# patrickltobing/cyclevae-vc

Measured on AMD Instinct MI355X. Metric: mcep_frames_per_sec_hu1024_ld32_cyc2, higher is better.
Workload: dtype f32 (every matrix product on exact fp32 operands: each operand carried as three fp16 limbs x = l0 + l1/2^11 + l2/2^22, six v_mfma_f32_32x32x16_f16 per product, f32 accumulate; dropped terms < 2^-33 of a product; gates, carried state, projection and outputs f32)

## Files before the change

### cyclevae-vc_amd/_cabi.py

```python
import ctypes as C
import os

ABI_VERSION = 10
FLAG_PERSISTENT = 1
FLAG_PROFILE = 2
FLAG_GENERIC_STEP = 4
FLAG_STEP_TIMING = 8
FLAG_HOISTED_FRONTEND = 32
FLAG_SPLIT_F16 = 256
FLAG_EXACT3 = 512
STATUS_RANGE = 7
STATUS_RANGE_WORD = 3
CLAMP_LAPLACE = 1 << 30

_HERE = os.path.dirname(os.path.abspath(__file__))
DEFAULT_LIB = os.environ.get("CYCLEVAE_LIB") or os.path.join(_HERE, "libcyclevae_hip.so")

_fp = C.c_void_p


class NetDesc(C.Structure):
    _fields_ = [("in_dim", C.c_int32), ("out_dim", C.c_int32), ("hidden", C.c_int32), ("kernel_size", C.c_int32),
                ("layers", C.c_int32), ("has_scale_in", C.c_int32), ("has_scale_out", C.c_int32)]


WEIGHT_FIELDS = ("scale_in_w", "scale_in_b", "conv0_w", "conv0_b", "conv1_w", "conv1_b", "w_ih", "w_hh", "b_ih",
                 "b_hh", "out_w", "out_b", "scale_out_w", "scale_out_b", "conv2_w", "conv2_b")

STATE_KEYS = {"scale_in_w": "scale_in.weight", "scale_in_b": "scale_in.bias", "conv0_w": "conv.conv.0.weight",
              "conv0_b": "conv.conv.0.bias", "conv1_w": "conv.conv.1.weight", "conv1_b": "conv.conv.1.bias",
              "conv2_w": "conv.conv.2.weight", "conv2_b": "conv.conv.2.bias",
              "w_ih": "gru.weight_ih_l0", "w_hh": "gru.weight_hh_l0", "b_ih": "gru.bias_ih_l0",
              "b_hh": "gru.bias_hh_l0", "out_w": "out_1.weight", "out_b": "out_1.bias",
              "scale_out_w": "scale_out.weight", "scale_out_b": "scale_out.bias"}


class NetWeights(C.Structure):
    _fields_ = [(f, _fp) for f in WEIGHT_FIELDS]


GRAD_FIELDS = ("conv0_w", "conv0_b", "conv1_w", "conv1_b", "w_ih", "w_hh", "b_ih", "b_hh", "out_w", "out_b")


class GruLayer(C.Structure):
    _fields_ = [(f, _fp) for f in ("w_ih", "w_hh", "b_ih", "b_hh")]


def upper_layer_keys(n_layers):
    return [tuple("gru.%s_l%d" % (k, l) for k in ("weight_ih", "weight_hh", "bias_ih", "bias_hh")) for l in range(1, n_layers)]


DEEP_PER_STEP, DEEP_GENERIC, DEEP_RESIDENT = 0, 1, 2
EVAL_PER_STEP, EVAL_GENERIC, EVAL_V2, EVAL_V4, EVAL_V5, EVAL_V6, EVAL_LL, EVAL_V6H = range(8)
MAX_LAYERS = 8


class NetGrads(C.Structure):
    _fields_ = [(f, _fp) for f in GRAD_FIELDS]


class Seg(C.Structure):
    _fields_ = [("ptr", _fp), ("width", C.c_int32), ("row_stride", C.c_int32)]


class PassInput(C.Structure):
    _fields_ = [("seg0", Seg), ("seg1", Seg), ("lat", _fp), ("lat_dim", C.c_int32), ("eps", _fp),
                ("seed", C.c_uint64), ("draw_id", C.c_uint64), ("frames", C.c_int32), ("n_draws", C.c_int32),
                ("ctx_before", C.c_int32), ("ctx_after", C.c_int32), ("draw_frame0", C.c_int64), ("eps_draw_stride", C.c_int64)]


class DtwProblem(C.Structure):
    _fields_ = [("org", _fp), ("trg", _fp), ("ld_org", C.c_int64), ("ld_trg", C.c_int64), ("T1", C.c_int32), ("T2", C.c_int32),
                ("D", C.c_int32), ("mcd", C.c_int32), ("aligned", _fp), ("twf", _fp), ("frames", _fp), ("mean_out", _fp)]


STAT_GV, STAT_MCD_SPC, STAT_MCD_L1, STAT_KL, STAT_GATHER64, STAT_LATDIST = range(6)
STAT_MEANSTD64, STAT_MCD64 = 6, 7


class StatJob(C.Structure):
    _fields_ = [("kind", C.c_int32), ("rows", C.c_int32), ("c0", C.c_int32), ("c1", C.c_int32), ("src_rows", C.c_int32),
                ("pad_", C.c_int32), ("a", _fp), ("b", _fp), ("lda", C.c_int64), ("ldb", C.c_int64), ("idx", _fp), ("dst", _fp),
                ("out_off", C.c_int64)]


class LatMeanJob(C.Structure):
    _fields_ = [("lat", _fp), ("eps", _fp), ("draw_id", C.c_uint64), ("frames", C.c_int32), ("pad_", C.c_int32), ("out", _fp)]


class Mc2eJob(C.Structure):
    _fields_ = [("mc", _fp), ("is_f64", C.c_int32), ("T", C.c_int32), ("D", C.c_int32), ("pad_", C.c_int32), ("ld", C.c_int64), ("e_out", _fp)]


# ... 46 lines not shown

                def fn(*args, _raw=raw, _ctx=ctx):
                    return _raw(_ctx, *args)
            self._cache[name] = fn
        return fn


NO_CONTEXT = ("cvae_last_error_string", "cvae_abi_version", "cvae_ctx_create", "cvae_ctx_destroy")
_CDLLS = {}


class CvaeLib(object):

    def __init__(self, path=None, _cdll=None):
        path = path or DEFAULT_LIB
        if not os.path.exists(path):
            raise CvaeError("HIP library %s not found: build it with `python __graft_entry__.py` (hipcc "
                            "--offload-arch=gfx950); there is no CPU fallback" % path)
        self.path = path
        if _cdll is None:
            _cdll = _CDLLS.get(path)
        if _cdll is None:
            _cdll = _CDLLS[path] = self._declare(C.CDLL(path), path)
        self.cdll = _cdll
        self.ctx = C.c_void_p(_cdll.cvae_ctx_create())
        if not self.ctx.value:
            raise CvaeError("cvae_ctx_create failed: %s" % _cdll.cvae_last_error_string().decode())
        self.lib = _Bound(_cdll, self.ctx)

    def new_context(self):
        return CvaeLib(self.path, _cdll=self.cdll)

    def close(self):
        if getattr(self, "ctx", None) is not None and self.ctx.value:
            self.cdll.cvae_ctx_destroy(self.ctx)
            self.ctx = C.c_void_p(None)

    @staticmethod
    def _declare(L, path):
        L.cvae_last_error_string.restype = C.c_char_p
        L.cvae_abi_version.restype = C.c_int
        for fn in ("cvae_net_prepared_bytes", "cvae_net_prepare_scratch_bytes"):
            getattr(L, fn).restype = C.c_size_t
            getattr(L, fn).argtypes = [C.POINTER(NetDesc)]
        L.cvae_net_prepare.restype = C.c_int
        L.cvae_net_prepare.argtypes = [C.POINTER(NetDesc), C.POINTER(NetWeights), _fp, C.c_size_t, _fp, C.c_size_t, _fp]
        L.cvae_net_prepared_in_range.restype = C.c_int
        L.cvae_net_prepared_in_range.argtypes = [C.POINTER(NetDesc), C.c_int, _fp, _fp]
        L.cvae_pass_workspace_bytes.restype = C.c_size_t
        L.cvae_pass_workspace_bytes.argtypes = [C.POINTER(NetDesc), C.c_int, C.c_int]
        L.cvae_gru_rnn_forward.restype = C.c_int
        L.cvae_gru_rnn_forward.argtypes = [C.POINTER(NetDesc), _fp, C.POINTER(PassInput), _fp, _fp, C.c_int, C.c_int,
                                           C.c_int, _fp, _fp, _fp, _fp, C.c_size_t, C.c_int, _fp]
        L.cvae_gru_rnn_forward_stacked.restype = C.c_int
        L.cvae_gru_rnn_forward_stacked.argtypes = [C.POINTER(NetDesc), _fp, C.c_int, C.POINTER(PassInput), C.POINTER(C.c_void_p),
                                                   C.c_int, C.c_int, C.c_int, C.POINTER(C.c_void_p), _fp, C.c_size_t, C.c_int, _fp]
        L.cvae_gru_rnn_forward_stacked_carry.restype = C.c_int
        L.cvae_gru_rnn_forward_stacked_carry.argtypes = [C.POINTER(NetDesc), _fp, C.c_int, C.POINTER(PassInput), C.POINTER(C.c_void_p),
                                                         C.POINTER(C.c_void_p), C.c_int, C.c_int, C.c_int, C.POINTER(C.c_void_p),
                                                         C.POINTER(C.c_void_p), _fp, C.c_size_t, C.c_int, _fp]
        for fn in ("cvae_net_prepared_bytes_deep", "cvae_net_prepare_scratch_bytes_deep"):
            getattr(L, fn).restype = C.c_size_t
            getattr(L, fn).argtypes = [C.POINTER(NetDesc), C.c_int]
        L.cvae_net_prepare_deep.restype = C.c_int
        L.cvae_net_prepare_deep.argtypes = [C.POINTER(NetDesc), C.c_int, C.POINTER(NetWeights), C.POINTER(GruLayer), _fp, C.c_size_t, _fp,
                                            C.c_size_t, _fp]
        L.cvae_pass_workspace_bytes_deep.restype = C.c_size_t
        L.cvae_pass_workspace_bytes_deep.argtypes = [C.POINTER(NetDesc), C.c_int, C.c_int, C.c_int]
        L.cvae_plan_pass.restype = C.c_int
        L.cvae_plan_pass.argtypes = [C.POINTER(NetDesc), C.c_int, C.c_int, C.c_int]
        L.cvae_plan_pass_deep.restype = C.c_int
        L.cvae_plan_pass_deep.argtypes = [C.POINTER(NetDesc), C.c_int, C.c_int, C.c_int, C.c_int]
        L.cvae_gru_rnn_forward_deep.restype = C.c_int
        L.cvae_gru_rnn_forward_deep.argtypes = [C.POINTER(NetDesc), C.c_int, _fp, C.POINTER(PassInput), _fp, _fp, C.c_int, C.c_int,
                                                C.c_int, _fp, _fp, _fp, _fp, C.c_size_t, C.c_int, _fp]
        L.cvae_sample.restype = C.c_int
        L.cvae_sample.argtypes = [_fp, C.c_int, C.c_int, _fp, C.c_uint64, C.c_uint64, _fp, _fp, _fp]
        L.cvae_sample_laplace.restype = C.c_int
        L.cvae_sample_laplace.argtypes = [_fp, C.c_int, C.c_int, _fp, C.c_uint64, C.c_uint64, _fp, _fp, _fp]
        L.cvae_sample_laplace_backward.restype = C.c_int
        L.cvae_sample_laplace_backward.argtypes = [_fp, _fp, _fp, C.c_int, C.c_int, _fp, _fp]
        L.cvae_cycle_workspace_bytes.restype = C.c_size_t
        L.cvae_cycle_workspace_bytes.argtypes = [C.POINTER(NetDesc), C.POINTER(NetDesc), C.c_int, C.c_int, C.c_int]
        L.cvae_cycle_forward.restype = C.c_int
        L.cvae_cycle_forward.argtypes = [C.POINTER(NetDesc), _fp, C.POINTER(NetDesc), _fp, _fp, _fp, C.c_int, _fp, _fp,
                                         C.c_int, _fp, _fp, C.c_int, C.c_int, C.c_int, C.c_int, _fp, C.c_uint64,
                                         _fp, _fp, _fp, _fp, _fp, _fp, C.c_size_t, C.c_int, _fp]
        L.cvae_cycle_forward_carry.restype = C.c_int
        L.cvae_cycle_forward_carry.argtypes = L.cvae_cycle_forward.argtypes + [C.POINTER(CycleState), C.POINTER(CycleState)]
        L.cvae_workspace_status.restype = C.c_int
        L.cvae_workspace_status.argtypes = [_fp, C.POINTER(C.c_int32 * 4), _fp]
        L.cvae_train_image_bytes.restype = C.c_size_t
        L.cvae_train_image_bytes.argtypes = [C.POINTER(NetDesc)]
        L.cvae_net_prepare_train.restype = C.c_int
        L.cvae_net_prepare_train.argtypes = [C.POINTER(NetDesc), C.POINTER(NetWeights), _fp, C.c_size_t, C.c_float, _fp]
        L.cvae_net_prepare_train_v.restype = C.c_int
        L.cvae_net_prepare_train_v.argtypes = [C.POINTER(NetDesc), C.POINTER(NetWeights), _fp, C.c_size_t, C.c_float, C.c_int, _fp]
        L.cvae_train_variants_needed.restype = C.c_int
        L.cvae_train_variants_needed.argtypes = [C.POINTER(NetDesc), C.c_int, C.c_int]
        for fn in ("cvae_train_tape_bytes", "cvae_train_scratch_bytes"):
            getattr(L, fn).restype = C.c_size_t
            getattr(L, fn).argtypes = [C.POINTER(NetDesc), C.c_int, C.c_int]
        L.cvae_gru_rnn_forward_train.restype = C.c_int
        L.cvae_gru_rnn_forward_train.argtypes = [C.POINTER(NetDesc), _fp, _fp, _fp, _fp, C.c_int, C.c_int, C.c_int, _fp, _fp,
                                                 C.c_uint64, C.c_float, _fp, _fp, _fp, _fp, C.c_size_t, _fp, C.c_size_t, _fp]
        L.cvae_gru_rnn_backward.restype = C.c_int
        L.cvae_gru_rnn_backward.argtypes = [C.POINTER(NetDesc), _fp, _fp, C.c_int, C.c_int, C.c_int, _fp, _fp, C.c_size_t, _fp,
                                            C.POINTER(NetGrads), C.c_int, _fp]
        L.cvae_train_debug_counters.restype = C.c_int
        L.cvae_train_debug_counters.argtypes = [C.POINTER(NetDesc), C.c_int, C.c_int, _fp, C.POINTER(C.c_longlong * 8), _fp]
        L.cvae_adam_step.restype = C.c_int
        L.cvae_adam_step.argtypes = [_fp, _fp, _fp, _fp, C.c_size_t, C.c_float, C.c_float, C.c_float, C.c_float, C.c_int, _fp, _fp]
        L.cvae_adam_step_counted.restype = C.c_int
        L.cvae_adam_step_counted.argtypes = [_fp, _fp, _fp, _fp, C.c_size_t, C.c_float, C.c_float, C.c_float, C.c_float, _fp, _fp, _fp]
        L.cvae_sample_cat.restype = C.c_int
        L.cvae_sample_cat.argtypes = [_fp, _fp, _fp, _fp, _fp, C.c_uint64, C.c_uint64, C.c_uint64, C.c_int, C.c_int, C.c_int, C.c_int,
                                      C.c_int, _fp, _fp, _fp]
        L.cvae_sample_cat_backward.restype = C.c_int
        L.cvae_sample_cat_backward.argtypes = [_fp, _fp, _fp, C.c_int, C.c_int, C.c_int, C.c_int, C.c_int, _fp, _fp]
        L.cvae_stage4_loss.restype = C.c_int
        L.cvae_stage4_loss.argtypes = [_fp, _fp, _fp, _fp, _fp, C.c_int, C.c_int, _fp, _fp, C.c_float, C.c_int, C.c_int, C.c_int, C.c_int,
                                       _fp, _fp, _fp, _fp, _fp, _fp, C.c_int, _fp]
        L.cvae_mcd_l1.restype = C.c_int
        L.cvae_mcd_l1.argtypes = [_fp, C.c_long, _fp, C.c_long, C.c_int, C.c_int, _fp, _fp, _fp]
        L.cvae_mcd_l1_backward.restype = C.c_int
        L.cvae_mcd_l1_backward.argtypes = [_fp, C.c_long, _fp, C.c_long, C.c_int, C.c_int, _fp, _fp, _fp, _fp, _fp]
        L.cvae_kl_gauss.restype = C.c_int
        L.cvae_kl_gauss.argtypes = [_fp, C.c_long, C.c_int, C.c_int, _fp, _fp]
        L.cvae_kl_gauss_backward.restype = C.c_int
        L.cvae_kl_gauss_backward.argtypes = [_fp, C.c_long, C.c_int, C.c_int, _fp, _fp, _fp]
        L.cvae_gv_postfilter.restype = C.c_int
        L.cvae_gv_postfilter.argtypes = [_fp, C.c_int, C.c_int, _fp, _fp, _fp, _fp, _fp, _fp, _fp]
        L.cvae_mc2e.restype = C.c_int
        L.cvae_mc2e.argtypes = [_fp, C.c_int, C.c_long, C.c_int, C.c_int, C.c_double, C.c_int, _fp, _fp]
        L.cvae_mcd_aligned.restype = C.c_int
        L.cvae_mcd_aligned.argtypes = [_fp, C.c_long, _fp, C.c_long, C.c_int, C.c_int, C.c_int, C.c_int, _fp, _fp, _fp]
        L.cvae_dtw_work_bytes.restype = C.c_size_t
        L.cvae_dtw_work_bytes.argtypes = [C.c_int, C.c_int]
        L.cvae_dtw_org_to_trg.restype = C.c_int
        L.cvae_dtw_org_to_trg.argtypes = [_fp, _fp, C.c_int, C.c_int, C.c_int, C.c_int, _fp, _fp, _fp, _fp, _fp, C.c_size_t, _fp]
        L.cvae_dtw_batch_work_bytes.restype = C.c_size_t
        L.cvae_dtw_batch_work_bytes.argtypes = [C.c_int, C.c_int, C.c_int]
        L.cvae_dtw_batch.restype = C.c_int
        L.cvae_dtw_batch.argtypes = [C.POINTER(DtwProblem), C.c_int, _fp, C.c_size_t, _fp]
        L.cvae_eval_stats.restype = C.c_int
        L.cvae_eval_stats.argtypes = [_fp, C.c_int, _fp, _fp]
        L.cvae_latent_mean.restype = C.c_int
        L.cvae_latent_mean.argtypes = [C.POINTER(LatMeanJob), C.c_int, C.c_int, C.c_int, C.c_uint64, _fp]
        L.cvae_mc2e_batch_work_bytes.restype = C.c_size_t
        L.cvae_mc2e_batch_work_bytes.argtypes = [C.c_int, C.c_int, C.c_int]
        L.cvae_mc2e_batch.restype = C.c_int
        L.cvae_mc2e_batch.argtypes = [C.POINTER(Mc2eJob), C.c_int, C.c_double, C.c_int, _fp, C.c_size_t, _fp]
        L.cvae_decode_jobs.restype = C.c_int
        L.cvae_decode_jobs.argtypes = [C.POINTER(DecodeJob), C.c_int, _fp, C.c_size_t, _fp]
        L.cvae_step_timing.restype = C.c_int
        L.cvae_step_timing.argtypes = [C.POINTER(NetDesc), C.c_int, C.c_int, _fp, C.POINTER(C.c_double * 8), _fp]
        L.cvae_profile_collect.restype = C.c_int
        L.cvae_profile_collect.argtypes = [C.POINTER(C.c_double), C.POINTER(C.c_int)]
        L.cvae_profile_collect_launches.restype = C.c_int
        L.cvae_profile_collect_launches.argtypes = [C.POINTER(C.c_double), C.POINTER(C.c_int), C.POINTER(C.c_int), C.c_int]
        L.cvae_train_profile_collect.restype = C.c_int
        L.cvae_train_profile_collect.argtypes = [C.POINTER(C.c_double * 4), C.POINTER(C.c_int * 4), C.POINTER(C.c_double * 4)]
        L.cvae_set_status_sink.restype = C.c_int
        L.cvae_set_status_sink.argtypes = [_fp]
        L.cvae_status_latch.restype = C.c_int
        L.cvae_status_latch.argtypes = [_fp, _fp]
# ... 78 lines not shown
        n = len(pins)
        arr = (PassInput * n)(*pins)
        ys = (C.c_void_p * n)(*y_ins)
        outs = (C.c_void_p * n)(*trj_outs)
        self._check(self.lib.cvae_gru_rnn_forward_stacked(C.byref(d), prepared, n, arr, ys, B, T, clamp_lat_dim, outs, ws,
                                                          ws_bytes, flags, stream or None), "cvae_gru_rnn_forward_stacked")

    def gru_rnn_forward_stacked_carry(self, d, prepared, pins, y_ins, h_ins, B, T, clamp_lat_dim, trj_outs, h_lasts, ws, ws_bytes,
                                      flags=0, stream=0):
        n = len(pins)
        arr = (PassInput * n)(*pins)
        ys = (C.c_void_p * n)(*[y or None for y in y_ins])
        hi = (C.c_void_p * n)(*[h or None for h in h_ins])
        outs = (C.c_void_p * n)(*trj_outs)
        hl = (C.c_void_p * n)(*[h or None for h in h_lasts])
        self._check(self.lib.cvae_gru_rnn_forward_stacked_carry(C.byref(d), prepared, n, arr, ys, hi, B, T, clamp_lat_dim, outs, hl,
                                                                ws, ws_bytes, flags, stream or None),
                    "cvae_gru_rnn_forward_stacked_carry")

    def gru_rnn_forward(self, d, prepared, pin, y_in, h_in, B, T, clamp_lat_dim, trj_out, y_last, h_last, ws, ws_bytes,
                        flags=0, stream=0):
        self._check(self.lib.cvae_gru_rnn_forward(C.byref(d), prepared, C.byref(pin), y_in, h_in or None, B, T,
                                                  clamp_lat_dim, trj_out, y_last or None, h_last or None, ws, ws_bytes,
                                                  flags, stream or None), "cvae_gru_rnn_forward")

    def prepared_bytes_deep(self, d, n_layers):
        n = self.lib.cvae_net_prepared_bytes_deep(C.byref(d), n_layers)
        if n == 0:
            raise CvaeError("bad net descriptor / n_layers: %s" % self.lib.cvae_last_error_string().decode())
        return n

    def prepare_scratch_bytes_deep(self, d, n_layers):
        return self.lib.cvae_net_prepare_scratch_bytes_deep(C.byref(d), n_layers)

    def net_prepare_deep(self, d, n_layers, weight_ptrs, upper_ptrs, prepared, prepared_bytes, scratch, scratch_bytes, stream=0):
        if len(upper_ptrs) != n_layers - 1:
            raise CvaeError("net_prepare_deep: %d upper layers given, n_layers=%d" % (len(upper_ptrs), n_layers))
        w = NetWeights(**{f: weight_ptrs.get(f) or None for f in WEIGHT_FIELDS})
        up = (GruLayer * max(1, n_layers - 1))(*[GruLayer(*u) for u in upper_ptrs])
        self._check(self.lib.cvae_net_prepare_deep(C.byref(d), n_layers, C.byref(w), up, prepared, prepared_bytes, scratch,
                                                   scratch_bytes, stream or None), "cvae_net_prepare_deep")

    def pass_workspace_bytes_deep(self, d, n_layers, B, T):
        n = self.lib.cvae_pass_workspace_bytes_deep(C.byref(d), n_layers, B, T)
        if n == 0:
            raise CvaeError("cvae_pass_workspace_bytes_deep: bad arguments (n_layers=%d, B=%d, T=%d)" % (n_layers, B, T))
        return n

    def plan_pass(self, d, rows, T, flags=0):
        rc = self.lib.cvae_plan_pass(C.byref(d), rows, T, flags)
        if rc < 0:
            self._check(rc, "cvae_plan_pass")
        return rc

    def plan_pass_deep(self, d, n_layers, B, T, flags=0):
        rc = self.lib.cvae_plan_pass_deep(C.byref(d), n_layers, B, T, flags)
        if rc < 0:
            self._check(rc, "cvae_plan_pass_deep")
        return rc

    def gru_rnn_forward_deep(self, d, n_layers, prepared, pin, y_in, h_in, B, T, clamp_lat_dim, trj_out, y_last, h_last, ws, ws_bytes,
                             flags=0, stream=0):
        self._check(self.lib.cvae_gru_rnn_forward_deep(C.byref(d), n_layers, prepared, C.byref(pin), y_in, h_in or None, B, T,
                                                       clamp_lat_dim, trj_out, y_last or None, h_last or None, ws, ws_bytes, flags,
                                                       stream or None), "cvae_gru_rnn_forward_deep")

    def sample(self, lat, rows, lat_dim, eps, seed, draw_id, z, eps_out=None, stream=0):
        self._check(self.lib.cvae_sample(lat, rows, lat_dim, eps or None, seed, draw_id, z, eps_out or None,
                                         stream or None), "cvae_sample")

    def sample_laplace(self, lat, rows, lat_dim, eps, seed, draw_id, z, eps_out=None, stream=0):
        self._check(self.lib.cvae_sample_laplace(lat, rows, lat_dim, eps or None, seed, draw_id, z, eps_out or None, stream or None),
                    "cvae_sample_laplace")

    def sample_laplace_backward(self, dz, lat, z, rows, lat_dim, dlat, stream=0):
        self._check(self.lib.cvae_sample_laplace_backward(dz, lat, z, rows, lat_dim, dlat, stream or None), "cvae_sample_laplace_backward")

    def cycle_workspace_bytes(self, de, dd, B, T, n_cyc):
        n = self.lib.cvae_cycle_workspace_bytes(C.byref(de), C.byref(dd), B, T, n_cyc)
        if n == 0:
            raise CvaeError("cvae_cycle_workspace_bytes: bad arguments")
        return n

    def cycle_forward(self, de, enc_prep, dd, dec_prep, x, cvx, stdim, code_src, code_trg, ncode, y_in_enc, y_in_dec,
                      B, T, n_cyc, lat_dim, eps, seed, out_lat, out_rec, out_cv, out_latcv, out_reccyc, ws, ws_bytes,
                      flags=0, stream=0):
        self._check(self.lib.cvae_cycle_forward(C.byref(de), enc_prep, C.byref(dd), dec_prep, x, cvx, stdim, code_src,
                                                code_trg, ncode, y_in_enc, y_in_dec, B, T, n_cyc, lat_dim, eps or None,
                                                seed, out_lat or None, out_rec or None, out_cv or None,
                                                out_latcv or None, out_reccyc or None, ws, ws_bytes, flags,
                                                stream or None), "cvae_cycle_forward")

    def cycle_forward_carry(self, de, enc_prep, dd, dec_prep, x, cvx, stdim, code_src, code_trg, ncode, y_in_enc, y_in_dec,
                            B, T, n_cyc, lat_dim, eps, seed, out_lat, out_rec, out_cv, out_latcv, out_reccyc, ws, ws_bytes,
                            flags=0, stream=0, state_in=None, state_out=None):
        si = CycleState(*state_in) if state_in else None
        so = CycleState(*state_out) if state_out else None
        self._check(self.lib.cvae_cycle_forward_carry(C.byref(de), enc_prep, C.byref(dd), dec_prep, x, cvx, stdim, code_src,
                                                      code_trg, ncode, y_in_enc, y_in_dec, B, T, n_cyc, lat_dim, eps or None,
                                                      seed, out_lat or None, out_rec or None, out_cv or None,
                                                      out_latcv or None, out_reccyc or None, ws, ws_bytes, flags,
                                                      stream or None, C.byref(si) if si else None, C.byref(so) if so else None),
                    "cvae_cycle_forward_carry")

    def train_image_bytes(self, d):
        return self.lib.cvae_train_image_bytes(C.byref(d))

    def net_prepare_train(self, d, weight_ptrs, image, image_bytes, stream=0, gru_drop_p=0.0, variants=7):
        w = NetWeights(**{f: weight_ptrs.get(f) or None for f in WEIGHT_FIELDS})
        self._check(self.lib.cvae_net_prepare_train_v(C.byref(d), C.byref(w), image, image_bytes, gru_drop_p, int(variants),
                                                      stream or None), "cvae_net_prepare_train_v")

    def train_variants_needed(self, d, B, T):
        return self.lib.cvae_train_variants_needed(C.byref(d), B, T)

    def train_tape_bytes(self, d, B, T):
        return self.lib.cvae_train_tape_bytes(C.byref(d), B, T)

    def train_scratch_bytes(self, d, B, T):
        return self.lib.cvae_train_scratch_bytes(C.byref(d), B, T)

    def forward_train(self, d, image, x, y_in, h_in, B, T, clamp_lat_dim, cmask, gmask, seed, p_drop, trj_out, y_last, h_last,
                      tape, tape_bytes, scratch, scratch_bytes, stream=0):
        self._check(self.lib.cvae_gru_rnn_forward_train(C.byref(d), image, x, y_in, h_in or None, B, T, clamp_lat_dim,
                                                        cmask or None, gmask or None, seed, p_drop, trj_out, y_last or None,
                                                        h_last or None, tape, tape_bytes, scratch, scratch_bytes,
                                                        stream or None), "cvae_gru_rnn_forward_train")

    def backward(self, d, image, dout, B, T, clamp_lat_dim, tape, scratch, scratch_bytes, dx, grad_ptrs, accumulate=False,
                 stream=0):
        g = NetGrads(**{f: grad_ptrs[f] for f in GRAD_FIELDS})
        self._check(self.lib.cvae_gru_rnn_backward(C.byref(d), image, dout, B, T, clamp_lat_dim, tape, scratch, scratch_bytes,
                                                   dx or None, C.byref(g), int(bool(accumulate)), stream or None),
                    "cvae_gru_rnn_backward")

    def train_debug_counters(self, d, B, T, scratch, stream=0):
        out = (C.c_longlong * 8)()
        self._check(self.lib.cvae_train_debug_counters(C.byref(d), B, T, scratch, C.byref(out), stream or None),
                    "cvae_train_debug_counters")
        return list(out)

    def adam_step(self, p, g, m, v, n, lr, b1, b2, eps, step, stream=0, gate=None):
        self._check(self.lib.cvae_adam_step(p, g, m, v, n, lr, b1, b2, eps, step, gate or None, stream or None), "cvae_adam_step")

    def adam_step_counted(self, p, g, m, v, n, lr, b1, b2, eps, state, stream=0, gate=None):
        self._check(self.lib.cvae_adam_step_counted(p, g, m, v, n, lr, b1, b2, eps, state, gate or None, stream or None),
                    "cvae_adam_step_counted")

    def sample_cat(self, lat, codes, eps, seed, draws, B, T, lat_dim, ncode, out, eps_out, stream=0):
        parts = len(codes)
        c = list(codes) + [None] * (2 - parts)
        e = list(eps) + [None] * (2 - parts)
        d = list(draws) + [0] * (2 - parts)
        self._check(self.lib.cvae_sample_cat(lat, c[0], c[1] or None, e[0] or None, e[1] or None, seed, d[0], d[1], B, T, lat_dim, ncode,
                                             parts, out, eps_out, stream or None), "cvae_sample_cat")

    def sample_cat_backward(self, dout, lat, eps, B, T, lat_dim, ncode, parts, dlat, stream=0):
        self._check(self.lib.cvae_sample_cat_backward(dout, lat, eps, B, T, lat_dim, ncode, parts, dlat, stream or None),
                    "cvae_sample_cat_backward")

    def stage4_loss(self, rec, reccyc, lat, latcv, x, x_stride, stdim, w, latcv_w, kl_scale, B, T, D, lat_dim, d_rec, d_reccyc, d_lat,
                    d_latcv, frame_loss, loss, accumulate, stream=0):
        self._check(self.lib.cvae_stage4_loss(rec, reccyc or None, lat, latcv or None, x, x_stride, stdim, w, latcv_w or None, kl_scale,
                                              B, T, D, lat_dim, d_rec, d_reccyc or None, d_lat, d_latcv or None, frame_loss, loss,
                                              int(bool(accumulate)), stream or None), "cvae_stage4_loss")

# ... 48 lines not shown
        arr = (Mc2eJob * max(1, len(jobs)))(*jobs)
        self._check(self.lib.cvae_mc2e_batch(arr, len(jobs), alpha, irlen, work, work_bytes, stream or None), "cvae_mc2e_batch")

    def decode_jobs(self, jobs, work, work_bytes, stream=0):
        arr = (DecodeJob * max(1, len(jobs)))(*jobs)
        self._check(self.lib.cvae_decode_jobs(arr, len(jobs), work, work_bytes, stream or None), "cvae_decode_jobs")

    def step_timing(self, d, B, T, ws, stream=0):
        out = (C.c_double * 8)()
        self._check(self.lib.cvae_step_timing(C.byref(d), B, T, ws, C.byref(out), stream or None), "cvae_step_timing")
        return list(out)

    def set_status_sink(self, ptr):
        self._check(self.lib.cvae_set_status_sink(ptr or None), "cvae_set_status_sink")

    def status_latch(self, latch, stream=0):
        self._check(self.lib.cvae_status_latch(latch, stream or None), "cvae_status_latch")

    def set_draw_origin(self, row0, global_rows, frames_per_row=0):
        self._check(self.lib.cvae_set_draw_origin(row0, global_rows, frames_per_row), "cvae_set_draw_origin")

    def selftest_limbs(self, x_ptr, y_ptr, n, stream=None):
        self._check(self.lib.cvae_selftest_limbs(x_ptr, y_ptr, n, stream), "cvae_selftest_limbs")

    def selftest_occupy(self, blocks, lds_bytes, cycles, stream=None):
        self._check(self.lib.cvae_selftest_occupy(blocks, lds_bytes, cycles, stream), "cvae_selftest_occupy")

    def selftest_gemm_work_bytes(self):
        return self.lib.cvae_selftest_gemm_work_bytes()

    def selftest_gemm(self, case, work, work_bytes, stream=None):
        ran = (C.c_int32 * 4)()
        self._check(self.lib.cvae_selftest_gemm(C.byref(case), work or None, work_bytes, C.byref(ran), stream or None), "cvae_selftest_gemm")
        return list(ran)

    def set_side_stream(self, stream):
        self._check(self.lib.cvae_set_side_stream(stream), "cvae_set_side_stream")

    def join_side_stream(self, stream):
        self._check(self.lib.cvae_join_side_stream(stream), "cvae_join_side_stream")

    def set_draw_parts(self, parts):
        self._check(self.lib.cvae_set_draw_parts(parts), "cvae_set_draw_parts")

    def set_option(self, name, value):
        self._check(self.lib.cvae_set_option(name.encode(), int(value)), "cvae_set_option")

    def get_option(self, name):
        v = C.c_int64(0)
        self._check(self.lib.cvae_get_option(name.encode(), C.byref(v)), "cvae_get_option")
        return v.value

    def reset_options(self):
        self._check(self.lib.cvae_reset_options(), "cvae_reset_options")

    def profile_collect(self):
        ms, n = C.c_double(0.0), C.c_int(0)
        self._check(self.lib.cvae_profile_collect(C.byref(ms), C.byref(n)), "cvae_profile_collect")
        return ms.value, n.value

    def profile_collect_launches(self, cap=4096):
        ms, rows, cin = (C.c_double * cap)(), (C.c_int * cap)(), (C.c_int * cap)()
        n = self.lib.cvae_profile_collect_launches(ms, rows, cin, cap)
        if n < 0:
            raise CvaeError("cvae_profile_collect_launches failed (%d): %s" % (n, self.lib.cvae_last_error_string().decode()))
        return [(ms[i], rows[i], cin[i]) for i in range(n)]

    TRAIN_PROFILE_CLASSES = ("fwd_recurrence", "bwd_recurrence", "forward_and_dgrad_gemms", "wgrad_gemms")

    def train_profile_collect(self):
        ms, n, fl = (C.c_double * 4)(), (C.c_int * 4)(), (C.c_double * 4)()
        self._check(self.lib.cvae_train_profile_collect(C.byref(ms), C.byref(n), C.byref(fl)), "cvae_train_profile_collect")
        return {name: (ms[i], n[i], fl[i]) for i, name in enumerate(self.TRAIN_PROFILE_CLASSES)}

    def workspace_status(self, ws, stream=0):
        st = (C.c_int32 * 4)()
        self._check(self.lib.cvae_workspace_status(ws, C.byref(st), stream or None), "cvae_workspace_status")
        return list(st)


EXPORTS = ("cvae_last_error_string", "cvae_abi_version", "cvae_ctx_create", "cvae_ctx_destroy", "cvae_set_status_sink", "cvae_status_latch", "cvae_set_draw_origin", "cvae_set_draw_parts",
           "cvae_set_option", "cvae_get_option", "cvae_reset_options", "cvae_selftest_limbs", "cvae_selftest_occupy", "cvae_selftest_gemm_work_bytes", "cvae_selftest_gemm", "cvae_set_side_stream", "cvae_join_side_stream", "cvae_net_prepared_bytes", "cvae_net_prepare_scratch_bytes",
           "cvae_net_prepare", "cvae_pass_workspace_bytes", "cvae_gru_rnn_forward", "cvae_gru_rnn_forward_stacked", "cvae_gru_rnn_forward_stacked_carry", "cvae_sample", "cvae_sample_laplace", "cvae_sample_laplace_backward",
           "cvae_cycle_workspace_bytes", "cvae_cycle_forward", "cvae_cycle_forward_carry", "cvae_profile_collect", "cvae_profile_collect_launches", "cvae_train_profile_collect", "cvae_step_timing", "cvae_workspace_status",
           "cvae_train_image_bytes", "cvae_net_prepare_train", "cvae_net_prepare_train_v", "cvae_train_variants_needed", "cvae_train_tape_bytes", "cvae_train_scratch_bytes",
           "cvae_gru_rnn_forward_train", "cvae_gru_rnn_backward", "cvae_adam_step", "cvae_adam_step_counted", "cvae_train_debug_counters",
           "cvae_sample_cat", "cvae_sample_cat_backward", "cvae_stage4_loss", "cvae_mcd_l1", "cvae_mcd_l1_backward", "cvae_kl_gauss",
           "cvae_kl_gauss_backward",
           "cvae_gv_postfilter", "cvae_mcd_aligned", "cvae_mc2e", "cvae_dtw_work_bytes", "cvae_dtw_org_to_trg",
           "cvae_dtw_batch_work_bytes", "cvae_dtw_batch", "cvae_eval_stats", "cvae_latent_mean",
           "cvae_mc2e_batch_work_bytes", "cvae_mc2e_batch", "cvae_decode_jobs",
           "cvae_net_prepared_bytes_deep", "cvae_net_prepare_scratch_bytes_deep", "cvae_net_prepare_deep", "cvae_pass_workspace_bytes_deep",
           "cvae_plan_pass", "cvae_plan_pass_deep", "cvae_gru_rnn_forward_deep", "cvae_net_prepared_in_range")
```

### cyclevae-vc_amd/csrc/cvae_exact3.h

```cpp
#pragma once
#include <cvae_intrin.h>

#if defined(__HIP_DEVICE_COMPILE__)
#define CVAE_V6_IN_AGPR(x) asm volatile("" : "+a"(x))
#else
#define CVAE_V6_IN_AGPR(x) ((void)0)
#endif

struct Step6Params {
    const float* gx0;
    const float* w2s;
    float* hbuf;
    long mtot;
    float* hx;
    const float* wrec3;
    const float* afold3;
    const float* cfold;
    const float* bhn;
    const float* xt;
    int Tp, Cp;
    int B, Bp, H, T;
    unsigned* flags;
    int* status;
    long long* prof;
// ... 319 lines not shown
            if (live) {
                float sg[4];
#pragma unroll
                for (int g = 0; g < 4; ++g)
                    sg[g] = red[(0 * 32 + row) * RS + g * 8 + u] + red[(1 * 32 + row) * RS + g * 8 + u] +
                            red[(2 * 32 + row) * RS + g * 8 + u] + red[(3 * 32 + row) * RS + g * 8 + u];
                const float rg = cvae_sigmoid_fast(gxr + sg[0]);
                const float zg = cvae_sigmoid_fast(gxz + sg[1]);
                const float ng = cvae_tanh_fast(gxn + sg[2] + rg * (sg[3] + bhn));
                hn_ = ng + zg * (hold - ng);
            }
            if (keep1) hkeep1 = hn_; else hkeep0 = hn_;
            hsh[row * 8 + u] = hn_;
            unsigned short l0, l1;
            unsigned char l2;
            cvae_split3_f16b8(hn_, l0, l1, l2);
            hl[row * 8 + u] = l0;
            hl[256 + row * 8 + u] = l1;
            ((unsigned char*)(hl + 512))[row * 8 + u] = l2;
        }
        __syncthreads();
        if (tid < 64) {
            const unsigned so = ((unsigned)(c >> 1) * tstride + tile0 + (unsigned)(p.Bp >> 5)) * 2560u;
            cvae_buf_store_f4_sc1(xb_, (unsigned)(c & 1) * 512u + (unsigned)(tid & 31) * 16u, so + (unsigned)(tid >> 5) * 1024u,
                                  *(const f32x4*)(hl + tid * 8));
            if (LIMBS == 3 && tid < 32)
                cvae_buf_store_f2_sc1(xb_, 2048u + (unsigned)(c & 1) * 256u + (unsigned)tid * 8u, so, *(const f32x2*)(hl + 512 + tid * 4));
            cvae_drain_vmem();
            cvae_wave_barrier();
            if (tid == 0) cvae_atomic_store_agent(p.flags + (long)i * NB + c, (unsigned)(t + 1));
        } else if (tid < 128 && p.want_f32) {
            const int l = tid - 64, r = l >> 1, half = l & 1;
            *(f32x4*)(p.hbuf + (((long)(c >> 1) * p.mtot + row0 + p.Bp + r) * 16 + (c & 1) * 8 + half * 4)) =
                *(const f32x4*)(hsh + r * 8 + half * 4);
        }
        if constexpr (!HOIST) {
            if (k + 1 < ntask && (xmode == 1 || (xmode == 2 && wave == 0))) {
#pragma unroll
                for (int s = 0; s < RF; ++s) load_x(s);
            }
        }
        if (ntile > 1 && k + 1 < ntask) {
            const int kn = k + 1, tn = kn / ntile, in_ = ti + (kn % ntile) * rts;
            fpre = (unsigned)tn;
            if (tn > 0 && lane < 2 * KPW && 2 * s_lo + lane < NB)
                fpre = cvae_atomic_load_agent(p.flags + (long)in_ * NB + 2 * s_lo + lane);
        }
        if constexpr (FPRE && FW0_EARLY) { if (k + 1 < ntask) load_fw(0); }
        if constexpr (PROF) { const long long c1 = cvae_clock(); pc[3] += c1 - c0; c0 = c1; }
    }
    if constexpr (PROF) {
        if (p.prof && tid == 64 * ((p.exp >> 2) & 3))
            for (int q = 0; q < 4; ++q) p.prof[(long)blockIdx.x * 4 + q] = pc[q];
    }
}

struct Out6Params {
    const float* hx;
    long mtot;
    const float* wo3;
    const float* bo2;
    int H, Bp, T, B, ncell, Co, clamp_from;
    float clamp_min;
    float* out[CVAE_MAX_CELLS];
};

__global__ void k_prep_wo3(const float* wo2, float* wo3, int H, int Cop, int NT, int* unfit) {
    const int nk = H >> 4;
    const long idx = (long)blockIdx.x * blockDim.x + threadIdx.x;
    if (idx < (long)NT * nk * 512) {
        const int e = (int)(idx & 7), lane = (int)((idx >> 3) & 63), s = (int)((idx >> 9) % nk), n = (int)((idx >> 9) / nk);
        const int col = 32 * n + (lane & 31), k = 16 * s + 8 * (lane >> 5) + e;
        const float w = col < Cop ? wo2[(long)col * H + k] : 0.0f;
        unsigned short l0, l1, l2;
        cvae_split3_f16(w, l0, l1, l2);
        cvae_flag_unfit(unfit, w);
        unsigned short* dst = (unsigned short*)wo3 + (((long)n * nk + s) * 3) * 512 + lane * 8 + e;
        dst[0] = l0;
        dst[512] = l1;
        dst[1024] = l2;
    }
}

template <int KPW>
__global__ __launch_bounds__(256) void k_outproj_v6(Out6Params p) {
    constexpr float S1 = 1.0f / 2048.0f;
    constexpr int RS = 36;
    const int tid = threadIdx.x, wave = cvae_uniform(tid >> 6), lane = tid & 63, lc = lane & 31, kh = lane >> 5;
    const int nk = p.H >> 4, nt32 = p.Bp >> 5;
    const int n = blockIdx.y;
    const long tile = (long)nt32 + blockIdx.x;
    float* red = (float*)CVAE_SMEM;
    const long tstride = p.mtot >> 5;
    f32x16 a0 = cvae_zero16(), a1 = cvae_zero16(), a2 = cvae_zero16(), a3 = cvae_zero16();
    constexpr int RD = KPW < 4 ? KPW : 4;
    f32x4 ha[2 * RD], wb[3 * RD];
    f32x2 hb[RD];
    auto load = [&](int s) {
        const int sg = wave * KPW + s;
        const unsigned char* hp = (const unsigned char*)p.hx + ((long)sg * tstride + tile) * 2560;
        ha[2 * (s % RD)] = *(const f32x4*)(hp + kh * 512 + lc * 16);
        ha[2 * (s % RD) + 1] = *(const f32x4*)(hp + 1024 + kh * 512 + lc * 16);
        hb[s % RD] = *(const f32x2*)(hp + 2048 + kh * 256 + lc * 8);
        const float* wp = p.wo3 + (((long)n * nk + sg) * 3) * 256 + lane * 4;
#pragma unroll
        for (int m = 0; m < 3; ++m) wb[3 * (s % RD) + m] = *(const f32x4*)(wp + m * 256);
    };
    const bool has_k = wave * KPW < nk;
    if (has_k) {
#pragma unroll
        for (int s = 0; s < RD; ++s) load(s);
#pragma unroll
        for (int s = 0; s < KPW; ++s) {
            const f32x4 l0 = ha[2 * (s % RD)], l1 = ha[2 * (s % RD) + 1], l2 = cvae_bf8x8_to_h8(hb[s % RD]);
            const f32x4 w0 = wb[3 * (s % RD)], w1 = wb[3 * (s % RD) + 1], w2 = wb[3 * (s % RD) + 2];
            a0 = cvae_mfma_32x32x16_f16(l0, w0, a0);
            a1 = cvae_mfma_32x32x16_f16(l0, w1, a1);
            a2 = cvae_mfma_32x32x16_f16(l1, w1, a2);
            a3 = cvae_mfma_32x32x16_f16(l0, w2, a3);
            a1 = cvae_mfma_32x32x16_f16(l1, w0, a1);
            a2 = cvae_mfma_32x32x16_f16(l2, w0, a2);
            cvae_sched_fence();
            if (s + RD < KPW) load(s + RD);
        }
    }
#pragma unroll
    for (int q = 0; q < 16; ++q)
        red[(wave * 32 + (q & 3) + 8 * (q >> 2) + 4 * kh) * RS + lc] = a0[q] + (a1[q] + (a2[q] + a3[q]) * S1) * S1;
    __syncthreads();
    {
        const int r = tid >> 3;
        const long m = (long)blockIdx.x * 32 + r;
        const int t = (int)(m / p.Bp), b = (int)(m - (long)t * p.Bp);
        if (b < p.ncell * p.B) {
            const int cell = b / p.B, bb = b - cell * p.B;
            float* orow = p.out[cell] + ((long)bb * p.T + t) * p.Co;
#pragma unroll
            for (int jj = 0; jj < 4; ++jj) {
                const int cl = (tid & 7) + 8 * jj, col = 32 * n + cl;
                if (col < p.Co) {
                    float v = red[(0 * 32 + r) * RS + cl] + red[(1 * 32 + r) * RS + cl] + red[(2 * 32 + r) * RS + cl] +
                              red[(3 * 32 + r) * RS + cl] + p.bo2[col];
                    if (p.clamp_from >= 0 && col >= p.clamp_from) v = fmaxf(v, p.clamp_min);
                    orow[col] = v;
                }
            }
        }
    }
}

__global__ void k_selftest_occupy(long long cycles, int lds_words) {
    float* occupy_lds = (float*)CVAE_SMEM;
    for (int i = threadIdx.x; i < lds_words; i += blockDim.x) occupy_lds[i] = (float)i;
    __syncthreads();
    const long long t0 = cvae_clock();
    float acc = 0.f;
    int guard = 0;
    while (cvae_clock() - t0 < cycles && ++guard < (1 << 28)) {
        acc += occupy_lds[(threadIdx.x * 33 + guard) % (lds_words > 0 ? lds_words : 1)];
        cvae_sleep();
    }
    if (acc == -1.0f) occupy_lds[0] = acc;
}

__global__ void k_selftest_limbs(const float* x, float* y, long n) {
    const long i0 = 8 * ((long)blockIdx.x * blockDim.x + threadIdx.x);
    if (i0 + 8 > n) return;
    unsigned short l0[8], l1[8];
    unsigned char b[8];
#pragma unroll
    for (int e = 0; e < 8; ++e) cvae_split3_f16b8(x[i0 + e], l0[e], l1[e], b[e]);
    unsigned w0 = 0, w1 = 0;
#pragma unroll
    for (int e = 0; e < 4; ++e) {
        w0 |= (unsigned)b[e] << (8 * e);
        w1 |= (unsigned)b[4 + e] << (8 * e);
    }
    const f32x2 raw = (f32x2){__builtin_bit_cast(float, w0), __builtin_bit_cast(float, w1)};
    const f32x4 h8 = cvae_bf8x8_to_h8(raw);
#pragma unroll
    for (int e = 0; e < 8; ++e) {
        const float pair = h8[e >> 1];
        const unsigned bits = __builtin_bit_cast(unsigned, pair);
        const unsigned short hb = (unsigned short)((e & 1) ? bits >> 16 : bits & 0xffffu);
        y[i0 + e] = cvae_f16_bits_to_f32(l0[e]) + cvae_f16_bits_to_f32(l1[e]) * (1.0f / 2048.0f) +
                    cvae_f16_bits_to_f32(hb) * (1.0f / 4194304.0f);
    }
}
```

### cyclevae-vc_amd/csrc/cvae_kernels.h

```cpp
#pragma once
#include <cvae_intrin.h>
#include <stdint.h>

struct CvaeSeg {
    const float* ptr;
    int width;
    int row_stride;
};

__device__ __forceinline__ void cvae_philox(uint32_t c0, uint32_t c1, uint32_t c2, uint32_t c3, uint32_t k0,
                                            uint32_t k1, uint32_t out[4]) {
    for (int i = 0; i < 10; ++i) {
        const uint64_t p0 = (uint64_t)0xD2511F53u * c0, p1 = (uint64_t)0xCD9E8D57u * c2;
        const uint32_t n0 = (uint32_t)(p1 >> 32) ^ c1 ^ k0, n1 = (uint32_t)p1;
        const uint32_t n2 = (uint32_t)(p0 >> 32) ^ c3 ^ k1, n3 = (uint32_t)p0;
        c0 = n0; c1 = n1; c2 = n2; c3 = n3;
        k0 += 0x9E3779B9u; k1 += 0xBB67AE85u;
    }
    out[0] = c0; out[1] = c1; out[2] = c2; out[3] = c3;
}

__device__ __forceinline__ void cvae_randn_pair(uint32_t w0, uint32_t w1, float& zc, float& zs) {
    const float u1 = ((float)(w0 >> 8) + 0.5f) * (1.0f / 16777216.0f);
    const float u2 = ((float)(w1 >> 8) + 0.5f) * (1.0f / 16777216.0f);
// ... 83 lines not shown
        const int a = col >> 2, u = col & 3, j = 4 * g + u, k = 16 * c + kk;
        const int gate = a < 3 ? a : 2;
        double s = 0.0;
        if (a < 3) {
            const float* wrow = wih + (long)(gate * H + j) * tot + c2;
            for (int q = 0; q < Co; ++q) s += (double)wrow[q] * (double)wo[(long)q * H + k];
        }
        if (a != 2) s += (double)whh[(long)(gate * H + j) * H + k];
        wrec[idx] = (float)s;
    }
}

__global__ void k_prep_wrec2(const float* wih, const float* whh, const float* wo, float* wrec2, int c2, int Co,
                             int tot, int H) {
    const int nch = H >> 4;
    const long idx = (long)blockIdx.x * blockDim.x + threadIdx.x;
    if (idx < (long)nch * 4 * nch * 256) {
        const int kk = (int)(idx & 15), u = (int)((idx >> 4) & 15);
        const int c = (int)((idx >> 8) % nch), a = (int)(((idx >> 8) / nch) & 3), jg = (int)((idx >> 8) / nch / 4);
        const int j = 16 * jg + u, k = 16 * c + kk;
        const int gate = a < 3 ? a : 2;
        double s = 0.0;
        if (a < 3) {
            const float* wrow = wih + (long)(gate * H + j) * tot + c2;
            for (int q = 0; q < Co; ++q) s += (double)wrow[q] * (double)wo[(long)q * H + k];
        }
        if (a != 2) s += (double)whh[(long)(gate * H + j) * H + k];
        wrec2[idx] = (float)s;
    }
}

__global__ void k_prep_wo2(const float* wo, const float* bo, const float* sw, const float* sb, float* wo2, float* bo2,
                           int Co, int Cop, int H) {
    const long idx = (long)blockIdx.x * blockDim.x + threadIdx.x;
    if (idx < (long)Cop * H) {
        const int k = (int)(idx % H), c = (int)(idx / H);
        double s = 0.0;
        if (c < Co) {
            if (sw)
                for (int q = 0; q < Co; ++q) s += (double)sw[(long)c * Co + q] * (double)wo[(long)q * H + k];
            else
                s = (double)wo[(long)c * H + k];
        }
        wo2[idx] = (float)s;
    } else if (idx < (long)Cop * H + Cop) {
        const int c = (int)(idx - (long)Cop * H);
        double s = 0.0;
        if (c < Co) {
            if (sw) {
                s = (double)sb[c];
                for (int q = 0; q < Co; ++q) s += (double)sw[(long)c * Co + q] * (double)bo[q];
            } else {
                s = (double)bo[c];
            }
        }
        bo2[c] = (float)s;
    }
}

__global__ void k_copy2d(float* dst, long dld, const float* src, long sld, int rows, int cols) {
    const long idx = (long)blockIdx.x * blockDim.x + threadIdx.x;
    if (idx < (long)rows * cols) {
        const int c = (int)(idx % cols), r = (int)(idx / cols);
        dst[(long)r * dld + c] = src[(long)r * sld + c];
    }
}

struct ProCell {
    CvaeSeg seg0, seg1;
    const float* lat;
    const float* eps;
    uint64_t seed, draw;
    const float* y_in;
    const float* h_in;
    int frames;
    int n_draws;
    int ctx_before, ctx_after;
    long draw_frame0;
    long eps_stride;
};
#define CVAE_FRAME_VALID(p, c, t) ((t) >= -(c).ctx_before && (t) < ((c).frames > 0 ? (c).frames : (p).T) + (c).ctx_after)

#define CVAE_MAX_CELLS 32
struct ProParams {
    ProCell cell[CVAE_MAX_CELLS];
    int ncell, L;
    uint64_t frame0;
    const float* sin_w;
    const float* sin_b;
    const float* wo;
    const float* bo;
    int B, T, C, Cp, pad, Co, H, Bp, nslack, nzero;
    long mtot;
    float* xnp;
    float* hbuf;
    float* hx;
    float* xt;
    int nxt_slack;
    float* hs;
    float* xs;
    long xs_plane;
    float* dy;
    unsigned* zero_words;
    int* zero_status;
    int zero_status_n;
    unsigned* ll_counter;
    int nA, nH, nD;
    int nG;
    float* gx0;
    const float* wyT;
    int* range_word;
    int* range_epoch;
    int range_val;
    float range_at;
    const int* image_unfit;
};
#ifndef CVAE_STATUS_RANGE_WORD
#define CVAE_STATUS_RANGE_WORD 3
#endif
#define CVAE_WS_RANGE_WORD 20
#define CVAE_WS_RANGE_EPOCH 21
#define CVAE_LIMB_MAX 65504.0f
__device__ __forceinline__ bool cvae_out_of_range(float v, float bound) { return !(fabsf(v) < bound); }
__device__ __forceinline__ void cvae_flag_unfit(int* unfit, float w) {
    if (cvae_out_of_range(w, CVAE_LIMB_MAX)) *unfit = 1;
}
static_assert(sizeof(ProParams) <= 4096, "ProParams is a kernel argument: 4 KiB at most");

__device__ __forceinline__ float cvae_input_value(const ProParams& p, const ProCell& c, int b, int t, int q, const float* emean = nullptr) {
    const long fr = (long)b * p.T + t;
    if (q < c.seg0.width) return c.seg0.ptr[fr * c.seg0.row_stride + q];
    if (!c.lat) return c.seg1.ptr[fr * c.seg1.row_stride + (q - c.seg0.width)];
    const int l = q - c.seg0.width;
    float e;
    if (c.n_draws > 1 && emean) {
        e = emean[l];
    } else if (c.n_draws > 1) {
        e = 0.0f;
        const long es = c.eps_stride ? c.eps_stride : (long)p.B * p.T * p.L;
        for (int k = 0; k < c.n_draws; ++k)
            e += c.eps ? c.eps[(long)k * es + fr * p.L + l]
                       : cvae_randn(c.seed, c.draw + (uint64_t)k, (uint64_t)(fr + c.draw_frame0) + p.frame0, (uint32_t)l);
        e *= 1.0f / (float)c.n_draws;
    } else {
        e = c.eps ? c.eps[fr * p.L + l] : cvae_randn(c.seed, c.draw, (uint64_t)(fr + c.draw_frame0) + p.frame0, (uint32_t)l);
    }
    return c.lat[fr * 2 * p.L + l] + expf(c.lat[fr * 2 * p.L + p.L + l] * 0.5f) * e;
}

__device__ __forceinline__ void cvae_mean_draws(const ProParams& p, const ProCell& c, int b, int t, float* part, float* emean) {
    const int tid = threadIdx.x, L = p.L, nq = L >> 2, nsl = 256 / nq, qd = tid % nq, sl = tid / nq;
    const long fr = (long)b * p.T + t;
    const long es = c.eps_stride ? c.eps_stride : (long)p.B * p.T * p.L;
    if (sl < nsl) {
        float e[4] = {0.f, 0.f, 0.f, 0.f};
        for (int k = sl; k < c.n_draws; k += nsl) {
            float z[4];
            if (c.eps) {
                const float* ep = c.eps + (long)k * es + fr * p.L + 4 * qd;
                z[0] = ep[0]; z[1] = ep[1]; z[2] = ep[2]; z[3] = ep[3];
            } else {
                cvae_randn4(c.seed, c.draw + (uint64_t)k, (uint64_t)(fr + c.draw_frame0) + p.frame0, (uint32_t)qd, z);
            }
#pragma unroll
            for (int j = 0; j < 4; ++j) e[j] += z[j];
        }
#pragma unroll
        for (int j = 0; j < 4; ++j) part[sl * L + 4 * qd + j] = e[j];
    }
    __syncthreads();
    if (tid < L) {
        float m = 0.0f;
        for (int q = 0; q < nsl; ++q) m += part[q * L + tid];
        emean[tid] = m * (1.0f / (float)c.n_draws);
    }
    __syncthreads();
}

__global__ void k_prologue(ProParams p) {
    const int tid = threadIdx.x, blk = blockIdx.x;
    const int Tp = p.T + 2 * p.pad;
    if (blk < p.nA && p.xt) {
        float* raw = (float*)CVAE_SMEM;
        unsigned char* img = (unsigned char*)(raw + 32 * (p.C + 1));
        const int tile = blk / Tp, tp = blk % Tp, t = tp - p.pad, np = p.Cp >> 3;
        float* tmean = (float*)(img + np * 1280);
        const bool quads = p.L > 0 && (p.L & 3) == 0;
        if (quads) {
            const int nq = p.L >> 2;
            for (int item = tid; item < 32 * nq; item += 256) {
                const int r = item / nq, qd = item - r * nq, bb = tile * 32 + r;
                if (bb >= p.ncell * p.B) continue;
                const ProCell& c = p.cell[bb / p.B];
                if (!c.lat || c.n_draws <= 1 || !CVAE_FRAME_VALID(p, c, t)) continue;
                const long fr = (long)(bb % p.B) * p.T + t, es = c.eps_stride ? c.eps_stride : (long)p.B * p.T * p.L;
                float e[4] = {0.f, 0.f, 0.f, 0.f};
                for (int k = 0; k < c.n_draws; ++k) {
                    float z[4];
                    if (c.eps) {
                        const float* ep = c.eps + (long)k * es + fr * p.L + 4 * qd;
                        z[0] = ep[0]; z[1] = ep[1]; z[2] = ep[2]; z[3] = ep[3];
                    } else {
                        cvae_randn4(c.seed, c.draw + (uint64_t)k, (uint64_t)(fr + c.draw_frame0) + p.frame0, (uint32_t)qd, z);
                    }
#pragma unroll
                    for (int j = 0; j < 4; ++j) e[j] += z[j];
                }
#pragma unroll
                for (int j = 0; j < 4; ++j) tmean[r * p.L + 4 * qd + j] = e[j] * (1.0f / (float)c.n_draws);
            }
            __syncthreads();
        }
        for (int idx = tid; idx < 32 * p.C; idx += 256) {
            const int r = idx / p.C, q = idx - r * p.C, bb = tile * 32 + r;
            float v = 0.0f;
            if (bb < p.ncell * p.B) {
                const ProCell& c = p.cell[bb / p.B];
                if (CVAE_FRAME_VALID(p, c, t)) v = cvae_input_value(p, c, bb % p.B, t, q, quads ? tmean + r * p.L : nullptr);
            }
            raw[r * (p.C + 1) + q] = v;
        }
        __syncthreads();
        const ProCell* const cells = p.cell;
        bool bad = false;
        for (int q = tid & 63; q < p.Cp; q += 64) {
            float v[8];
            bool ok[8];
#pragma unroll
            for (int i = 0; i < 8; ++i) {
                const int r = (tid >> 6) + 4 * i, bb = tile * 32 + r;
                ok[i] = false;
                if (bb < p.ncell * p.B) {
                    const ProCell& c = cells[bb / p.B];
                    ok[i] = CVAE_FRAME_VALID(p, c, t) && q < p.C;
                }
                v[i] = !ok[i] ? 0.0f : (p.sin_w ? p.sin_b[q] : raw[r * (p.C + 1) + q]);
            }
            if (p.sin_w && q < p.C)
                for (int k = 0; k < p.C; ++k) {
                    const float w = p.sin_w[(long)q * p.C + k];
#pragma unroll
                    for (int i = 0; i < 8; ++i) v[i] += w * raw[((tid >> 6) + 4 * i) * (p.C + 1) + k];
                }
            unsigned char* pc = img + (q >> 3) * 1280;
#pragma unroll
            for (int i = 0; i < 8; ++i) {
                const int r = (tid >> 6) + 4 * i;
                unsigned short l0, l1;
                unsigned char l2;
                cvae_split3_f16b8(ok[i] ? v[i] : 0.0f, l0, l1, l2);
                bad = bad || (ok[i] && cvae_out_of_range(v[i], p.range_at));
                ((unsigned short*)pc)[r * 8 + (q & 7)] = l0;
                ((unsigned short*)(pc + 512))[r * 8 + (q & 7)] = l1;
                pc[1024 + r * 8 + (q & 7)] = l2;
            }
        }
        const bool fits = cvae_block_all(!bad);
        if (!fits && p.range_word && tid == 0) *p.range_word = p.range_val;
        f32x4* dst = (f32x4*)((unsigned char*)p.xt + ((long)tile * Tp + tp) * np * 1280);
        for (int e = tid; e < np * 80; e += 256) dst[e] = ((const f32x4*)img)[e];
        return;
    }
    if (p.nG > 0 && blk >= p.nA + p.nH + p.nD && blk < p.nA + p.nH + p.nD + p.nG) {
        const long q4 = ((long)(blk - p.nA - p.nH - p.nD) * blockDim.x + tid) * 4, H3 = 3L * p.H;
        if (q4 < (long)p.ncell * p.B * H3) {
            const int bb = (int)(q4 / H3), col = (int)(q4 - (long)bb * H3);
            const float* yi = p.cell[bb / p.B].y_in + (long)(bb % p.B) * p.Co;
            float a0 = 0.f, a1 = 0.f, a2 = 0.f, a3 = 0.f;
            int c = 0;
            for (; c + 8 <= p.Co; c += 8) {
                float d[8], w[8][4];
#pragma unroll
                for (int q = 0; q < 8; ++q) {
                    d[q] = yi[c + q] - p.bo[c + q];
                    const float* wp = p.wyT + (long)(c + q) * H3 + col;
                    w[q][0] = wp[0]; w[q][1] = wp[1]; w[q][2] = wp[2]; w[q][3] = wp[3];
                }
#pragma unroll
                for (int q = 0; q < 8; ++q) { a0 += w[q][0] * d[q]; a1 += w[q][1] * d[q]; a2 += w[q][2] * d[q]; a3 += w[q][3] * d[q]; }
            }
            for (; c < p.Co; ++c) {
                const float d = yi[c] - p.bo[c];
                const float* w = p.wyT + (long)c * H3 + col;
                a0 += w[0] * d; a1 += w[1] * d; a2 += w[2] * d; a3 += w[3] * d;
            }
            float* o = p.gx0 + (long)bb * H3 + col;
            o[0] = a0; o[1] = a1; o[2] = a2; o[3] = a3;
        }
        return;
    }
    const float* emean = nullptr;
    if (blk < p.nA && blockDim.x == 256) {
        const int tp = blk % Tp, bb = blk / Tp, t = tp - p.pad;
        if (bb < p.ncell * p.B) {
            const ProCell& c = p.cell[bb / p.B];
            if (c.lat && c.n_draws > 1 && p.L <= 256 && (p.L & 3) == 0 && CVAE_FRAME_VALID(p, c, t)) {
                float* part = (float*)CVAE_SMEM + p.C;
                cvae_mean_draws(p, c, bb % p.B, t, part, part + 1024);
                emean = part + 1024;
            }
        }
    }
    if (tid >= 64) return;
    if (blk < p.nA) {
        float* row = (float*)CVAE_SMEM;
        const int tp = blk % Tp, bb = blk / Tp, t = tp - p.pad;
        const bool real_row = bb < p.ncell * p.B;
        const int ci = real_row ? bb / p.B : 0, b = real_row ? bb % p.B : 0;
        const ProCell& c = p.cell[ci];
        const bool valid = real_row && CVAE_FRAME_VALID(p, c, t);
        const long fr = (long)b * p.T + t;
        if (valid)
            for (int q = tid; q < p.C; q += 64) row[q] = cvae_input_value(p, c, b, t, q, emean);
        __syncthreads();
        bool bad = false;
        for (int q = tid; q < p.Cp; q += 64) {
            float v = 0.0f;
            if (valid && q < p.C) {
                if (p.sin_w) {
                    v = p.sin_b[q];
                    for (int r = 0; r < p.C; ++r) v += p.sin_w[(long)q * p.C + r] * row[r];
                } else {
                    v = row[q];
                }
            }
            if (real_row) p.xnp[((long)bb * Tp + tp) * p.Cp + q] = v;
            if (p.xs) {
                unsigned short hi, lo;
                cvae_split_f16(v, hi, lo);
                unsigned short* xh = (unsigned short*)p.xs + ((long)bb * Tp + tp) * p.Cp + q;
                xh[0] = hi;
                xh[p.xs_plane] = lo;
                bad = bad || cvae_out_of_range(v, p.range_at);
            }
        }
        if (p.xs && p.range_word && !cvae_wave_all(!bad) && tid == 0) *p.range_word = p.range_val;
    } else if (blk < p.nA + p.nH) {
        const long base = (long)(blk - p.nA) * 1024;
        bool any_h = false;
        for (int c = 0; c < p.ncell; ++c) any_h = any_h || p.cell[c].h_in != nullptr;
        if (!any_h) {
            const f32x4 z4 = (f32x4){0.f, 0.f, 0.f, 0.f};
            const long nel = (long)p.Bp * p.H, hb_ = blk - p.nA;
            for (int e = 0; e < 4; ++e) {
                const long idx = base + 4 * (e * 64 + tid);
                if (idx < nel) *(f32x4*)(p.hbuf + ((idx >> 4) / p.Bp * p.mtot + (idx >> 4) % p.Bp) * 16 + (idx & 15)) = z4;
            }
            if (p.hx) {
                const long per = (long)(p.Bp >> 5) * 160, npc = (long)(p.H >> 4) * per;
                for (int e = 0; e < 5; ++e) {
                    const long pi = hb_ * 320 + e * 64 + tid;
                    if (pi < npc) *(f32x4*)((unsigned char*)p.hx + (pi / per) * (p.mtot >> 5) * 2560 + (pi % per) * 16) = z4;
                }
            }
            if (p.hs) {
                const long per = (long)p.Bp * 4, npc = (long)(p.H >> 4) * per;
                for (int e = 0; e < 4; ++e) {
                    const long pi = hb_ * 256 + e * 64 + tid;
                    if (pi < npc) *(f32x4*)((unsigned char*)p.hs + (pi / per) * p.mtot * 64 + (pi % per) * 16) = z4;
                }
            }
            return;
        }
        bool bad = false;
        for (int e = 0; e < 16; ++e) {
            const long idx = base + e * 64 + tid;
            if (idx < (long)p.Bp * p.H) {
                const int kk = (int)(idx & 15), r = (int)((idx >> 4) % p.Bp), ch = (int)((idx >> 4) / p.Bp);
                float v = 0.0f;
                if (r < p.ncell * p.B) {
                    const float* h_in = p.cell[r / p.B].h_in;
                    if (h_in) v = h_in[(long)(r % p.B) * p.H + 16 * ch + kk];
                }
                p.hbuf[((long)ch * p.mtot + r) * 16 + kk] = v;
                bad = bad || cvae_out_of_range(v, p.range_at);
                if (p.hx) {
                    unsigned short l0, l1;
                    unsigned char l2;
                    cvae_split3_f16b8(v, l0, l1, l2);
                    unsigned char* pc = (unsigned char*)p.hx + ((long)ch * (p.mtot >> 5) + (r >> 5)) * 2560;
                    const int at = (kk >> 3) * 256 + (r & 31) * 8 + (kk & 7);
                    ((unsigned short*)pc)[at] = l0;
                    ((unsigned short*)(pc + 1024))[at] = l1;
                    pc[2048 + at] = l2;
                }
                if (p.hs) {
                    unsigned short hi, lo;
                    cvae_split_f16(v, hi, lo);
                    unsigned short* hrow = (unsigned short*)p.hs + ((long)ch * p.mtot + r) * 32;
                    hrow[kk] = hi;
                    hrow[16 + kk] = lo;
                }
            }
        }
        if (p.range_word && !cvae_wave_all(!bad) && tid == 0) *p.range_word = p.range_val;
    } else if (blk < p.nA + p.nH + p.nD) {
        const int idx = (blk - p.nA - p.nH) * 64 + tid;
        if (idx < p.ncell * p.B * p.Co) {
            const int q = idx % p.Co, bb = idx / p.Co;
            const ProCell& c = p.cell[bb / p.B];
            const int b = bb % p.B;
            float yh = p.bo[q];
            if (c.h_in && c.y_in)
                for (int k = 0; k < p.H; ++k) yh += p.wo[(long)q * p.H + k] * c.h_in[(long)b * p.H + k];
            p.dy[idx] = c.y_in ? c.y_in[(long)b * p.Co + q] - yh : 0.0f;
        }
    } else {
        for (int q = tid; q < p.nslack; q += 64) p.xnp[(long)p.ncell * p.B * Tp * p.Cp + q] = 0.0f;
        if (p.xs)
            for (int q = tid; q < p.nslack; q += 64) {
                unsigned short* xh = (unsigned short*)p.xs + (long)p.ncell * p.B * Tp * p.Cp + q;
                xh[0] = 0;
                xh[p.xs_plane] = 0;
            }
        if (p.xt)
            for (int q = tid; q < p.nxt_slack; q += 64) ((unsigned short*)p.xt)[(long)(p.Bp >> 5) * Tp * (p.Cp >> 3) * 640 + q] = 0;
        for (int q = tid; q < p.nzero; q += 64) p.zero_words[q] = 0u;
        if (p.zero_status && tid < p.zero_status_n && tid != CVAE_STATUS_RANGE_WORD) p.zero_status[tid] = 0;
        if (tid == 0) {
            if (p.range_epoch) *p.range_epoch = p.range_val;
            if (p.range_word && p.image_unfit && *p.image_unfit) *p.range_word = p.range_val;
        }
        if (p.ll_counter && tid == 0) *p.ll_counter += 1u;
    }
}

__global__ void k_sample(const float* lat, int rows, int L, const float* eps, uint64_t seed, uint64_t draw,
                         float* z, float* eps_out, uint64_t frame0) {
    const long idx = (long)blockIdx.x * blockDim.x + threadIdx.x;
    if (idx < (long)rows * L) {
        const int l = (int)(idx % L);
        const long n = idx / L;
        const float e = eps ? eps[idx] : cvae_randn(seed, draw, (uint64_t)n + frame0, (uint32_t)l);
        z[idx] = lat[n * 2 * L + l] + expf(lat[n * 2 * L + L + l] * 0.5f) * e;
        if (eps_out) eps_out[idx] = e;
    }
}

__global__ void k_sample_laplace(const float* lat, int rows, int L, const float* eps, uint64_t seed, uint64_t draw, float* z,
                                 float* eps_out, uint64_t frame0) {
    const long idx = (long)blockIdx.x * blockDim.x + threadIdx.x;
    if (idx < (long)rows * L) {
        const int l = (int)(idx % L);
        const long n = idx / L;
        float e;
        if (eps) {
            e = eps[idx];
        } else {
            const uint64_t frame = (uint64_t)n + frame0;
            uint32_t o[4];
            cvae_philox((uint32_t)frame, (uint32_t)l >> 2, (uint32_t)draw, (uint32_t)(frame >> 32), (uint32_t)seed, (uint32_t)(seed >> 32), o);
            e = -0.4999f + 0.9999f * (((float)o[l & 3] + 0.5f) * 2.3283064365386963e-10f);
            e = fminf(fmaxf(e, -0.4999f), 0.49999997f);
        }
        const float sgn = e > 0.f ? 1.f : (e < 0.f ? -1.f : 0.f);
        z[idx] = lat[n * 2 * L + l] - expf(lat[n * 2 * L + L + l]) * sgn * log1pf(-2.0f * fabsf(e));
        if (eps_out) eps_out[idx] = e;
    }
}
__global__ void k_sample_laplace_bwd(const float* dz, const float* lat, const float* z, int rows, int L, float* dlat) {
    const long idx = (long)blockIdx.x * blockDim.x + threadIdx.x;
    if (idx < (long)rows * L) {
        const int l = (int)(idx % L);
        const long n = idx / L;
        const float g = dz[idx];
        dlat[n * 2 * L + l] = g;
        dlat[n * 2 * L + L + l] = g * (z[idx] - lat[n * 2 * L + l]);
    }
}

template <int TM, int TN, int WGM, int WGN, bool A_CHUNKED>
__global__ __launch_bounds__(64 * WGM * WGN) void k_gemm_nt(const float* __restrict__ A, long lda, long a_plane,
                                                            const float* __restrict__ Bm, long ldb,
                                                            const float* __restrict__ bias, float* __restrict__ C,
                                                            long ldc, int M, int N, int K) {
    const int wave = threadIdx.x >> 6, lane = threadIdx.x & 63, lr = lane & 15, kq = lane >> 4;
    const int wm = wave / WGN, wn = wave % WGN;
    const int m0 = (blockIdx.y * WGM + wm) * TM * 16, n0 = (blockIdx.x * WGN + wn) * TN * 16;
    f32x4 acc[TM][TN];
#pragma unroll
    for (int i = 0; i < TM; ++i)
#pragma unroll
        for (int j = 0; j < TN; ++j) acc[i][j] = (f32x4){0.f, 0.f, 0.f, 0.f};
    long arow[TM], brow[TN];
#pragma unroll
    for (int i = 0; i < TM; ++i) {
        int r = m0 + 16 * i + lr;
        r = r < M ? r : M - 1;
        arow[i] = A_CHUNKED ? (long)r * 16 + 4 * kq : (long)r * lda + 4 * kq;
    }
#pragma unroll
    for (int j = 0; j < TN; ++j) {
        int c = n0 + 16 * j + lr;
        c = c < N ? c : N - 1;
        brow[j] = (long)c * ldb + 4 * kq;
    }
    for (int k0 = 0; k0 < K; k0 += 16) {
        float4 a[TM], b[TN];
        const long aoff = A_CHUNKED ? (long)(k0 >> 4) * a_plane * 16 : (long)k0;
#pragma unroll
        for (int i = 0; i < TM; ++i) a[i] = *(const float4*)(A + arow[i] + aoff);
#pragma unroll
        for (int j = 0; j < TN; ++j) b[j] = *(const float4*)(Bm + brow[j] + k0);
#pragma unroll
        for (int i = 0; i < TM; ++i)
#pragma unroll
            for (int j = 0; j < TN; ++j) {
                acc[i][j] = cvae_mfma_16x16x4(a[i].x, b[j].x, acc[i][j]);
                acc[i][j] = cvae_mfma_16x16x4(a[i].y, b[j].y, acc[i][j]);
// ... 828 lines not shown
```

### cyclevae-vc_amd/csrc/cvae_lib.hip

```cpp
#include <cvae_intrin.h>

#include <stdarg.h>
#include <stdio.h>
#include <stdlib.h>
#include <string.h>

#include <atomic>
#include <map>
#include <mutex>
#include <new>
#include <utility>
#include <vector>

#include "cvae_kernels.h"
#include "cvae_train_kernels.h"
#include "cvae_deep.h"
#include "cyclevae_hip.h"

namespace {

thread_local char g_err[512] = "";

enum OptId {
    OPT_V6_LIMBS_H64, OPT_NO_LL, OPT_MAX_RT, OPT_LL_BACKOFF, OPT_EXP, OPT_GEMM_FORCE, OPT_GEMM_LOG, OPT_TRAIN_OLD_GEMM,
    OPT_GEMM_TRACE, OPT_TRAIN_PER_STEP, OPT_TRAIN_PROF, OPT_TRAIN_BACKOFF, OPT_TRAIN_FP32_MFMA, OPT_TRAIN_BWD_PER_STEP, OPT_TRAIN_KERNEL, OPT_X3_TILE, OPT_BWD_OVERFLOW_AT, OPT_GEMM_MAX_SPLIT, OPT_BWD_KS, OPT_COOP_LAUNCH, OPT_V6_LIMBS_H2048, OPT_V6_W2S_H64, OPT_STEP_COL_TILES, OPT_TRAIN_PROFILE, OPT_TRAIN_XMAP, OPT_MASKS_ON_SIDE, OPT_V6_BACKOFF, OPT_TRAIN_BWD_BACKOFF, OPT_LL_ROW_PAD, OPT_GEMM_MIN_DEPTH, OPT_TRAIN_BWD_GEOM, OPT_BWD_W3_L1_H64, OPT_TRAIN_FWD_GEOM, OPT_TRAIN_FWD_BACKOFF, OPT_EXACT_RANGE_AT, OPT_DTW_BATCH_COST, OPT_COUNT
};
struct OptEntry { const char* name; long dflt; };
const OptEntry g_opt[OPT_COUNT] = {
    {"v6_limbs_h64", 3},
    {"no_ll", 0},
    {"max_rt", 0},
    {"ll_backoff", -1},
    {"exp", 0},
    {"gemm_force", 0},
    {"gemm_log", 0},
    {"train_old_gemm", 0},
    {"gemm_trace", 0},
    {"train_per_step", 0},
    {"train_prof", 0},
    {"train_backoff", 32},
    {"train_fp32_mfma", 0},
    {"train_bwd_per_step", 0},
    {"train_kernel", 0},
    {"x3_tile", 0},
    {"bwd_overflow_at", 60000},
    {"gemm_max_split", 16},
    {"bwd_ks", 8},
    {"coop_launch", 0},
    {"v6_limbs_h2048", 3},
    {"v6_w2s_h64", 0},
    {"step_col_tiles", 0},
    {"train_profile", 0},
    {"train_xmap", 0},
    {"masks_on_side", 1},
    {"v6_backoff", -1},
    {"train_bwd_backoff", -1},
    {"ll_row_pad", 0},
    {"gemm_min_depth", 128},
    {"train_bwd_geom", -1},
    {"bwd_w3_l1_h64", 0},
    {"train_fwd_geom", -1},
    {"train_fwd_backoff", -1},
    {"exact_range_at", 65504},
    {"dtw_batch_cost", 1},
};

struct ProfEvents {
    std::vector<hipEvent_t> start, stop;
    std::vector<int> rows, cin;
    size_t used = 0;
};
enum { TPROF_FWD = 0, TPROF_BWD = 1, TPROF_GEMM = 2, TPROF_WGRAD = 3, TPROF_CLASSES = 4 };
struct TrainProfEvents {
    std::vector<hipEvent_t> start, stop;
    std::vector<int> cls;
    std::vector<double> flop;
    size_t used = 0;
};
struct SideDone { const void* scratch; hipEvent_t ev; };

}

struct cvae_ctx {
    int32_t* status_sink = nullptr;
    long draw_row0 = 0, draw_rows = 0, draw_frames = 0, draw_parts = 1;
    long opt[OPT_COUNT];
    ProfEvents prof;
    TrainProfEvents tprof;
    hipStream_t side = nullptr;
    SideDone side_done[8] = {};
    hipEvent_t side_ready = nullptr, side_join = nullptr, side_last = nullptr;
    int side_cap = 0;
    hipEvent_t mask_fork = nullptr, mask_join = nullptr;
    unsigned side_evict = 0;
    int32_t* gemm_ran = nullptr;
    std::map<const void*, std::pair<int, unsigned long>> train_var;
    unsigned long train_var_tick = 0;
    std::map<const void*, bool> image_unfit;
    int range_serial = 0;
    std::atomic<unsigned> ll_train_launch{1u};
};

namespace {

thread_local cvae_ctx* tl_ctx = nullptr;
inline cvae_ctx& cx() { return *tl_ctx; }
inline long opt(OptId i) { return tl_ctx->opt[i]; }
struct CtxScope {
    cvae_ctx* prev;
    explicit CtxScope(cvae_ctx* c) : prev(tl_ctx) {
        tl_ctx = c;
        g_cvae_coop_launch = (int)c->opt[OPT_COOP_LAUNCH];
    }
    ~CtxScope() { tl_ctx = prev; }
};

int fail(int code, const char* fmt, ...) {
    va_list ap;
    va_start(ap, fmt);
    vsnprintf(g_err, sizeof(g_err), fmt, ap);
    va_end(ap);
    return code;
}

#define CVAE_ENTER(c)                                                          \
    if (!(c)) return fail(-1, "null context (cvae_ctx_create)");               \
    CtxScope cvae_scope_(c)
#define CVAE_ENTER_SZ(c)                                                       \
    if (!(c)) {                                                                \
        (void)fail(-1, "null context (cvae_ctx_create)");                      \
        return 0;                                                              \
    }                                                                          \
    CtxScope cvae_scope_(c)

#define CVAE_HIP_OK(expr)                                                                         \
    do {                                                                                          \
        hipError_t e_ = (expr);                                                                   \
        if (e_ != hipSuccess) return fail(-3, "%s failed: %s", #expr, hipGetErrorString(e_));     \
    } while (0)

inline long up(long x, long m) { return (x + m - 1) / m * m; }
inline int clamp_dim(int v) { return v < 0 ? -1 : (v & ~CVAE_CLAMP_LAPLACE); }
inline float clamp_floor(int v) { return v >= 0 && (v & CVAE_CLAMP_LAPLACE) ? -7.2543288692621097f : -13.815510557964274f; }
inline unsigned nblk(long n, int per) { return (unsigned)((n + per - 1) / per); }

struct Dims {
    int C, Cp, Co, Cop, H, H3, ks, layers, R, pad, cl[3], cw, tot, Kfe, nch, KFW;
};

int make_dims(const cvae_net_desc* d, Dims* o) {
    if (!d) return fail(-1, "null net descriptor");
    if (d->layers < 1 || d->layers > 3) return fail(-1, "layers (reference dilation_size) must be 1, 2 or 3, got %d", d->layers);
    if (d->kernel_size < 1 || d->kernel_size % 2 == 0) return fail(-1, "kernel_size must be odd, got %d", d->kernel_size);
    if (d->hidden < 16 || d->hidden % 16) return fail(-1, "hidden must be a positive multiple of 16, got %d", d->hidden);
    if (d->in_dim < 1 || d->out_dim < 1) return fail(-1, "bad in_dim/out_dim %d/%d", d->in_dim, d->out_dim);
    if (d->layers == 3 && d->kernel_size != 3)
        return fail(-1, "layers == 3 needs kernel_size == 3: a front-end of kernel_size^3 >= 125 frames is not supported, got kernel_size %d",
                    d->kernel_size);
    if (d->layers == 3 && d->hidden % 64)
        return fail(-1, "layers == 3 needs hidden to be a multiple of 64, got %d", d->hidden);
    o->C = d->in_dim;
    o->Cp = (int)up(d->in_dim, 8);
    o->Co = d->out_dim;
    o->Cop = (int)up(d->out_dim, 16);
    o->H = d->hidden;
    o->H3 = 3 * d->hidden;
    o->ks = d->kernel_size;
    o->layers = d->layers;
    o->R = 1;
    o->cl[0] = o->cl[1] = o->cl[2] = 0;
    for (int i = 0; i < o->layers; ++i) {
        o->R *= o->ks;
        o->cl[i] = o->R * o->C;
    }
    o->pad = (o->R - 1) / 2;
    o->cw = o->R * o->C;
    o->tot = o->cw + o->Co;
    o->Kfe = (int)up((long)o->R * o->Cp, 16);
    o->nch = o->H / 16;
    o->KFW = (o->Kfe / 16 + 3) / 4;
    return 0;
}

int make_train_dims(const cvae_net_desc* d, Dims* o) {
    if (int rc = make_dims(d, o)) return rc;
    if (o->layers != 2)
        return fail(-1, "training is implemented for layers (reference dilation_size) == 2 only, got %d (eval and conversion run 1..3)", o->layers);
    return 0;
}

struct FoldScratch { long ma, mb, ba, bb, total; };
inline long fold_m_size(const Dims& m, int n) { return (long)m.cl[n] * (m.cl[n] / m.C) * m.C; }
inline FoldScratch fold_scratch(const Dims& m) {
    FoldScratch f;
    f.ma = 0;
    f.mb = fold_m_size(m, m.layers - 1);
    f.ba = f.mb + (m.layers > 1 ? fold_m_size(m, m.layers - 2) : 0);
    f.bb = f.ba + m.cw;
    f.total = f.bb + (m.layers > 1 ? m.cl[m.layers - 2] : 0) + 64;
    return f;
}

struct V6Inst { int H, KFW, limbs; bool w2s; void (*fn)(Step6Params); void (*fn_prof)(Step6Params); };
#define V6_PAIR(KPW, KFW, LIMBS) k_gru_steps_v6<KPW, KFW, LIMBS>, k_gru_steps_v6<KPW, KFW, LIMBS, false, true>
#define V6_W2S(KPW, KFW) k_gru_steps_v6<KPW, KFW, 3, true>, nullptr
const V6Inst g_v6_inst[] = {
    {1024, 8, 3, false, V6_PAIR(16, 8, 3)},  {1024, 6, 3, false, V6_PAIR(16, 6, 3)},
    {1024, 3, 3, false, V6_PAIR(16, 3, 3)},  {1024, 2, 3, false, V6_PAIR(16, 2, 3)},
    {2048, 8, 3, true, V6_W2S(32, 8)},       {2048, 11, 3, true, V6_W2S(32, 11)},
    {2048, 8, 2, false, V6_PAIR(32, 8, 2)},  {2048, 11, 2, false, V6_PAIR(32, 11, 2)},
    {64, 3, 3, false, V6_PAIR(1, 3, 3)},     {64, 2, 3, false, V6_PAIR(1, 2, 3)},          {64, 1, 3, false, V6_PAIR(1, 1, 3)},
    {64, 3, 3, true, V6_W2S(1, 3)},          {64, 2, 3, true, V6_W2S(1, 2)},               {64, 1, 3, true, V6_W2S(1, 1)},
    {64, 3, 2, false, V6_PAIR(1, 3, 2)},     {64, 2, 2, false, V6_PAIR(1, 2, 2)},          {64, 1, 2, false, V6_PAIR(1, 1, 2)},
};
const int V6H_MIN_KFW = 12;
const V6Inst g_v6h_inst[] = {
    {1024, 0, 3, false, V6_PAIR(16, 0, 3)},
    {2048, 0, 3, true, V6_W2S(32, 0)},
    {64, 0, 3, false, V6_PAIR(1, 0, 3)},     {64, 0, 3, true, V6_W2S(1, 0)},               {64, 0, 2, false, V6_PAIR(1, 0, 2)},
};
#undef V6_PAIR
#undef V6_W2S
struct Fused16Inst { int H, KFW; void (*v5)(Step3Params); void (*v4)(Step3Params); };
const Fused16Inst g_fused16_inst[] = {
    {1024, 8, k_gru_steps_v5<16, 8>, k_gru_steps_v4<16, 8>}, {1024, 6, k_gru_steps_v5<16, 6>, k_gru_steps_v4<16, 6>},
    {64, 2, k_gru_steps_v5<1, 2>, k_gru_steps_v4<1, 2>},     {64, 1, k_gru_steps_v5<1, 1>, k_gru_steps_v4<1, 1>},
};
struct Out6Inst { int H; void (*fn)(Out6Params); };
const Out6Inst g_out6_inst[] = {{1024, k_outproj_v6<16>}, {2048, k_outproj_v6<32>}, {64, k_outproj_v6<1>}};

inline int exact3_kpw(const Dims& m) { return m.H / 64; }
inline const V6Inst* find_v6(const Dims& m, int limbs = -1, bool w2s = false) {
    for (const V6Inst& i : g_v6_inst)
        if (i.H == m.H && i.KFW == m.KFW && (limbs < 0 || (i.limbs == limbs && i.w2s == w2s))) return &i;
    return nullptr;
}
inline const Fused16Inst* find_fused16(const Dims& m) {
    for (const Fused16Inst& i : g_fused16_inst)
        if (i.H == m.H && i.KFW == m.KFW) return &i;
    return nullptr;
}
inline const V6Inst* find_v6h(const Dims& m, int limbs = -1, bool w2s = false) {
    if (m.KFW < V6H_MIN_KFW) return nullptr;
    for (const V6Inst& i : g_v6h_inst)
        if (i.H == m.H && (limbs < 0 || (i.limbs == limbs && i.w2s == w2s))) return &i;
    return nullptr;
}
inline bool exact3_fused(const Dims& m) { return find_v6(m) != nullptr; }
inline bool exact3_ok(const Dims& m) { return exact3_fused(m) || find_v6h(m) != nullptr; }
inline int v6_limbs(const Dims& m) {
    return (m.H == 64 && opt(OPT_V6_LIMBS_H64) == 2) || (m.H == 2048 && opt(OPT_V6_LIMBS_H2048) == 2) ? 2 : 3;
}
inline bool v6_w2s(const Dims& m) { return v6_limbs(m) == 3 && (m.H == 2048 || (m.H == 64 && opt(OPT_V6_W2S_H64))); }

struct Prep {
    long afold, afold3, afold_h, afold_t, cfold, wrec, wrec2, wrec_h, wrec_t, wrec_l2b, bhn, wyT, wo, bo, wo2, bo2, wo3, sin_w, sin_b, sout_w,
        sout_b, range, total;
};

Prep prep_layout(const Dims& m, bool sin, bool sout) {
    Prep p;
    long o = 0;
    auto take = [&](long n) { long r = o; o += up(n, 64); return r; };
    p.afold = take((long)m.H3 * m.Kfe);
    p.afold3 = take((long)m.nch * 4 * m.KFW * 3 * 256);
    p.afold_h = take((long)m.nch * 4 * ((m.KFW + 1) / 2) * 6 * 256);
    p.cfold = take(m.H3);
    p.wrec = take((long)(m.H / 4) * m.nch * 256);
    p.wrec2 = take((long)m.nch * 4 * m.nch * 256);
    p.wrec_h = take((long)m.nch * 4 * (m.H / 32) * 2 * 256);
    p.wrec_t = exact3_ok(m) ? take((long)(m.H / 8) * 4 * exact3_kpw(m) * 3 * 256) : -1;
    p.afold_t = exact3_fused(m) ? take((long)(m.H / 8) * 4 * m.KFW * 3 * 256) : -1;
    p.wrec_l2b = exact3_ok(m) ? take((long)(m.H / 8) * 4 * exact3_kpw(m) * 128) : -1;
    p.bhn = take(m.H);
    p.wyT = take((long)m.H3 * m.Co);
    p.wo = take((long)m.Cop * m.H);
    p.bo = take(m.Cop);
    p.wo2 = take((long)m.Cop * m.H);
    p.bo2 = take(m.Cop);
    p.wo3 = exact3_ok(m) ? take((long)((m.Cop + 31) / 32) * (m.H / 16) * 3 * 256) : -1;
    p.sin_w = sin ? take((long)m.C * m.C) : -1;
    p.sin_b = sin ? take(m.C) : -1;
    p.sout_w = sout ? take((long)m.Co * m.Co) : -1;
    p.sout_b = sout ? take(m.Co) : -1;
    p.range = take(64);
    p.total = o;
    return p;
}

struct Work {
    long status, xnp, xs, xs_plane, xt, xt_slack, gx, hbuf, hs, y, dy, gx0, prof, flags, total;
    int Bp, Tp, prof_blocks;
    long mtot;
};

inline int eval_row_pad(const Dims& m, int Brows) {
    return Brows <= 3 ? 16 : (exact3_ok(m) || Brows > 16 ? (int)up(Brows, 32) : 16);
}

Work work_layout(const Dims& m, int Brows, int T) {
    Work w;
    w.Bp = eval_row_pad(m, Brows);
    w.Tp = T + 2 * m.pad;
    w.mtot = (long)(T + 1) * w.Bp;
    long o = 0;
    auto take = [&](long n) { long r = o; o += up(n, 64); return r; };
    w.status = take(64);
    w.xnp = take((long)Brows * w.Tp * m.Cp + 64L * m.KFW + 64);
    w.xs_plane = up((long)Brows * w.Tp * m.Cp + 64L * m.KFW + 64, 8);
    w.xs = take(w.xs_plane);
    w.xt_slack = (64L * m.KFW / 8 + 2) * 640 + 64;
    w.xt = exact3_fused(m) && w.Bp % 32 == 0 ? take(((long)w.Bp * w.Tp * m.Cp * 5 / 2 + w.xt_slack) / 2 + 8) : -1;
// ... 152 lines not shown
}

inline bool image_known_unfit(const float* P) {
    auto it = cx().image_unfit.find((const void*)P);
    return it != cx().image_unfit.end() && it->second;
}
inline void range_params(ProParams& pp, int* ws_status, bool limbs, bool new_call, const float* P, const Prep& pl) {
    if (new_call) {
        cx().range_serial += 1;
        if (cx().range_serial <= 0) cx().range_serial = 1;
    }
    long at = opt(OPT_EXACT_RANGE_AT);
    at = at < 1 ? 1 : (at > 65504 ? 65504 : at);
    pp.range_at = (float)at;
    pp.image_unfit = (const int*)(P + pl.range);
    if (cx().status_sink) {
        pp.range_word = limbs ? cx().status_sink + CVAE_STATUS_RANGE_WORD : nullptr;
        pp.range_epoch = nullptr;
        pp.range_val = CVAE_STATUS_RANGE;
    } else {
        pp.range_word = limbs ? ws_status + CVAE_WS_RANGE_WORD : nullptr;
        pp.range_epoch = new_call ? ws_status + CVAE_WS_RANGE_EPOCH : nullptr;
        pp.range_val = cx().range_serial;
    }
}

struct Cell {
    const cvae_pass_input* in;
    const float* y_in;
    const float* h_in;
    float* trj_out;
    float* y_last;
    float* h_last;
};


inline int last_slot(const cvae_pass_input* in, int T) { return in->frames > 0 && in->frames < T ? in->frames : T; }

struct PassRows {
    const Cell* cells;
    int ncell, B, T, Bp;
    long mtot;
};

int check_cells(const Dims& m, const PassRows& r) {
    const Cell* cells = r.cells;
    const int ncell = r.ncell, B = r.B, T = r.T;
    if (ncell > CVAE_MAX_CELLS) return fail(-1, "at most %d stacked cells per pass", CVAE_MAX_CELLS);
    for (int c = 0; c < ncell; ++c) {
        const cvae_pass_input* in = cells[c].in;
        const int w_in = in->seg0.width + (in->lat ? in->lat_dim : in->seg1.width);
        if (w_in != m.C) return fail(-1, "cell %d: pass input width %d != in_dim %d", c, w_in, m.C);
        if (in->frames < 0 || in->frames > T) return fail(-1, "cell %d: frames %d outside [0, T=%d]", c, in->frames, T);
        if (in->ctx_before < 0 || in->ctx_after < 0 || in->draw_frame0 < 0 || in->eps_draw_stride < 0)
            return fail(-1, "cell %d: negative window context / draw origin", c);
        if ((in->ctx_before || in->ctx_after || in->draw_frame0) && B != 1)
            return fail(-1, "cell %d: windows of a longer utterance (ctx_before / ctx_after / draw_frame0) are single-row cells, B=%d", c, B);
    }
    return 0;
}

struct ProTargets {
    int shape;
    float* xnp;
    float* dy;
    float* slot0;
    unsigned* zero_words;
    int nzero;
    int* zero_status;
    int zero_status_n;
    int* ws_status;
    bool limbs, new_call;
    float* hx;
    float* xt;
    int nxt_slack;
    float* hs;
    float* xs;
    long xs_plane;
    float* gx0;
    unsigned* ll_counter;
};
struct RangeSlot { int* word; int val; float at; };

void run_prologue(const Dims& m, const cvae_net_desc* d, const float* P, const Prep& pl, const PassRows& r, const ProTargets& o,
                  hipStream_t st, RangeSlot* range = nullptr) {
    const Cell* cells = r.cells;
    const int ncell = r.ncell, B = r.B, T = r.T, Bp = r.Bp, shape = o.shape;
    const int Brows = ncell * B, Tp = T + 2 * m.pad;
    ProParams pp;
    memset(&pp, 0, sizeof(pp));
    for (int c = 0; c < ncell; ++c) {
        const cvae_pass_input* in = cells[c].in;
        pp.cell[c].seg0 = CvaeSeg{in->seg0.ptr, in->seg0.width, in->seg0.row_stride};
        pp.cell[c].seg1 = CvaeSeg{in->seg1.ptr, in->seg1.width, in->seg1.row_stride};
        pp.cell[c].lat = in->lat;
        pp.cell[c].eps = in->eps;
        pp.cell[c].seed = in->seed;
        pp.cell[c].draw = in->draw_id;
        pp.cell[c].y_in = cells[c].y_in;
        pp.cell[c].h_in = cells[c].h_in;
        pp.cell[c].frames = in->frames;
        pp.cell[c].n_draws = in->n_draws;
        pp.cell[c].ctx_before = in->ctx_before; pp.cell[c].ctx_after = in->ctx_after;
        pp.cell[c].draw_frame0 = (long)in->draw_frame0; pp.cell[c].eps_stride = (long)in->eps_draw_stride;
        if (in->lat) pp.L = in->lat_dim;
    }
    pp.ncell = ncell;
    pp.frame0 = (uint64_t)cx().draw_row0 * (uint64_t)T;
    pp.sin_w = d->has_scale_in ? P + pl.sin_w : nullptr;
    pp.sin_b = d->has_scale_in ? P + pl.sin_b : nullptr;
    pp.wo = P + pl.wo; pp.bo = P + pl.bo;
    pp.B = B; pp.T = T; pp.C = m.C; pp.Cp = m.Cp; pp.pad = m.pad; pp.Co = m.Co; pp.H = m.H; pp.Bp = Bp;
    pp.nslack = 64 * m.KFW + 64;
    pp.mtot = r.mtot;
    pp.xnp = o.xnp; pp.hbuf = o.slot0; pp.dy = o.dy;
    pp.hx = o.hx; pp.xt = o.xt; pp.nxt_slack = o.nxt_slack;
    pp.hs = o.hs; pp.xs = o.xs; pp.xs_plane = o.xs_plane;
    pp.zero_words = o.zero_words; pp.nzero = o.nzero;
    pp.zero_status = o.zero_status; pp.zero_status_n = o.zero_status_n;
    pp.ll_counter = o.ll_counter;
    pp.nA = (shape == PRO_TILES ? Bp / 32 : Brows) * Tp;
    pp.nH = (int)nblk((long)Bp * m.H, 1024);
    pp.nD = (int)nblk((long)Brows * m.Co, 64);
    pp.nG = o.gx0 ? (int)nblk((long)Brows * m.H3 / 4, shape == PRO_ROWS ? 64 : 256) : 0;
    pp.gx0 = o.gx0; pp.wyT = P + pl.wyT;
    range_params(pp, o.ws_status, o.limbs, o.new_call, P, pl);
    if (range) *range = RangeSlot{pp.range_word, pp.range_val, pp.range_at};
    const dim3 gp(pp.nA + pp.nH + pp.nD + pp.nG + 1);
    if (shape == PRO_TILES)
        hipLaunchKernelGGL((k_prologue), gp, dim3(256),
                           (size_t)32 * (m.C + 1) * sizeof(float) + (size_t)(m.Cp / 8) * 1280 + (size_t)32 * pp.L * sizeof(float), st, pp);
    else if (shape == PRO_DRAWS)
        hipLaunchKernelGGL((k_prologue), gp, dim3(256), (size_t)(m.C + 1024 + 256) * sizeof(float), st, pp);
    else
        hipLaunchKernelGGL((k_prologue), gp, dim3(64), m.C * sizeof(float), st, pp);
}

void run_front_end_gemm(const Dims& m, const float* P, const Prep& pl, const float* xnp, float* gx, int rows, int Tp, hipStream_t st) {
    const int M = rows * Tp, N = m.H3;
    hipLaunchKernelGGL((k_gemm_nt<4, 4, 2, 2, false>), dim3(nblk(N, 128), nblk(M, 128)), dim3(256), 0, st, xnp, (long)m.Cp, 0L,
                       P + pl.afold, (long)m.Kfe, P + pl.cfold, gx, (long)m.H3, M, N, m.Kfe);
}

void run_projection(const Dims& m, const cvae_net_desc* d, const float* P, const Prep& pl, const PassRows& r, int proj, const float* hbuf,
                    float* y, int clamp_lat_dim, hipStream_t st) {
    const Cell* cells = r.cells;
    const int ncell = r.ncell, B = r.B, T = r.T, Bp = r.Bp;
    const long mtot = r.mtot;
    if (proj == PROJ_FUSED) {
        OutParams op;
        op.hbuf = hbuf; op.mtot = mtot; op.wo2 = P + pl.wo2; op.bo2 = P + pl.bo2; op.H = m.H; op.Bp = Bp; op.T = T;
        op.B = B; op.ncell = ncell; op.Co = m.Co; op.clamp_from = d->has_scale_out ? -1 : clamp_dim(clamp_lat_dim);
        op.clamp_min = clamp_floor(clamp_lat_dim);
        for (int c = 0; c < CVAE_MAX_CELLS; ++c) op.out[c] = c < ncell ? cells[c].trj_out : nullptr;
        const int ntn = m.Cop / 16;
        const unsigned nb = (unsigned)((long)T * Bp / 16);
        const size_t lds = (size_t)4 * 16 * (m.Cop + 4) * sizeof(float);
        void (*const kout)(OutParams) = ntn == 1 ? k_outproj<1> : ntn == 4 ? k_outproj<4> : k_outproj<8>;
        hipLaunchKernelGGL(kout, dim3(nb), dim3(256), lds, st, op);
        return;
    }
    const int M = T * Bp, N = m.Co;
    hipLaunchKernelGGL((k_gemm_nt<2, 4, 4, 1, true>), dim3(nblk(N, 64), nblk(M, 128)), dim3(256), 0, st, hbuf + (long)Bp * 16, 0L, mtot,
                       P + pl.wo, (long)m.H, P + pl.bo, y, (long)m.Cop, M, N, m.H);
    for (int c = 0; c < ncell; ++c) {
        EpiParams ep;
        ep.y = y; ep.ldy = m.Cop;
        ep.sout_w = d->has_scale_out ? P + pl.sout_w : nullptr;
        ep.sout_b = d->has_scale_out ? P + pl.sout_b : nullptr;
        ep.clamp_from = d->has_scale_out ? -1 : clamp_dim(clamp_lat_dim);
        ep.clamp_min = clamp_floor(clamp_lat_dim);
        ep.B = B; ep.Bp = Bp; ep.T = T; ep.Co = m.Co; ep.b0 = c * B;
        ep.trj_out = cells[c].trj_out; ep.y_last = cells[c].y_last;
        ep.t_last = last_slot(cells[c].in, T) - 1;
        hipLaunchKernelGGL((k_epilogue), dim3(B * T), dim3(64), m.Co * sizeof(float), st, ep);
    }
}

void run_last_states(const Dims& m, const PassRows& r, const float* hbuf, hipStream_t st) {
    for (int c = 0; c < r.ncell; ++c)
        if (r.cells[c].h_last)
            hipLaunchKernelGGL((k_hlast), dim3(nblk((long)r.B * m.H, 256)), dim3(256), 0, st, hbuf, r.mtot, r.cells[c].h_last, r.B, r.Bp,
                               m.H, last_slot(r.cells[c].in, r.T), c * r.B);
}

int run_pass(const Dims& m, const cvae_net_desc* d, const float* P, const Cell* cells, int ncell, int B, int T,
             int clamp_lat_dim, float* ws, int* status, int flags, hipStream_t st, bool clear_status = false) {
    const Prep pl = prep_layout(m, d->has_scale_in != 0, d->has_scale_out != 0);
    const int Brows = ncell * B;
    const Work wl = work_layout(m, Brows, T);
    int* const ws_status = status;
    if (cx().status_sink) status = cx().status_sink;
    const PassRows rows = {cells, ncell, B, T, wl.Bp, wl.mtot};
    if (int rc = check_cells(m, rows)) return rc;
    unsigned* bar = (unsigned*)(ws + wl.status) + 8;
    float* xnp = ws + wl.xnp;
    float* gx = ws + wl.gx;
    float* hbuf = ws + wl.hbuf;
    float* dy = ws + wl.dy;
    unsigned* hflags = (unsigned*)(ws + wl.flags);
    long long* const step_prof = (flags & CVAE_FLAG_STEP_TIMING) ? (long long*)(ws + wl.prof) : nullptr;
    const int cus = cu_count();
    PassFacts facts = {};
    for (int c = 0; c < ncell; ++c) {
        facts.h_in = facts.h_in || cells[c].h_in != nullptr;
        facts.y_last = facts.y_last || cells[c].y_last != nullptr;
        facts.h_last = facts.h_last || cells[c].h_last != nullptr;
        facts.many_draws = facts.many_draws || (cells[c].in->lat && cells[c].in->n_draws > 1);
    }
    const EvalPlan pn = plan_eval_pass(m, Brows, T, flags, cus, image_known_unfit(P), facts);

    {
        ProTargets o = {};
        o.shape = pn.prologue; o.xnp = xnp; o.dy = dy;
        o.slot0 = hbuf;
        o.zero_words = hflags; o.nzero = wl.Bp / 16 * m.nch;
        o.zero_status = clear_status ? status : nullptr;
        o.zero_status_n = cx().status_sink ? 4 : 8;
        o.ws_status = ws_status; o.limbs = pn.limbs; o.new_call = clear_status;
        const bool triples = pn.form == CVAE_EVAL_V6 || pn.form == CVAE_EVAL_V6H;
        o.hx = triples ? ws + wl.hs : nullptr;
        o.xt = pn.form == CVAE_EVAL_V6 ? ws + wl.xt : nullptr;
        o.nxt_slack = (int)wl.xt_slack;
        o.hs = pn.pairs ? ws + wl.hs : nullptr;
        o.xs = pn.pairs ? ws + wl.xs : nullptr;
        o.xs_plane = wl.xs_plane;
        o.gx0 = pn.gx0_ready ? ws + wl.gx0 : nullptr;
        o.ll_counter = pn.form == CVAE_EVAL_LL ? (unsigned*)(ws + wl.status) + 16 : nullptr;
        run_prologue(m, d, P, pl, rows, o, st);
    }

    const size_t lds2 = (4 * 16 * 84 + 16 * 16) * sizeof(float);
    const bool prof = (flags & CVAE_FLAG_PROFILE) && prof_begin(st, ncell * B, m.C);
    const auto refused = [](hipError_t e) {
        if (e == hipSuccess) return false;
        (void)hipGetLastError();
        return true;
    };
    int form = pn.form;
    if (form == CVAE_EVAL_LL || form == CVAE_EVAL_V6H || form <= CVAE_EVAL_V2) run_front_end_gemm(m, P, pl, xnp, gx, Brows, wl.Tp, st);
    switch (form) {
    case CVAE_EVAL_LL: {
        StepLLParams q;
        q.hbuf = hbuf; q.mtot = wl.mtot; q.xbuf = ws + wl.hs; q.wrec2 = P + pl.wrec2; q.gx = gx; q.gx_bstride = (long)wl.Tp * m.H3;
        q.bhn = P + pl.bhn; q.B = Brows; q.Bp = wl.Bp; q.H = m.H; q.T = T; q.status = status;
        q.prof = step_prof;
        q.wyT = P + pl.wyT; q.dy = dy; q.Co = m.Co;
        q.dbg = (int*)(ws + wl.status);
        q.backoff = pn.backoff;
        q.nonce_src = (const unsigned*)(ws + wl.status) + 16;
        const dim3 gl(m.H / 4);
        const size_t ldsl = (size_t)(2 * 64 * 49 + 4 * 48) * sizeof(float);
        const hipError_t e = cvae_launch_coop(Brows == 1 ? k_gru_steps_ll<1> : Brows == 2 ? k_gru_steps_ll<2> : k_gru_steps_ll<3>, gl,
                                              dim3(256), ldsl, st, q);
        if (refused(e)) return fail(-3, "small-batch recurrent kernel failed to launch: %s", hipGetErrorString(e));
        break;
    }
    case CVAE_EVAL_V6:
    case CVAE_EVAL_V6H: {
        const bool fused = form == CVAE_EVAL_V6;
        Step6Params q;
        q.hbuf = hbuf; q.mtot = wl.mtot; q.hx = ws + wl.hs; q.wrec3 = P + pl.wrec_t; q.afold3 = fused ? P + pl.afold_t : nullptr; q.w2s = P + pl.wrec_l2b;
        q.cfold = P + pl.cfold; q.bhn = P + pl.bhn; q.xt = fused ? ws + wl.xt : nullptr; q.Tp = wl.Tp; q.Cp = m.Cp;
        q.gx = fused ? nullptr : gx; q.gx_bstride = (long)wl.Tp * m.H3;
        q.B = Brows; q.Bp = wl.Bp; q.H = m.H; q.T = T; q.flags = hflags; q.status = status;
        q.prof = step_prof;
        q.wyT = P + pl.wyT; q.dy = dy; q.Co = m.Co;
        q.gx0 = pn.gx0_ready ? ws + wl.gx0 : nullptr;
        q.want_f32 = pn.want_f32 ? 1 : 0;
        q.rts = pn.rts;
        q.exp = (int)opt(OPT_EXP);
        q.backoff = pn.backoff;
        const size_t lds6 = (size_t)(4 * 32 * 40 + 32 * 8 + 384 + (fused ? 4 * m.KFW * v6_limbs(m) * 256 : 0)) * sizeof(float);
        const hipError_t e = cvae_launch_coop(pn.k6, dim3(m.H / 8 * pn.rts), dim3(256), lds6, st, q);
        if (refused(e)) return fail(-3, "exact-operand recurrent kernel failed to launch: %s", hipGetErrorString(e));
        break;
    }
    case CVAE_EVAL_V5:
    case CVAE_EVAL_V4: {
        Step3Params q;
        q.hbuf = hbuf; q.mtot = wl.mtot; q.wrec2 = P + pl.wrec2; q.cfold = P + pl.cfold;
        q.xnp = xnp; q.Tp = wl.Tp; q.Cp = m.Cp; q.bhn = P + pl.bhn; q.B = Brows; q.Bp = wl.Bp; q.H = m.H; q.T = T;
        q.flags = hflags; q.status = status;
        q.prof = step_prof;
        q.wyT = P + pl.wyT; q.dy = dy; q.Co = m.Co;
        q.rts = pn.rts;
        q.hs = ws + wl.hs; q.wrec_h = P + pl.wrec_h; q.xs = ws + wl.xs; q.xs_plane = wl.xs_plane;
        q.exp = (int)opt(OPT_EXP);
        const dim3 g(m.nch * pn.rts);
        if (form == CVAE_EVAL_V5) {
            q.afold2 = P + pl.afold_h;
            const size_t lds5 = lds2 + (size_t)4 * ((m.KFW + 1) / 2) * 6 * 256 * sizeof(float);
            if (!refused(cvae_launch_coop(pn.k5, g, dim3(256), lds5, st, q))) break;
        }
        q.afold2 = P + pl.afold3;
        const size_t lds4 = lds2 + (size_t)4 * m.KFW * 3 * 256 * sizeof(float);
        if (!refused(cvae_launch_coop(pn.k4, g, dim3(256), lds4, st, q))) break;
        run_front_end_gemm(m, P, pl, xnp, gx, Brows, wl.Tp, st);
        form = CVAE_EVAL_V2;
    }
        [[fallthrough]];
    case CVAE_EVAL_V2: {
        Step2Params q;
        q.hbuf = hbuf; q.mtot = wl.mtot; q.wrec2 = P + pl.wrec2; q.gx = gx; q.gx_bstride = (long)wl.Tp * m.H3;
        q.bhn = P + pl.bhn; q.B = Brows; q.Bp = wl.Bp; q.H = m.H; q.T = T; q.flags = hflags; q.status = status;
        q.prof = step_prof;
        q.wyT = P + pl.wyT; q.dy = dy; q.Co = m.Co;
        if (!refused(cvae_launch_coop(m.H == 1024 ? k_gru_steps_v2<16> : k_gru_steps_v2<1>, dim3(m.nch, pn.rts), dim3(256), lds2, st, q))) break;
        form = generic_resident(m, cus) ? CVAE_EVAL_GENERIC : CVAE_EVAL_PER_STEP;
    }
        [[fallthrough]];
    default: {
        const size_t step_lds = 4 * 64 * 20 * sizeof(float);
        StepParams sp;
        sp.hbuf = hbuf; sp.mtot = wl.mtot; sp.wrec = P + pl.wrec; sp.gx = gx; sp.gx_bstride = (long)wl.Tp * m.H3;
        sp.bhn = P + pl.bhn; sp.B = Brows; sp.Bp = wl.Bp; sp.H = m.H; sp.T = T; sp.t0 = 0; sp.bar = bar; sp.status = status;
        sp.nwg = (unsigned)(m.H / 4);
        sp.prof = nullptr;
        sp.wyT = P + pl.wyT; sp.dy = dy; sp.Co = m.Co;
        if (form == CVAE_EVAL_GENERIC) {
            CVAE_HIP_OK(hipMemsetAsync(bar, 0, 8 * sizeof(unsigned), st));
            if (!refused(cvae_launch_coop(k_gru_steps<true>, dim3(sp.nwg), dim3(256), step_lds, st, sp))) break;
        }
        for (int t = 0; t < T; ++t) {
            sp.t0 = t;
            hipLaunchKernelGGL((k_gru_steps<false>), dim3(sp.nwg), dim3(256), step_lds, st, sp);
        }
    }
    }
    if (prof) prof_end(st);

    if (pn.proj == PROJ_V6) {
        Out6Params op;
        op.hx = ws + wl.hs; op.mtot = wl.mtot; op.wo3 = P + pl.wo3; op.bo2 = P + pl.bo2; op.H = m.H; op.Bp = wl.Bp; op.T = T;
        op.B = B; op.ncell = ncell; op.Co = m.Co; op.clamp_from = d->has_scale_out ? -1 : clamp_dim(clamp_lat_dim);
        op.clamp_min = clamp_floor(clamp_lat_dim);
        for (int c = 0; c < CVAE_MAX_CELLS; ++c) op.out[c] = c < ncell ? cells[c].trj_out : nullptr;
        const dim3 g((unsigned)((long)T * wl.Bp / 32), (unsigned)((m.Cop + 31) / 32));
        hipLaunchKernelGGL(pn.kout6, g, dim3(256), (size_t)4 * 32 * 36 * sizeof(float), st, op);
    } else {
        run_projection(m, d, P, pl, rows, pn.proj, hbuf, ws + wl.y, clamp_lat_dim, st);
    }
    run_last_states(m, rows, hbuf, st);
    CVAE_HIP_OK(hipGetLastError());
    return 0;
}

}

extern "C" {

const char* cvae_last_error_string(void) { return g_err; }
int cvae_abi_version(void) { return CVAE_ABI_VERSION; }

cvae_ctx* cvae_ctx_create(void) {
    cvae_ctx* c = new (std::nothrow) cvae_ctx();
    if (!c) {
        (void)fail(-3, "out of memory");
        return nullptr;
    }
    for (int i = 0; i < OPT_COUNT; ++i) c->opt[i] = g_opt[i].dflt;
    c->range_serial = (int)(((uintptr_t)c >> 6) & 0x3fffffff);
    return c;
}

int cvae_ctx_destroy(cvae_ctx* ctx) {
    if (!ctx) return 0;
    if (tl_ctx == ctx) return fail(-1, "cvae_ctx_destroy from inside a call on the same context");
    for (hipEvent_t e : ctx->prof.start) (void)hipEventDestroy(e);
    for (hipEvent_t e : ctx->prof.stop) (void)hipEventDestroy(e);
    for (hipEvent_t e : ctx->tprof.start) (void)hipEventDestroy(e);
    for (hipEvent_t e : ctx->tprof.stop) (void)hipEventDestroy(e);
    for (SideDone& d : ctx->side_done)
        if (d.ev) (void)hipEventDestroy(d.ev);
    for (hipEvent_t e : {ctx->side_ready, ctx->side_join, ctx->side_last, ctx->mask_fork, ctx->mask_join})
        if (e) (void)hipEventDestroy(e);
    delete ctx;
    return 0;
}

int cvae_set_status_sink(cvae_ctx* ctx, int32_t* sink) {
    CVAE_ENTER(ctx);
    cx().status_sink = sink;
    return 0;
}

int cvae_set_draw_origin(cvae_ctx* ctx, int64_t row0, int64_t global_rows, int64_t frames_per_row) {
    CVAE_ENTER(ctx);
    if (row0 < 0 || global_rows < 0 || frames_per_row < 0 || (global_rows > 0 && row0 >= global_rows))
        return fail(-1, "bad draw origin: row0 %lld of %lld rows", (long long)row0, (long long)global_rows);
    cx().draw_row0 = (long)row0;
    cx().draw_rows = (long)global_rows;
    cx().draw_frames = (long)frames_per_row;
    return 0;
}

int cvae_selftest_limbs(cvae_ctx* ctx, const float* x, float* y, int64_t n, void* stream) {
    CVAE_ENTER(ctx);
    if (!x || !y || n < 0 || n % 8) return fail(-1, "selftest: n must be a non-negative multiple of 8");
    if (n) hipLaunchKernelGGL((k_selftest_limbs), dim3(nblk(n / 8, 256)), dim3(256), 0, (hipStream_t)stream, x, y, (long)n);
    CVAE_HIP_OK(hipGetLastError());
    return 0;
}

int cvae_selftest_occupy(cvae_ctx* ctx, int blocks, size_t lds_bytes, int64_t cycles, void* stream) {
    CVAE_ENTER(ctx);
    if (blocks < 1 || cycles < 0 || lds_bytes > 160 * 1024) return fail(-1, "selftest_occupy: bad argument");
    hipLaunchKernelGGL((k_selftest_occupy), dim3(blocks), dim3(256), lds_bytes, (hipStream_t)stream, (long long)cycles, (int)(lds_bytes / 4));
    CVAE_HIP_OK(hipGetLastError());
    return 0;
}

int cvae_set_option(cvae_ctx* ctx, const char* name, int64_t value) {
    CVAE_ENTER(ctx);
    if (!name) return fail(-1, "null option name");
    for (int i = 0; i < OPT_COUNT; ++i)
        if (!strcmp(g_opt[i].name, name)) {
            ctx->opt[i] = (long)value;
            return 0;
        }
    return fail(-1, "unknown option '%s'", name);
}

int cvae_get_option(cvae_ctx* ctx, const char* name, int64_t* value) {
    CVAE_ENTER(ctx);
    if (!name || !value) return fail(-1, "null argument");
    for (int i = 0; i < OPT_COUNT; ++i)
        if (!strcmp(g_opt[i].name, name)) {
// ... 147 lines not shown
    if (B < 1 || T < 1) return fail(-1, "empty batch: B=%d T=%d", B, T);
    if (!prepared || !in || !y_in || !trj_out || !workspace) return fail(-1, "null argument");
    if (!in->seg0.ptr || (in->seg1.width > 0 && !in->lat && !in->seg1.ptr)) return fail(-1, "null input segment");
    if (workspace_bytes < cvae_pass_workspace_bytes(ctx, d, B, T)) return fail(-2, "workspace too small");
    const Cell cell{in, y_in, h_in, trj_out, y_last, h_last};
    return run_pass(m, d, (const float*)prepared, &cell, 1, B, T, clamp_lat_dim, (float*)workspace, (int*)workspace,
                    flags, (hipStream_t)stream, true);
}

int cvae_gru_rnn_forward_stacked(cvae_ctx* ctx, const cvae_net_desc* d, const void* prepared, int ncell, const cvae_pass_input* in,
                                 const float* const* y_in, int B, int T, int clamp_lat_dim, float* const* trj_out,
                                 void* workspace, size_t workspace_bytes, int flags, void* stream) {
    CVAE_ENTER(ctx);
    Dims m;
    if (int rc = make_dims(d, &m)) return rc;
    if (B < 1 || T < 1 || ncell < 1 || ncell > CVAE_MAX_CELLS) return fail(-1, "bad sizes: ncell=%d B=%d T=%d", ncell, B, T);
    if (!prepared || !in || !y_in || !trj_out || !workspace) return fail(-1, "null argument");
    if (workspace_bytes < cvae_pass_workspace_bytes(ctx, d, ncell * B, T)) return fail(-2, "workspace too small");
    Cell cells[CVAE_MAX_CELLS];
    for (int c = 0; c < ncell; ++c) {
        if (!in[c].seg0.ptr || (in[c].seg1.width > 0 && !in[c].lat && !in[c].seg1.ptr) || !y_in[c] || !trj_out[c])
            return fail(-1, "cell %d: null pointer", c);
        cells[c] = Cell{&in[c], y_in[c], nullptr, trj_out[c], nullptr, nullptr};
    }
    return run_pass(m, d, (const float*)prepared, cells, ncell, B, T, clamp_lat_dim, (float*)workspace, (int*)workspace, flags,
                    (hipStream_t)stream, true);
}

int cvae_gru_rnn_forward_stacked_carry(cvae_ctx* ctx, const cvae_net_desc* d, const void* prepared, int ncell, const cvae_pass_input* in,
                                       const float* const* y_in, const float* const* h_in, int B, int T, int clamp_lat_dim,
                                       float* const* trj_out, float* const* h_last, void* workspace, size_t workspace_bytes,
                                       int flags, void* stream) {
    CVAE_ENTER(ctx);
    Dims m;
    if (int rc = make_dims(d, &m)) return rc;
    if (B < 1 || T < 1 || ncell < 1 || ncell > CVAE_MAX_CELLS) return fail(-1, "bad sizes: ncell=%d B=%d T=%d", ncell, B, T);
    if (!prepared || !in || !y_in || !trj_out || !workspace) return fail(-1, "null argument");
    if (workspace_bytes < cvae_pass_workspace_bytes(ctx, d, ncell * B, T)) return fail(-2, "workspace too small");
    Cell cells[CVAE_MAX_CELLS];
    for (int c = 0; c < ncell; ++c) {
        const float* hi = h_in ? h_in[c] : nullptr;
        if (!in[c].seg0.ptr || (in[c].seg1.width > 0 && !in[c].lat && !in[c].seg1.ptr) || !trj_out[c])
            return fail(-1, "cell %d: null pointer", c);
        if (!y_in[c] && !hi) return fail(-1, "cell %d: no y_in and no state to continue from", c);
        cells[c] = Cell{&in[c], y_in[c], hi, trj_out[c], nullptr, h_last ? h_last[c] : nullptr};
    }
    return run_pass(m, d, (const float*)prepared, cells, ncell, B, T, clamp_lat_dim, (float*)workspace, (int*)workspace, flags,
                    (hipStream_t)stream, true);
}

int cvae_sample(cvae_ctx* ctx, const float* lat, int rows, int lat_dim, const float* eps, uint64_t seed, uint64_t draw_id, float* z,
                float* eps_out, void* stream) {
    CVAE_ENTER(ctx);
    if (!lat || !z || rows < 0 || lat_dim < 1) return fail(-1, "bad argument");
    if (rows == 0) return 0;
    hipLaunchKernelGGL((k_sample), dim3(nblk((long)rows * lat_dim, 256)), dim3(256), 0, (hipStream_t)stream, lat, rows,
                       lat_dim, eps, seed, draw_id, z, eps_out, (uint64_t)cx().draw_row0 * (uint64_t)cx().draw_frames);
    CVAE_HIP_OK(hipGetLastError());
    return 0;
}

int cvae_sample_laplace(cvae_ctx* ctx, const float* lat, int rows, int lat_dim, const float* eps, uint64_t seed, uint64_t draw_id,
                        float* z, float* eps_out, void* stream) {
    CVAE_ENTER(ctx);
    if (!lat || !z || rows < 0 || lat_dim < 1) return fail(-1, "bad argument");
    if (rows == 0) return 0;
    hipLaunchKernelGGL((k_sample_laplace), dim3(nblk((long)rows * lat_dim, 256)), dim3(256), 0, (hipStream_t)stream, lat, rows,
                       lat_dim, eps, seed, draw_id, z, eps_out, (uint64_t)cx().draw_row0 * (uint64_t)cx().draw_frames);
    CVAE_HIP_OK(hipGetLastError());
    return 0;
}

int cvae_sample_laplace_backward(cvae_ctx* ctx, const float* dz, const float* lat, const float* z, int rows, int lat_dim, float* dlat,
                                 void* stream) {
    CVAE_ENTER(ctx);
    if (!dz || !lat || !z || !dlat || rows < 0 || lat_dim < 1) return fail(-1, "bad argument");
    if (rows == 0) return 0;
    hipLaunchKernelGGL((k_sample_laplace_bwd), dim3(nblk((long)rows * lat_dim, 256)), dim3(256), 0, (hipStream_t)stream, dz, lat, z,
                       rows, lat_dim, dlat);
    CVAE_HIP_OK(hipGetLastError());
    return 0;
}

static long cycle_layout(const Dims& me, const Dims& md, int B, int T, long* pass_off, long* traj_off) {
    const long pe = work_layout(me, B, T).total, pd = work_layout(md, 2 * B, T).total;
    long o = 64;
    *pass_off = o;
    o += pe > pd ? pe : pd;
    *traj_off = o;
    o += up((long)B * T * me.Co, 64) * 2 + up((long)B * T * md.Co, 64) * 3;
    return o;
}

size_t cvae_cycle_workspace_bytes(cvae_ctx* ctx, const cvae_net_desc* enc, const cvae_net_desc* dec, int B, int T, int n_cyc) {
    CVAE_ENTER_SZ(ctx);
    Dims me, md;
    if (make_dims(enc, &me) || make_dims(dec, &md) || B < 1 || T < 1 || n_cyc < 1) return 0;
    long po, to;
    return (size_t)cycle_layout(me, md, B, T, &po, &to) * sizeof(float);
}

static int cycle_forward_impl(const cvae_net_desc* enc, const void* enc_prepared, const cvae_net_desc* dec,
                       const void* dec_prepared, const float* x, const float* cvx, int stdim, const float* code_src,
                       const float* code_trg, int ncode, const float* y_in_enc, const float* y_in_dec, int B, int T,
                       int n_cyc, int lat_dim, const float* eps, uint64_t seed, float* out_lat, float* out_rec,
                       float* out_cv, float* out_latcv, float* out_reccyc, void* workspace, size_t workspace_bytes,
                       int flags, void* stream, const cvae_cycle_state* sin, const cvae_cycle_state* sout) {
    Dims me, md;
    if (int rc = make_dims(enc, &me)) return rc;
    if (int rc = make_dims(dec, &md)) return rc;
    if (B < 1 || T < 1 || n_cyc < 1) return fail(-1, "empty work: B=%d T=%d n_cyc=%d", B, T, n_cyc);
    if (!enc_prepared || !dec_prepared || !x || !cvx || !code_src || !code_trg || !y_in_enc || !y_in_dec || !workspace)
        return fail(-1, "null argument");
    if (me.Co != 2 * lat_dim) return fail(-1, "encoder out_dim %d != 2*lat_dim %d", me.Co, 2 * lat_dim);
    if (md.C != ncode + lat_dim) return fail(-1, "decoder in_dim %d != ncode+lat_dim %d", md.C, ncode + lat_dim);
    if (me.C != stdim + md.Co) return fail(-1, "encoder in_dim %d != stdim+decoder out_dim %d", me.C, stdim + md.Co);
    if (workspace_bytes < cvae_cycle_workspace_bytes(tl_ctx, enc, dec, B, T, n_cyc)) return fail(-2, "workspace too small");
    hipStream_t st = (hipStream_t)stream;
    float* ws = (float*)workspace;
    long po, to;
    cycle_layout(me, md, B, T, &po, &to);
    float* pws = ws + po;
    const long ne = (long)B * T * me.Co, nd = (long)B * T * md.Co;
    float* t_lat = ws + to;
    float* t_latcv = t_lat + up(ne, 64);
    float* t_rec = t_latcv + up(ne, 64);
    float* t_cv = t_rec + up(nd, 64);
    float* t_reccyc = t_cv + up(nd, 64);
    const float* prev_reccyc = nullptr;
    int* status = (int*)workspace;
    const long neps = (long)B * T * lat_dim;
    if (sin && (!sin->y_enc || !sin->y_dec || !sin->h_enc || !sin->h_dec)) return fail(-1, "incomplete input cycle state");
    if (sout && (!sout->y_enc || !sout->y_dec || !sout->h_enc || !sout->h_dec)) return fail(-1, "incomplete output cycle state");
    auto ye = [&](const cvae_cycle_state* s, int i, int slot) { return s ? s->y_enc + ((long)i * 2 + slot) * B * me.Co : nullptr; };
    auto he = [&](const cvae_cycle_state* s, int i, int slot) { return s ? s->h_enc + ((long)i * 2 + slot) * B * me.H : nullptr; };
    auto yd = [&](const cvae_cycle_state* s, int i, int slot) { return s ? s->y_dec + ((long)i * 3 + slot) * B * md.Co : nullptr; };
    auto hd = [&](const cvae_cycle_state* s, int i, int slot) { return s ? s->h_dec + ((long)i * 3 + slot) * B * md.H : nullptr; };

    for (int i = 0; i < n_cyc; ++i) {
        float* lat = out_lat ? out_lat + i * ne : t_lat;
        float* latcv = out_latcv ? out_latcv + i * ne : t_latcv;
        float* rec = out_rec ? out_rec + i * nd : t_rec;
        float* cv = out_cv ? out_cv + i * nd : t_cv;
        float* reccyc = out_reccyc ? out_reccyc + i * nd : t_reccyc;
        cvae_pass_input in, in2;
        memset(&in, 0, sizeof(in));
        int rc;
        if (i == 0) {
            in.seg0 = cvae_seg{x, me.C, me.C};
        } else {
            in.seg0 = cvae_seg{x, stdim, me.C};
            in.seg1 = cvae_seg{prev_reccyc, md.Co, md.Co};
        }
        {
            const Cell c{&in, sin ? ye(sin, i, 0) : y_in_enc, he(sin, i, 0), lat, ye(sout, i, 0), he(sout, i, 0)};
            if ((rc = run_pass(me, enc, (const float*)enc_prepared, &c, 1, B, T, lat_dim, pws, status, flags, st, i == 0))) return rc;
        }
        memset(&in, 0, sizeof(in));
        in.seg0 = cvae_seg{code_src, ncode, ncode};
        in.lat = lat; in.lat_dim = lat_dim;
        in.eps = eps ? eps + (i * 3 + 0) * neps : nullptr;
        in.seed = seed; in.draw_id = (uint64_t)(i * 3 + 0);
        in2 = in;
        in2.seg0 = cvae_seg{code_trg, ncode, ncode};
        in2.eps = eps ? eps + (i * 3 + 1) * neps : nullptr;
        in2.draw_id = (uint64_t)(i * 3 + 1);
        {
            const Cell c2[2] = {{&in, sin ? yd(sin, i, 0) : y_in_dec, hd(sin, i, 0), rec, yd(sout, i, 0), hd(sout, i, 0)},
                                {&in2, sin ? yd(sin, i, 1) : y_in_dec, hd(sin, i, 1), cv, yd(sout, i, 1), hd(sout, i, 1)}};
            if ((rc = run_pass(md, dec, (const float*)dec_prepared, c2, 2, B, T, -1, pws, status, flags, st))) return rc;
        }
        memset(&in, 0, sizeof(in));
        in.seg0 = cvae_seg{cvx, stdim, stdim};
        in.seg1 = cvae_seg{cv, md.Co, md.Co};
        {
            const Cell c{&in, sin ? ye(sin, i, 1) : y_in_enc, he(sin, i, 1), latcv, ye(sout, i, 1), he(sout, i, 1)};
            if ((rc = run_pass(me, enc, (const float*)enc_prepared, &c, 1, B, T, lat_dim, pws, status, flags, st))) return rc;
        }
        memset(&in, 0, sizeof(in));
        in.seg0 = cvae_seg{code_src, ncode, ncode};
        in.lat = latcv; in.lat_dim = lat_dim;
        in.eps = eps ? eps + (i * 3 + 2) * neps : nullptr;
        in.seed = seed; in.draw_id = (uint64_t)(i * 3 + 2);
        {
            const Cell c{&in, sin ? yd(sin, i, 2) : y_in_dec, hd(sin, i, 2), reccyc, yd(sout, i, 2), hd(sout, i, 2)};
            if ((rc = run_pass(md, dec, (const float*)dec_prepared, &c, 1, B, T, -1, pws, status, flags, st))) return rc;
        }
        prev_reccyc = reccyc;
    }
    return 0;
}

int cvae_cycle_forward(cvae_ctx* ctx, const cvae_net_desc* enc, const void* enc_prepared, const cvae_net_desc* dec,
                       const void* dec_prepared, const float* x, const float* cvx, int stdim, const float* code_src,
                       const float* code_trg, int ncode, const float* y_in_enc, const float* y_in_dec, int B, int T,
                       int n_cyc, int lat_dim, const float* eps, uint64_t seed, float* out_lat, float* out_rec,
                       float* out_cv, float* out_latcv, float* out_reccyc, void* workspace, size_t workspace_bytes,
                       int flags, void* stream) {
    CVAE_ENTER(ctx);
    return cycle_forward_impl(enc, enc_prepared, dec, dec_prepared, x, cvx, stdim, code_src, code_trg, ncode, y_in_enc, y_in_dec,
                              B, T, n_cyc, lat_dim, eps, seed, out_lat, out_rec, out_cv, out_latcv, out_reccyc, workspace,
                              workspace_bytes, flags, stream, nullptr, nullptr);
}

int cvae_cycle_forward_carry(cvae_ctx* ctx, const cvae_net_desc* enc, const void* enc_prepared, const cvae_net_desc* dec,
                             const void* dec_prepared, const float* x, const float* cvx, int stdim, const float* code_src,
                             const float* code_trg, int ncode, const float* y_in_enc, const float* y_in_dec, int B, int T,
                             int n_cyc, int lat_dim, const float* eps, uint64_t seed, float* out_lat, float* out_rec,
                             float* out_cv, float* out_latcv, float* out_reccyc, void* workspace, size_t workspace_bytes,
                             int flags, void* stream, const cvae_cycle_state* state_in, const cvae_cycle_state* state_out) {
    CVAE_ENTER(ctx);
    return cycle_forward_impl(enc, enc_prepared, dec, dec_prepared, x, cvx, stdim, code_src, code_trg, ncode, y_in_enc, y_in_dec,
                              B, T, n_cyc, lat_dim, eps, seed, out_lat, out_rec, out_cv, out_latcv, out_reccyc, workspace,
                              workspace_bytes, flags, stream, state_in, state_out);
}

int cvae_step_timing(cvae_ctx* ctx, const cvae_net_desc* d, int B, int T, const void* workspace, double out[8], void* stream) {
    CVAE_ENTER(ctx);
    Dims m;
    if (int rc = make_dims(d, &m)) return rc;
    if (!workspace || !out || B < 1 || T < 1) return fail(-1, "bad argument");
    const Work wl = work_layout(m, B, T);
    const EvalPlan pn = plan_eval_pass(m, B, T, CVAE_FLAG_PERSISTENT, cu_count(), false, PassFacts{});
    const int nwg = pn.rts < 1 ? 1 : (m.nch * pn.rts > wl.prof_blocks ? wl.prof_blocks : m.nch * pn.rts);
    std::vector<long long> h((size_t)nwg * 4);
    CVAE_HIP_OK(hipMemcpyAsync(h.data(), (const float*)workspace + wl.prof, h.size() * sizeof(long long),
                               hipMemcpyDeviceToHost, (hipStream_t)stream));
    CVAE_HIP_OK(hipStreamSynchronize((hipStream_t)stream));
    for (int q = 0; q < 4; ++q) {
        double sum = 0, mx = 0;
        for (int g = 0; g < nwg; ++g) {
            const double v = (double)h[(size_t)g * 4 + q];
            sum += v;
            mx = v > mx ? v : mx;
        }
        out[q] = sum / nwg;
        out[4 + q] = mx;
    }
    return 0;
}

int cvae_profile_collect_launches(cvae_ctx* ctx, double* ms, int* rows, int* cin, int cap) {
    CVAE_ENTER(ctx);
    const int n = (int)cx().prof.used < cap ? (int)cx().prof.used : cap;
    for (int i = 0; i < n; ++i) {
        float t = 0.f;
        CVAE_HIP_OK(hipEventSynchronize(cx().prof.stop[i]));
        CVAE_HIP_OK(hipEventElapsedTime(&t, cx().prof.start[i], cx().prof.stop[i]));
        if (ms) ms[i] = t;
        if (rows) rows[i] = cx().prof.rows[i];
        if (cin) cin[i] = cx().prof.cin[i];
    }
    cx().prof.used = 0;
    return n;
}

int cvae_profile_collect(cvae_ctx* ctx, double* total_ms, int* launches) {
    CVAE_ENTER(ctx);
    double tot = 0.0;
    for (size_t i = 0; i < cx().prof.used; ++i) {
        float ms = 0.f;
        CVAE_HIP_OK(hipEventSynchronize(cx().prof.stop[i]));
        CVAE_HIP_OK(hipEventElapsedTime(&ms, cx().prof.start[i], cx().prof.stop[i]));
        tot += ms;
    }
    if (total_ms) *total_ms = tot;
    if (launches) *launches = (int)cx().prof.used;
    cx().prof.used = 0;
    return 0;
}

int cvae_train_profile_collect(cvae_ctx* ctx, double total_ms[4], int launches[4], double flop[4]) {
    CVAE_ENTER(ctx);
    for (int c = 0; c < TPROF_CLASSES; ++c) {
        if (total_ms) total_ms[c] = 0.0;
        if (launches) launches[c] = 0;
        if (flop) flop[c] = 0.0;
    }
    for (size_t i = 0; i < cx().tprof.used; ++i) {
        float ms = 0.f;
        CVAE_HIP_OK(hipEventSynchronize(cx().tprof.stop[i]));
        CVAE_HIP_OK(hipEventElapsedTime(&ms, cx().tprof.start[i], cx().tprof.stop[i]));
        const int c = cx().tprof.cls[i];
        if (total_ms) total_ms[c] += ms;
        if (launches) launches[c] += 1;
        if (flop) flop[c] += cx().tprof.flop[i];
    }
    cx().tprof.used = 0;
    return 0;
}

int cvae_workspace_status(cvae_ctx* ctx, const void* workspace, int32_t status_out[4], void* stream) {
    CVAE_ENTER(ctx);
    if (!workspace || !status_out) return fail(-1, "null argument");
    int32_t w[CVAE_WS_RANGE_EPOCH + 1];
    CVAE_HIP_OK(hipMemcpyAsync(w, workspace, sizeof(w), hipMemcpyDeviceToHost, (hipStream_t)stream));
    CVAE_HIP_OK(hipStreamSynchronize((hipStream_t)stream));
// ... 30 lines not shown
```

### include/cyclevae_hip.h

```cpp
#ifndef CYCLEVAE_HIP_H
#define CYCLEVAE_HIP_H

#include <stddef.h>
#include <stdint.h>

#ifdef __cplusplus
extern "C" {
#endif

#define CVAE_ABI_VERSION 10

typedef struct cvae_net_desc {
    int32_t in_dim;
    int32_t out_dim;
    int32_t hidden;
    int32_t kernel_size;
    int32_t layers;
    int32_t has_scale_in;
    int32_t has_scale_out;
} cvae_net_desc;

typedef struct cvae_net_weights {
    const float* scale_in_w;
    const float* scale_in_b;
// ... 6 lines not shown
    const float* b_ih;
    const float* b_hh;
    const float* out_w;
    const float* out_b;
    const float* scale_out_w;
    const float* scale_out_b;
    const float* conv2_w;
    const float* conv2_b;
} cvae_net_weights;

typedef struct cvae_seg {
    const float* ptr;
    int32_t width;
    int32_t row_stride;
} cvae_seg;

typedef struct cvae_pass_input {
    cvae_seg seg0, seg1;
    const float* lat;
    int32_t lat_dim;
    const float* eps;
    uint64_t seed;
    uint64_t draw_id;
    int32_t frames;
    int32_t n_draws;
    int32_t ctx_before, ctx_after;
    int64_t draw_frame0;
    int64_t eps_draw_stride;
} cvae_pass_input;

const char* cvae_last_error_string(void);
int cvae_abi_version(void);

typedef struct cvae_ctx cvae_ctx;
cvae_ctx* cvae_ctx_create(void);
int cvae_ctx_destroy(cvae_ctx* ctx);

int cvae_set_status_sink(cvae_ctx* ctx, int32_t* sink);
int cvae_status_latch(cvae_ctx* ctx, int32_t* latch, void* stream);
int cvae_set_draw_origin(cvae_ctx* ctx, int64_t row0, int64_t global_rows, int64_t frames_per_row);
int cvae_set_draw_parts(cvae_ctx* ctx, int32_t parts);

int cvae_set_option(cvae_ctx* ctx, const char* name, int64_t value);
int cvae_get_option(cvae_ctx* ctx, const char* name, int64_t* value);
int cvae_reset_options(cvae_ctx* ctx);

int cvae_selftest_limbs(cvae_ctx* ctx, const float* x, float* y, int64_t n, void* stream);
int cvae_selftest_occupy(cvae_ctx* ctx, int blocks, size_t lds_bytes, int64_t cycles, void* stream);
enum { CVAE_GEMM_NT = 0, CVAE_GEMM_TN = 1, CVAE_GEMM_KS = 2, CVAE_GEMM_COLSUM = 3 };
#define CVAE_SELFTEST_GEMM_CNT 4096
typedef struct cvae_gemm_case {
    int32_t kind, accumulate, use_split;
    int32_t M, N, K;
    int32_t seglen;
    int32_t mask_B, mask_Bp, mask_T;
    int64_t lda, ldb, ldc, segstride;
    int64_t a_lo, a_hi, b_lo, b_hi, c_hi;
    const float* A;
    const float* B;
    const float* bias;
    const float* mask;
    float* C;
} cvae_gemm_case;
size_t cvae_selftest_gemm_work_bytes(cvae_ctx* ctx);
int cvae_selftest_gemm(cvae_ctx* ctx, const cvae_gemm_case* c, void* work, size_t work_bytes, int32_t ran[4], void* stream);

size_t cvae_net_prepared_bytes(cvae_ctx* ctx, const cvae_net_desc* d);
size_t cvae_net_prepare_scratch_bytes(cvae_ctx* ctx, const cvae_net_desc* d);

int cvae_net_prepare(cvae_ctx* ctx, const cvae_net_desc* d, const cvae_net_weights* w, void* prepared, size_t prepared_bytes,
                     void* scratch, size_t scratch_bytes, void* stream);
int cvae_net_prepared_in_range(cvae_ctx* ctx, const cvae_net_desc* d, int n_layers, const void* prepared, void* stream);

size_t cvae_pass_workspace_bytes(cvae_ctx* ctx, const cvae_net_desc* d, int B, int T);

#define CVAE_FLAG_PERSISTENT 1
#define CVAE_FLAG_HOISTED_FRONTEND 32
#define CVAE_FLAG_SPLIT_F16 256
#define CVAE_CLAMP_LAPLACE (1 << 30)
#define CVAE_FLAG_EXACT3 512
#define CVAE_FLAG_GENERIC_STEP 4
#define CVAE_FLAG_STEP_TIMING 8
#define CVAE_FLAG_PROFILE 2

#define CVAE_STATUS_RANGE 7
#define CVAE_STATUS_RANGE_WORD 3

typedef enum cvae_eval_form {
    CVAE_EVAL_PER_STEP = 0,
    CVAE_EVAL_GENERIC = 1,
    CVAE_EVAL_V2 = 2,
    CVAE_EVAL_V4 = 3,
    CVAE_EVAL_V5 = 4,
    CVAE_EVAL_V6 = 5,
    CVAE_EVAL_LL = 6,
    CVAE_EVAL_V6H = 7
} cvae_eval_form;
int cvae_plan_pass(cvae_ctx* ctx, const cvae_net_desc* d, int rows, int T, int flags);

int cvae_gru_rnn_forward(cvae_ctx* ctx, const cvae_net_desc* d, const void* prepared, const cvae_pass_input* in,
                         const float* y_in, const float* h_in, int B, int T, int clamp_lat_dim,
                         float* trj_out, float* y_last, float* h_last,
                         void* workspace, size_t workspace_bytes, int flags, void* stream);

int cvae_gru_rnn_forward_stacked(cvae_ctx* ctx, const cvae_net_desc* d, const void* prepared, int ncell, const cvae_pass_input* in,
                                 const float* const* y_in, int B, int T, int clamp_lat_dim, float* const* trj_out,
                                 void* workspace, size_t workspace_bytes, int flags, void* stream);

int cvae_gru_rnn_forward_stacked_carry(cvae_ctx* ctx, const cvae_net_desc* d, const void* prepared, int ncell, const cvae_pass_input* in,
                                       const float* const* y_in, const float* const* h_in, int B, int T, int clamp_lat_dim,
                                       float* const* trj_out, float* const* h_last, void* workspace, size_t workspace_bytes,
                                       int flags, void* stream);

typedef struct cvae_gru_layer {
    const float* w_ih;
    const float* w_hh;
    const float* b_ih;
    const float* b_hh;
} cvae_gru_layer;
size_t cvae_net_prepared_bytes_deep(cvae_ctx* ctx, const cvae_net_desc* d, int n_layers);
size_t cvae_net_prepare_scratch_bytes_deep(cvae_ctx* ctx, const cvae_net_desc* d, int n_layers);
int cvae_net_prepare_deep(cvae_ctx* ctx, const cvae_net_desc* d, int n_layers, const cvae_net_weights* w, const cvae_gru_layer* upper,
                          void* prepared, size_t prepared_bytes, void* scratch, size_t scratch_bytes, void* stream);
size_t cvae_pass_workspace_bytes_deep(cvae_ctx* ctx, const cvae_net_desc* d, int n_layers, int B, int T);
int cvae_plan_pass_deep(cvae_ctx* ctx, const cvae_net_desc* d, int n_layers, int B, int T, int flags);
int cvae_gru_rnn_forward_deep(cvae_ctx* ctx, const cvae_net_desc* d, int n_layers, const void* prepared, const cvae_pass_input* in,
                              const float* y_in, const float* h_in, int B, int T, int clamp_lat_dim, float* trj_out, float* y_last,
                              float* h_last, void* workspace, size_t workspace_bytes, int flags, void* stream);

int cvae_sample(cvae_ctx* ctx, const float* lat, int rows, int lat_dim, const float* eps, uint64_t seed, uint64_t draw_id,
                float* z, float* eps_out, void* stream);

int cvae_sample_laplace(cvae_ctx* ctx, const float* lat, int rows, int lat_dim, const float* eps, uint64_t seed, uint64_t draw_id,
                        float* z, float* eps_out, void* stream);
int cvae_sample_laplace_backward(cvae_ctx* ctx, const float* dz, const float* lat, const float* z, int rows, int lat_dim, float* dlat,
                                 void* stream);

size_t cvae_cycle_workspace_bytes(cvae_ctx* ctx, const cvae_net_desc* enc, const cvae_net_desc* dec, int B, int T, int n_cyc);

int cvae_cycle_forward(cvae_ctx* ctx, const cvae_net_desc* enc, const void* enc_prepared,
                       const cvae_net_desc* dec, const void* dec_prepared,
                       const float* x, const float* cvx, int stdim,
                       const float* code_src, const float* code_trg, int ncode,
                       const float* y_in_enc, const float* y_in_dec,
                       int B, int T, int n_cyc, int lat_dim, const float* eps, uint64_t seed,
                       float* out_lat, float* out_rec, float* out_cv, float* out_latcv, float* out_reccyc,
                       void* workspace, size_t workspace_bytes, int flags, void* stream);

typedef struct cvae_cycle_state {
    float* y_enc;
    float* y_dec;
    float* h_enc;
    float* h_dec;
} cvae_cycle_state;
int cvae_cycle_forward_carry(cvae_ctx* ctx, const cvae_net_desc* enc, const void* enc_prepared,
                             const cvae_net_desc* dec, const void* dec_prepared,
                             const float* x, const float* cvx, int stdim,
                             const float* code_src, const float* code_trg, int ncode,
                             const float* y_in_enc, const float* y_in_dec,
                             int B, int T, int n_cyc, int lat_dim, const float* eps, uint64_t seed,
                             float* out_lat, float* out_rec, float* out_cv, float* out_latcv, float* out_reccyc,
                             void* workspace, size_t workspace_bytes, int flags, void* stream,
                             const cvae_cycle_state* state_in, const cvae_cycle_state* state_out);

int cvae_profile_collect(cvae_ctx* ctx, double* total_ms, int* launches);
int cvae_profile_collect_launches(cvae_ctx* ctx, double* ms, int* rows, int* cin, int cap);

int cvae_step_timing(cvae_ctx* ctx, const cvae_net_desc* d, int B, int T, const void* workspace, double out[8], void* stream);


typedef struct cvae_net_grads {
    float *conv0_w, *conv0_b, *conv1_w, *conv1_b, *w_ih, *w_hh, *b_ih, *b_hh, *out_w, *out_b;
} cvae_net_grads;

size_t cvae_train_image_bytes(cvae_ctx* ctx, const cvae_net_desc* d);
int cvae_net_prepare_train(cvae_ctx* ctx, const cvae_net_desc* d, const cvae_net_weights* w, void* image, size_t image_bytes, float gru_drop_p,
                           void* stream);
int cvae_net_prepare_train_v(cvae_ctx* ctx, const cvae_net_desc* d, const cvae_net_weights* w, void* image, size_t image_bytes, float gru_drop_p,
                             int variants, void* stream);
int cvae_train_variants_needed(cvae_ctx* ctx, const cvae_net_desc* d, int B, int T);
size_t cvae_train_tape_bytes(cvae_ctx* ctx, const cvae_net_desc* d, int B, int T);
size_t cvae_train_scratch_bytes(cvae_ctx* ctx, const cvae_net_desc* d, int B, int T);

int cvae_gru_rnn_forward_train(cvae_ctx* ctx, const cvae_net_desc* d, const void* image, const float* x, const float* y_in, const float* h_in,
                               int B, int T, int clamp_lat_dim, const float* cmask, const float* gmask, uint64_t seed,
                               float p_drop, float* trj_out, float* y_last, float* h_last, void* tape, size_t tape_bytes,
                               void* scratch, size_t scratch_bytes, void* stream);

int cvae_set_side_stream(cvae_ctx* ctx, void* stream);
int cvae_join_side_stream(cvae_ctx* ctx, void* stream);

int cvae_gru_rnn_backward(cvae_ctx* ctx, const cvae_net_desc* d, const void* image, const float* dout, int B, int T, int clamp_lat_dim,
                          const void* tape, void* scratch, size_t scratch_bytes, float* dx, const cvae_net_grads* g,
                          int accumulate, void* stream);

int cvae_train_profile_collect(cvae_ctx* ctx, double total_ms[4], int launches[4], double flop[4]);

int cvae_train_debug_counters(cvae_ctx* ctx, const cvae_net_desc* d, int B, int T, const void* scratch, long long out[8], void* stream);

int cvae_adam_step(cvae_ctx* ctx, float* param, const float* grad, float* exp_avg, float* exp_avg_sq, size_t n, float lr, float beta1,
                   float beta2, float eps, int step, const int32_t* gate, void* stream);
int cvae_adam_step_counted(cvae_ctx* ctx, float* param, const float* grad, float* exp_avg, float* exp_avg_sq, size_t n, float lr, float beta1,
                           float beta2, float eps, int32_t* state, const int32_t* gate, void* stream);

int cvae_sample_cat(cvae_ctx* ctx, const float* lat, const float* code0, const float* code1, const float* eps0, const float* eps1, uint64_t seed,
                    uint64_t draw0, uint64_t draw1, int B, int T, int lat_dim, int ncode, int parts, float* out, float* eps_out,
                    void* stream);
int cvae_sample_cat_backward(cvae_ctx* ctx, const float* dout, const float* lat, const float* eps, int B, int T, int lat_dim, int ncode, int parts,
                             float* dlat, void* stream);
int cvae_stage4_loss(cvae_ctx* ctx, const float* rec, const float* reccyc, const float* lat, const float* latcv, const float* x, int x_stride, int stdim,
                     const float* w, const float* latcv_w, float kl_scale, int B, int T, int D, int lat_dim, float* d_rec,
                     float* d_reccyc, float* d_lat, float* d_latcv, float* frame_loss, float* loss, int accumulate, void* stream);
int cvae_mcd_l1(cvae_ctx* ctx, const float* x, long x_stride, const float* y, long y_stride, int frames, int D, float* frame_mcd, float* out3, void* stream);
int cvae_mcd_l1_backward(cvae_ctx* ctx, const float* x, long x_stride, const float* y, long y_stride, int frames, int D, const float* frame_mcd,
                         const float* out3, const float* g3, float* dx, void* stream);
int cvae_kl_gauss(cvae_ctx* ctx, const float* param, long stride, int frames, int lat_dim, float* out1, void* stream);
int cvae_kl_gauss_backward(cvae_ctx* ctx, const float* param, long stride, int frames, int lat_dim, const float* g1, float* dparam, void* stream);

int cvae_gv_postfilter(cvae_ctx* ctx, const float* c, int T, int D, const double* dpow, const double* gv_trg, const double* cvgv, double* out,
                       double* out_var, double* work, void* stream);

int cvae_mc2e(cvae_ctx* ctx, const void* mc, int is_f64, long ld, int T, int D, double alpha, int irlen, double* e_out, void* stream);

int cvae_mcd_aligned(cvae_ctx* ctx, const float* a, long lda, const float* b, long ldb, int rows, int D, int d0, int l2, double* frames,
                     double* stats, void* stream);

size_t cvae_dtw_work_bytes(cvae_ctx* ctx, int T1, int T2);
int cvae_dtw_org_to_trg(cvae_ctx* ctx, const double* org, const double* trg, int T1, int T2, int D, int mcd, double* aligned, long long* twf,
                        double* frames, double* mean_out, void* work, size_t work_bytes, void* stream);

// ... 77 lines not shown
```

Baseline: 1.317 million.

## Fuse output projection with next pass prologue at cycle chain boundaries

```diff
diff --git a/cyclevae-vc_amd/_cabi.py b/cyclevae-vc_amd/_cabi.py
--- a/cyclevae-vc_amd/_cabi.py
+++ b/cyclevae-vc_amd/_cabi.py
@@ -9,6 +9,7 @@
 FLAG_HOISTED_FRONTEND = 32
 FLAG_SPLIT_F16 = 256
 FLAG_EXACT3 = 512
+FLAG_PLAN_CARRY = 1024
 STATUS_RANGE = 7
 STATUS_RANGE_WORD = 3
 CLAMP_LAPLACE = 1 << 30
@@ -221,6 +222,8 @@
         L.cvae_sample_laplace_backward.argtypes = [_fp, _fp, _fp, C.c_int, C.c_int, _fp, _fp]
         L.cvae_cycle_workspace_bytes.restype = C.c_size_t
         L.cvae_cycle_workspace_bytes.argtypes = [C.POINTER(NetDesc), C.POINTER(NetDesc), C.c_int, C.c_int, C.c_int]
+        L.cvae_cycle_plan.restype = C.c_int
+        L.cvae_cycle_plan.argtypes = [C.POINTER(NetDesc), C.POINTER(NetDesc), C.c_int, C.c_int, C.c_int, C.c_int, C.POINTER(C.c_int)]
         L.cvae_cycle_forward.restype = C.c_int
         L.cvae_cycle_forward.argtypes = [C.POINTER(NetDesc), _fp, C.POINTER(NetDesc), _fp, _fp, _fp, C.c_int, _fp, _fp,
                                          C.c_int, _fp, _fp, C.c_int, C.c_int, C.c_int, C.c_int, _fp, C.c_uint64,
@@ -465,6 +468,11 @@
             raise CvaeError("cvae_cycle_workspace_bytes: bad arguments")
         return n
 
+    def cycle_plan(self, de, dd, B, T, n_cyc, flags=0):
+        n = C.c_int(0)
+        self._check(self.lib.cvae_cycle_plan(C.byref(de), C.byref(dd), B, T, n_cyc, flags, C.byref(n)), "cvae_cycle_plan")
+        return n.value
+
     def cycle_forward(self, de, enc_prep, dd, dec_prep, x, cvx, stdim, code_src, code_trg, ncode, y_in_enc, y_in_dec,
                       B, T, n_cyc, lat_dim, eps, seed, out_lat, out_rec, out_cv, out_latcv, out_reccyc, ws, ws_bytes,
                       flags=0, stream=0):
@@ -679,7 +687,7 @@
 EXPORTS = ("cvae_last_error_string", "cvae_abi_version", "cvae_ctx_create", "cvae_ctx_destroy", "cvae_set_status_sink", "cvae_status_latch", "cvae_set_draw_origin", "cvae_set_draw_parts",
            "cvae_set_option", "cvae_get_option", "cvae_reset_options", "cvae_selftest_limbs", "cvae_selftest_occupy", "cvae_selftest_gemm_work_bytes", "cvae_selftest_gemm", "cvae_set_side_stream", "cvae_join_side_stream", "cvae_net_prepared_bytes", "cvae_net_prepare_scratch_bytes",
            "cvae_net_prepare", "cvae_pass_workspace_bytes", "cvae_gru_rnn_forward", "cvae_gru_rnn_forward_stacked", "cvae_gru_rnn_forward_stacked_carry", "cvae_sample", "cvae_sample_laplace", "cvae_sample_laplace_backward",
-           "cvae_cycle_workspace_bytes", "cvae_cycle_forward", "cvae_cycle_forward_carry", "cvae_profile_collect", "cvae_profile_collect_launches", "cvae_train_profile_collect", "cvae_step_timing", "cvae_workspace_status",
+           "cvae_cycle_workspace_bytes", "cvae_cycle_plan", "cvae_cycle_forward", "cvae_cycle_forward_carry", "cvae_profile_collect", "cvae_profile_collect_launches", "cvae_train_profile_collect", "cvae_step_timing", "cvae_workspace_status",
            "cvae_train_image_bytes", "cvae_net_prepare_train", "cvae_net_prepare_train_v", "cvae_train_variants_needed", "cvae_train_tape_bytes", "cvae_train_scratch_bytes",
            "cvae_gru_rnn_forward_train", "cvae_gru_rnn_backward", "cvae_adam_step", "cvae_adam_step_counted", "cvae_train_debug_counters",
            "cvae_sample_cat", "cvae_sample_cat_backward", "cvae_stage4_loss", "cvae_mcd_l1", "cvae_mcd_l1_backward", "cvae_kl_gauss",
diff --git a/cyclevae-vc_amd/csrc/cvae_exact3.h b/cyclevae-vc_amd/csrc/cvae_exact3.h
--- a/cyclevae-vc_amd/csrc/cvae_exact3.h
+++ b/cyclevae-vc_amd/csrc/cvae_exact3.h
@@ -425,19 +425,19 @@
     }
 }
 
-template <int KPW>
-__global__ __launch_bounds__(256) void k_outproj_v6(Out6Params p) {
+template <int KPW, int NT>
+__device__ __forceinline__ void cvae_outproj_tiles(const Out6Params& p, int bx, int n0, float* red, float* keep, int keep_ld) {
     constexpr float S1 = 1.0f / 2048.0f;
     constexpr int RS = 36;
     const int tid = threadIdx.x, wave = cvae_uniform(tid >> 6), lane = tid & 63, lc = lane & 31, kh = lane >> 5;
     const int nk = p.H >> 4, nt32 = p.Bp >> 5;
-    const int n = blockIdx.y;
-    const long tile = (long)nt32 + blockIdx.x;
-    float* red = (float*)CVAE_SMEM;
+    const long tile = (long)nt32 + bx;
     const long tstride = p.mtot >> 5;
-    f32x16 a0 = cvae_zero16(), a1 = cvae_zero16(), a2 = cvae_zero16(), a3 = cvae_zero16();
-    constexpr int RD = KPW < 4 ? KPW : 4;
-    f32x4 ha[2 * RD], wb[3 * RD];
+    f32x16 a0[NT], a1[NT], a2[NT], a3[NT];
+#pragma unroll
+    for (int j = 0; j < NT; ++j) a0[j] = cvae_zero16(), a1[j] = cvae_zero16(), a2[j] = cvae_zero16(), a3[j] = cvae_zero16();
+    constexpr int RD0 = 4 / NT, RD = KPW < RD0 ? KPW : RD0;
+    f32x4 ha[2 * RD], wb[NT * 3 * RD];
     f32x2 hb[RD];
     auto load = [&](int s) {
         const int sg = wave * KPW + s;
@@ -445,9 +445,12 @@
         ha[2 * (s % RD)] = *(const f32x4*)(hp + kh * 512 + lc * 16);
         ha[2 * (s % RD) + 1] = *(const f32x4*)(hp + 1024 + kh * 512 + lc * 16);
         hb[s % RD] = *(const f32x2*)(hp + 2048 + kh * 256 + lc * 8);
-        const float* wp = p.wo3 + (((long)n * nk + sg) * 3) * 256 + lane * 4;
-#pragma unroll
-        for (int m = 0; m < 3; ++m) wb[3 * (s % RD) + m] = *(const f32x4*)(wp + m * 256);
+#pragma unroll
+        for (int j = 0; j < NT; ++j) {
+            const float* wp = p.wo3 + (((long)(n0 + j) * nk + sg) * 3) * 256 + lane * 4;
+#pragma unroll
+            for (int m = 0; m < 3; ++m) wb[(j * RD + s % RD) * 3 + m] = *(const f32x4*)(wp + m * 256);
+        }
     };
     const bool has_k = wave * KPW < nk;
     if (has_k) {
@@ -456,39 +459,95 @@
 #pragma unroll
         for (int s = 0; s < KPW; ++s) {
             const f32x4 l0 = ha[2 * (s % RD)], l1 = ha[2 * (s % RD) + 1], l2 = cvae_bf8x8_to_h8(hb[s % RD]);
-            const f32x4 w0 = wb[3 * (s % RD)], w1 = wb[3 * (s % RD) + 1], w2 = wb[3 * (s % RD) + 2];
-            a0 = cvae_mfma_32x32x16_f16(l0, w0, a0);
-            a1 = cvae_mfma_32x32x16_f16(l0, w1, a1);
-            a2 = cvae_mfma_32x32x16_f16(l1, w1, a2);
-            a3 = cvae_mfma_32x32x16_f16(l0, w2, a3);
-            a1 = cvae_mfma_32x32x16_f16(l1, w0, a1);
-            a2 = cvae_mfma_32x32x16_f16(l2, w0, a2);
+#pragma unroll
+            for (int j = 0; j < NT; ++j) {
+                const f32x4 w0 = wb[(j * RD + s % RD) * 3], w1 = wb[(j * RD + s % RD) * 3 + 1], w2 = wb[(j * RD + s % RD) * 3 + 2];
+                a0[j] = cvae_mfma_32x32x16_f16(l0, w0, a0[j]);
+                a1[j] = cvae_mfma_32x32x16_f16(l0, w1, a1[j]);
+                a2[j] = cvae_mfma_32x32x16_f16(l1, w1, a2[j]);
+                a3[j] = cvae_mfma_32x32x16_f16(l0, w2, a3[j]);
+                a1[j] = cvae_mfma_32x32x16_f16(l1, w0, a1[j]);
+                a2[j] = cvae_mfma_32x32x16_f16(l2, w0, a2[j]);
+            }
             cvae_sched_fence();
             if (s + RD < KPW) load(s + RD);
         }
     }
 #pragma unroll
-    for (int q = 0; q < 16; ++q)
-        red[(wave * 32 + (q & 3) + 8 * (q >> 2) + 4 * kh) * RS + lc] = a0[q] + (a1[q] + (a2[q] + a3[q]) * S1) * S1;
+    for (int j = 0; j < NT; ++j)
+#pragma unroll
+        for (int q = 0; q < 16; ++q)
+            red[((j * 4 + wave) * 32 + (q & 3) + 8 * (q >> 2) + 4 * kh) * RS + lc] = a0[j][q] + (a1[j][q] + (a2[j][q] + a3[j][q]) * S1) * S1;
     __syncthreads();
     {
         const int r = tid >> 3;
-        const long m = (long)blockIdx.x * 32 + r;
+        const long m = (long)bx * 32 + r;
         const int t = (int)(m / p.Bp), b = (int)(m - (long)t * p.Bp);
         if (b < p.ncell * p.B) {
             const int cell = b / p.B, bb = b - cell * p.B;
             float* orow = p.out[cell] + ((long)bb * p.T + t) * p.Co;
 #pragma unroll
-            for (int jj = 0; jj < 4; ++jj) {
-                const int cl = (tid & 7) + 8 * jj, col = 32 * n + cl;
-                if (col < p.Co) {
-                    float v = red[(0 * 32 + r) * RS + cl] + red[(1 * 32 + r) * RS + cl] + red[(2 * 32 + r) * RS + cl] +
-                              red[(3 * 32 + r) * RS + cl] + p.bo2[col];
-                    if (p.clamp_from >= 0 && col >= p.clamp_from) v = fmaxf(v, p.clamp_min);
-                    orow[col] = v;
+            for (int j = 0; j < NT; ++j) {
+                const float* rj = red + j * 4 * 32 * RS;
+#pragma unroll
+                for (int jj = 0; jj < 4; ++jj) {
+                    const int cl = (tid & 7) + 8 * jj, col = 32 * (n0 + j) + cl;
+                    if (col < p.Co) {
+                        float v = rj[(0 * 32 + r) * RS + cl] + rj[(1 * 32 + r) * RS + cl] + rj[(2 * 32 + r) * RS + cl] +
+                                  rj[(3 * 32 + r) * RS + cl] + p.bo2[col];
+                        if (p.clamp_from >= 0 && col >= p.clamp_from) v = fmaxf(v, p.clamp_min);
+                        orow[col] = v;
+                        if (keep) keep[r * keep_ld + col] = v;
+                    }
                 }
             }
         }
+    }
+}
+
+template <int KPW>
+__global__ __launch_bounds__(256) void k_outproj_v6(Out6Params p) {
+    cvae_outproj_tiles<KPW, 1>(p, (int)blockIdx.x, (int)blockIdx.y, (float*)CVAE_SMEM, nullptr, 0);
+}
+
+#define CVAE_BOUNDARY_CELLS 2
+struct BoundaryParams {
+    Out6Params out;
+    ProParamsN<CVAE_BOUNDARY_CELLS> pro;
+    int nF, nP;
+    int cell_tiles;
+    unsigned feed;
+    int keep_ld;
+};
+static_assert(sizeof(BoundaryParams) <= 4096, "BoundaryParams is a kernel argument: 4 KiB at most");
+
+template <int KPW>
+__global__ __launch_bounds__(256, 2) void k_boundary_v6(BoundaryParams p) {
+    const int blk = (int)blockIdx.x;
+    if (blk >= p.nF) {
+        int pb = p.pro.nA + (blk - p.nF - p.nP);
+        if (blk - p.nF < p.nP) {
+            const int tile = (blk - p.nF) / (2 * p.pro.pad), e = (blk - p.nF) % (2 * p.pro.pad);
+            pb = tile * (p.pro.T + 2 * p.pro.pad) + (e < p.pro.pad ? e : p.pro.T + e);
+        }
+        cvae_prologue_block(p.pro, pb);
+        return;
+    }
+    const int ntn = (p.out.Co + 31) >> 5;
+    float* red = (float*)CVAE_SMEM;
+    float* keep = red + 2 * 4 * 32 * 36;
+    float* asm_smem = keep + 32 * p.keep_ld;
+    for (int n0 = 0; n0 < ntn; n0 += 2) {
+        if (n0 > 0) __syncthreads();
+        if (n0 + 2 <= ntn) cvae_outproj_tiles<KPW, 2>(p.out, blk, n0, red, keep, p.keep_ld);
+        else cvae_outproj_tiles<KPW, 1>(p.out, blk, n0, red, keep, p.keep_ld);
+    }
+    const int nt32 = p.out.Bp >> 5, i = blk % nt32, t = blk / nt32;
+    const int sc = i / p.cell_tiles;
+    for (int dc = 0; dc < CVAE_BOUNDARY_CELLS; ++dc) {
+        if (!((p.feed >> (CVAE_BOUNDARY_CELLS * sc + dc)) & 1u)) continue;
+        __syncthreads();
+        cvae_assemble_tile(p.pro, dc * p.cell_tiles + i % p.cell_tiles, t + p.pro.pad, asm_smem, keep, p.keep_ld);
     }
 }
 
diff --git a/cyclevae-vc_amd/csrc/cvae_kernels.h b/cyclevae-vc_amd/csrc/cvae_kernels.h
--- a/cyclevae-vc_amd/csrc/cvae_kernels.h
+++ b/cyclevae-vc_amd/csrc/cvae_kernels.h
@@ -189,8 +189,7 @@
 #define CVAE_FRAME_VALID(p, c, t) ((t) >= -(c).ctx_before && (t) < ((c).frames > 0 ? (c).frames : (p).T) + (c).ctx_after)
 
 #define CVAE_MAX_CELLS 32
-struct ProParams {
-    ProCell cell[CVAE_MAX_CELLS];
+struct ProCommon {
     int ncell, L;
     uint64_t frame0;
     const float* sin_w;
@@ -222,6 +221,11 @@
     float range_at;
     const int* image_unfit;
 };
+template <int NC>
+struct ProParamsN : ProCommon {
+    ProCell cell[NC];
+};
+typedef ProParamsN<CVAE_MAX_CELLS> ProParams;
 #ifndef CVAE_STATUS_RANGE_WORD
 #define CVAE_STATUS_RANGE_WORD 3
 #endif
@@ -234,10 +238,12 @@
 }
 static_assert(sizeof(ProParams) <= 4096, "ProParams is a kernel argument: 4 KiB at most");
 
-__device__ __forceinline__ float cvae_input_value(const ProParams& p, const ProCell& c, int b, int t, int q, const float* emean = nullptr) {
+template <class PP>
+__device__ __forceinline__ float cvae_input_value(const PP& p, const ProCell& c, int b, int t, int q, const float* emean = nullptr,
+                                                  const float* prow = nullptr) {
     const long fr = (long)b * p.T + t;
     if (q < c.seg0.width) return c.seg0.ptr[fr * c.seg0.row_stride + q];
-    if (!c.lat) return c.seg1.ptr[fr * c.seg1.row_stride + (q - c.seg0.width)];
+    if (!c.lat) return prow ? prow[q - c.seg0.width] : c.seg1.ptr[fr * c.seg1.row_stride + (q - c.seg0.width)];
     const int l = q - c.seg0.width;
     float e;
     if (c.n_draws > 1 && emean) {
@@ -252,10 +258,12 @@
     } else {
         e = c.eps ? c.eps[fr * p.L + l] : cvae_randn(c.seed, c.draw, (uint64_t)(fr + c.draw_frame0) + p.frame0, (uint32_t)l);
     }
-    return c.lat[fr * 2 * p.L + l] + expf(c.lat[fr * 2 * p.L + p.L + l] * 0.5f) * e;
-}
-
-__device__ __forceinline__ void cvae_mean_draws(const ProParams& p, const ProCell& c, int b, int t, float* part, float* emean) {
+    const float* lt = prow ? prow : c.lat + fr * 2 * p.L;
+    return lt[l] + expf(lt[p.L + l] * 0.5f) * e;
+}
+
+template <class PP>
+__device__ __forceinline__ void cvae_mean_draws(const PP& p, const ProCell& c, int b, int t, float* part, float* emean) {
     const int tid = threadIdx.x, L = p.L, nq = L >> 2, nsl = 256 / nq, qd = tid % nq, sl = tid / nq;
     const long fr = (long)b * p.T + t;
     const long es = c.eps_stride ? c.eps_stride : (long)p.B * p.T * p.L;
@@ -284,88 +292,96 @@
     __syncthreads();
 }
 
-__global__ void k_prologue(ProParams p) {
-    const int tid = threadIdx.x, blk = blockIdx.x;
+template <class PP>
+__device__ __forceinline__ void cvae_assemble_tile(const PP& p, int tile, int tp, float* smem, const float* prev, int prev_ld) {
+    const int tid = threadIdx.x;
+    float* raw = smem;
+    unsigned char* img = (unsigned char*)(raw + 32 * (p.C + 1));
+    const int Tp = p.T + 2 * p.pad, t = tp - p.pad, np = p.Cp >> 3;
+    float* tmean = (float*)(img + np * 1280);
+    const bool quads = p.L > 0 && (p.L & 3) == 0;
+    if (quads) {
+        const int nq = p.L >> 2;
+        for (int item = tid; item < 32 * nq; item += 256) {
+            const int r = item / nq, qd = item - r * nq, bb = tile * 32 + r;
+            if (bb >= p.ncell * p.B) continue;
+            const ProCell& c = p.cell[bb / p.B];
+            if (!c.lat || c.n_draws <= 1 || !CVAE_FRAME_VALID(p, c, t)) continue;
+            const long fr = (long)(bb % p.B) * p.T + t, es = c.eps_stride ? c.eps_stride : (long)p.B * p.T * p.L;
+            float e[4] = {0.f, 0.f, 0.f, 0.f};
+            for (int k = 0; k < c.n_draws; ++k) {
+                float z[4];
+                if (c.eps) {
+                    const float* ep = c.eps + (long)k * es + fr * p.L + 4 * qd;
+                    z[0] = ep[0]; z[1] = ep[1]; z[2] = ep[2]; z[3] = ep[3];
+                } else {
+                    cvae_randn4(c.seed, c.draw + (uint64_t)k, (uint64_t)(fr + c.draw_frame0) + p.frame0, (uint32_t)qd, z);
+                }
+#pragma unroll
+                for (int j = 0; j < 4; ++j) e[j] += z[j];
+            }
+#pragma unroll
+            for (int j = 0; j < 4; ++j) tmean[r * p.L + 4 * qd + j] = e[j] * (1.0f / (float)c.n_draws);
+        }
+        __syncthreads();
+    }
+    for (int idx = tid; idx < 32 * p.C; idx += 256) {
+        const int r = idx / p.C, q = idx - r * p.C, bb = tile * 32 + r;
+        float v = 0.0f;
+        if (bb < p.ncell * p.B) {
+            const ProCell& c = p.cell[bb / p.B];
+            if (CVAE_FRAME_VALID(p, c, t))
+                v = cvae_input_value(p, c, bb % p.B, t, q, quads ? tmean + r * p.L : nullptr, prev ? prev + r * prev_ld : nullptr);
+        }
+        raw[r * (p.C + 1) + q] = v;
+    }
+    __syncthreads();
+    const ProCell* const cells = p.cell;
+    bool bad = false;
+    for (int q = tid & 63; q < p.Cp; q += 64) {
+        float v[8];
+        bool ok[8];
+#pragma unroll
+        for (int i = 0; i < 8; ++i) {
+            const int r = (tid >> 6) + 4 * i, bb = tile * 32 + r;
+            ok[i] = false;
+            if (bb < p.ncell * p.B) {
+                const ProCell& c = cells[bb / p.B];
+                ok[i] = CVAE_FRAME_VALID(p, c, t) && q < p.C;
+            }
+            v[i] = !ok[i] ? 0.0f : (p.sin_w ? p.sin_b[q] : raw[r * (p.C + 1) + q]);
+        }
+        if (p.sin_w && q < p.C)
+            for (int k = 0; k < p.C; ++k) {
+                const float w = p.sin_w[(long)q * p.C + k];
+#pragma unroll
+                for (int i = 0; i < 8; ++i) v[i] += w * raw[((tid >> 6) + 4 * i) * (p.C + 1) + k];
+            }
+        unsigned char* pc = img + (q >> 3) * 1280;
+#pragma unroll
+        for (int i = 0; i < 8; ++i) {
+            const int r = (tid >> 6) + 4 * i;
+            unsigned short l0, l1;
+            unsigned char l2;
+            cvae_split3_f16b8(ok[i] ? v[i] : 0.0f, l0, l1, l2);
+            bad = bad || (ok[i] && cvae_out_of_range(v[i], p.range_at));
+            ((unsigned short*)pc)[r * 8 + (q & 7)] = l0;
+            ((unsigned short*)(pc + 512))[r * 8 + (q & 7)] = l1;
+            pc[1024 + r * 8 + (q & 7)] = l2;
+        }
+    }
+    const bool fits = cvae_block_all(!bad);
+    if (!fits && p.range_word && tid == 0) *p.range_word = p.range_val;
+    f32x4* dst = (f32x4*)((unsigned char*)p.xt + ((long)tile * Tp + tp) * np * 1280);
+    for (int e = tid; e < np * 80; e += 256) dst[e] = ((const f32x4*)img)[e];
+}
+
+template <class PP>
+__device__ __forceinline__ void cvae_prologue_block(const PP& p, int blk) {
+    const int tid = threadIdx.x;
     const int Tp = p.T + 2 * p.pad;
     if (blk < p.nA && p.xt) {
-        float* raw = (float*)CVAE_SMEM;
-        unsigned char* img = (unsigned char*)(raw + 32 * (p.C + 1));
-        const int tile = blk / Tp, tp = blk % Tp, t = tp - p.pad, np = p.Cp >> 3;
-        float* tmean = (float*)(img + np * 1280);
-        const bool quads = p.L > 0 && (p.L & 3) == 0;
-        if (quads) {
-            const int nq = p.L >> 2;
-            for (int item = tid; item < 32 * nq; item += 256) {
-                const int r = item / nq, qd = item - r * nq, bb = tile * 32 + r;
-                if (bb >= p.ncell * p.B) continue;
-                const ProCell& c = p.cell[bb / p.B];
-                if (!c.lat || c.n_draws <= 1 || !CVAE_FRAME_VALID(p, c, t)) continue;
-                const long fr = (long)(bb % p.B) * p.T + t, es = c.eps_stride ? c.eps_stride : (long)p.B * p.T * p.L;
-                float e[4] = {0.f, 0.f, 0.f, 0.f};
-                for (int k = 0; k < c.n_draws; ++k) {
-                    float z[4];
-                    if (c.eps) {
-                        const float* ep = c.eps + (long)k * es + fr * p.L + 4 * qd;
-                        z[0] = ep[0]; z[1] = ep[1]; z[2] = ep[2]; z[3] = ep[3];
-                    } else {
-                        cvae_randn4(c.seed, c.draw + (uint64_t)k, (uint64_t)(fr + c.draw_frame0) + p.frame0, (uint32_t)qd, z);
-                    }
-#pragma unroll
-                    for (int j = 0; j < 4; ++j) e[j] += z[j];
-                }
-#pragma unroll
-                for (int j = 0; j < 4; ++j) tmean[r * p.L + 4 * qd + j] = e[j] * (1.0f / (float)c.n_draws);
-            }
-            __syncthreads();
-        }
-        for (int idx = tid; idx < 32 * p.C; idx += 256) {
-            const int r = idx / p.C, q = idx - r * p.C, bb = tile * 32 + r;
-            float v = 0.0f;
-            if (bb < p.ncell * p.B) {
-                const ProCell& c = p.cell[bb / p.B];
-                if (CVAE_FRAME_VALID(p, c, t)) v = cvae_input_value(p, c, bb % p.B, t, q, quads ? tmean + r * p.L : nullptr);
-            }
-            raw[r * (p.C + 1) + q] = v;
-        }
-        __syncthreads();
-        const ProCell* const cells = p.cell;
-        bool bad = false;
-        for (int q = tid & 63; q < p.Cp; q += 64) {
-            float v[8];
-            bool ok[8];
-#pragma unroll
-            for (int i = 0; i < 8; ++i) {
-                const int r = (tid >> 6) + 4 * i, bb = tile * 32 + r;
-                ok[i] = false;
-                if (bb < p.ncell * p.B) {
-                    const ProCell& c = cells[bb / p.B];
-                    ok[i] = CVAE_FRAME_VALID(p, c, t) && q < p.C;
-                }
-                v[i] = !ok[i] ? 0.0f : (p.sin_w ? p.sin_b[q] : raw[r * (p.C + 1) + q]);
-            }
-            if (p.sin_w && q < p.C)
-                for (int k = 0; k < p.C; ++k) {
-                    const float w = p.sin_w[(long)q * p.C + k];
-#pragma unroll
-                    for (int i = 0; i < 8; ++i) v[i] += w * raw[((tid >> 6) + 4 * i) * (p.C + 1) + k];
-                }
-            unsigned char* pc = img + (q >> 3) * 1280;
-#pragma unroll
-            for (int i = 0; i < 8; ++i) {
-                const int r = (tid >> 6) + 4 * i;
-                unsigned short l0, l1;
-                unsigned char l2;
-                cvae_split3_f16b8(ok[i] ? v[i] : 0.0f, l0, l1, l2);
-                bad = bad || (ok[i] && cvae_out_of_range(v[i], p.range_at));
-                ((unsigned short*)pc)[r * 8 + (q & 7)] = l0;
-                ((unsigned short*)(pc + 512))[r * 8 + (q & 7)] = l1;
-                pc[1024 + r * 8 + (q & 7)] = l2;
-            }
-        }
-        const bool fits = cvae_block_all(!bad);
-        if (!fits && p.range_word && tid == 0) *p.range_word = p.range_val;
-        f32x4* dst = (f32x4*)((unsigned char*)p.xt + ((long)tile * Tp + tp) * np * 1280);
-        for (int e = tid; e < np * 80; e += 256) dst[e] = ((const f32x4*)img)[e];
+        cvae_assemble_tile(p, blk / Tp, blk % Tp, (float*)CVAE_SMEM, nullptr, 0);
         return;
     }
     if (p.nG > 0 && blk >= p.nA + p.nH + p.nD && blk < p.nA + p.nH + p.nD + p.nG) {
@@ -532,6 +548,8 @@
     }
 }
 
+__global__ void k_prologue(ProParams p) { cvae_prologue_block(p, (int)blockIdx.x); }
+
 __global__ void k_sample(const float* lat, int rows, int L, const float* eps, uint64_t seed, uint64_t draw,
                          float* z, float* eps_out, uint64_t frame0) {
     const long idx = (long)blockIdx.x * blockDim.x + threadIdx.x;
diff --git a/cyclevae-vc_amd/csrc/cvae_lib.hip b/cyclevae-vc_amd/csrc/cvae_lib.hip
--- a/cyclevae-vc_amd/csrc/cvae_lib.hip
+++ b/cyclevae-vc_amd/csrc/cvae_lib.hip
@@ -23,7 +23,7 @@
 
 enum OptId {
     OPT_V6_LIMBS_H64, OPT_NO_LL, OPT_MAX_RT, OPT_LL_BACKOFF, OPT_EXP, OPT_GEMM_FORCE, OPT_GEMM_LOG, OPT_TRAIN_OLD_GEMM,
-    OPT_GEMM_TRACE, OPT_TRAIN_PER_STEP, OPT_TRAIN_PROF, OPT_TRAIN_BACKOFF, OPT_TRAIN_FP32_MFMA, OPT_TRAIN_BWD_PER_STEP, OPT_TRAIN_KERNEL, OPT_X3_TILE, OPT_BWD_OVERFLOW_AT, OPT_GEMM_MAX_SPLIT, OPT_BWD_KS, OPT_COOP_LAUNCH, OPT_V6_LIMBS_H2048, OPT_V6_W2S_H64, OPT_STEP_COL_TILES, OPT_TRAIN_PROFILE, OPT_TRAIN_XMAP, OPT_MASKS_ON_SIDE, OPT_V6_BACKOFF, OPT_TRAIN_BWD_BACKOFF, OPT_LL_ROW_PAD, OPT_GEMM_MIN_DEPTH, OPT_TRAIN_BWD_GEOM, OPT_BWD_W3_L1_H64, OPT_TRAIN_FWD_GEOM, OPT_TRAIN_FWD_BACKOFF, OPT_EXACT_RANGE_AT, OPT_DTW_BATCH_COST, OPT_COUNT
+    OPT_GEMM_TRACE, OPT_TRAIN_PER_STEP, OPT_TRAIN_PROF, OPT_TRAIN_BACKOFF, OPT_TRAIN_FP32_MFMA, OPT_TRAIN_BWD_PER_STEP, OPT_TRAIN_KERNEL, OPT_X3_TILE, OPT_BWD_OVERFLOW_AT, OPT_GEMM_MAX_SPLIT, OPT_BWD_KS, OPT_COOP_LAUNCH, OPT_V6_LIMBS_H2048, OPT_V6_W2S_H64, OPT_STEP_COL_TILES, OPT_TRAIN_PROFILE, OPT_TRAIN_XMAP, OPT_MASKS_ON_SIDE, OPT_V6_BACKOFF, OPT_TRAIN_BWD_BACKOFF, OPT_LL_ROW_PAD, OPT_GEMM_MIN_DEPTH, OPT_TRAIN_BWD_GEOM, OPT_BWD_W3_L1_H64, OPT_TRAIN_FWD_GEOM, OPT_TRAIN_FWD_BACKOFF, OPT_EXACT_RANGE_AT, OPT_DTW_BATCH_COST, OPT_CHAIN_FUSE, OPT_COUNT
 };
 struct OptEntry { const char* name; long dflt; };
 const OptEntry g_opt[OPT_COUNT] = {
@@ -63,6 +63,7 @@
     {"train_fwd_backoff", -1},
     {"exact_range_at", 65504},
     {"dtw_batch_cost", 1},
+    {"chain_fuse", 0},
 };
 
 struct ProfEvents {
@@ -228,6 +229,9 @@
 };
 struct Out6Inst { int H; void (*fn)(Out6Params); };
 const Out6Inst g_out6_inst[] = {{1024, k_outproj_v6<16>}, {2048, k_outproj_v6<32>}, {64, k_outproj_v6<1>}};
+
+struct Bnd6Inst { int H; void (*fn)(BoundaryParams); };
+const Bnd6Inst g_bnd6_inst[] = {{1024, k_boundary_v6<16>}, {2048, k_boundary_v6<32>}, {64, k_boundary_v6<1>}};
 
 inline int exact3_kpw(const Dims& m) { return m.H / 64; }
 inline const V6Inst* find_v6(const Dims& m, int limbs = -1, bool w2s = false) {
@@ -546,8 +550,8 @@
 };
 struct RangeSlot { int* word; int val; float at; };
 
-void run_prologue(const Dims& m, const cvae_net_desc* d, const float* P, const Prep& pl, const PassRows& r, const ProTargets& o,
-                  hipStream_t st, RangeSlot* range = nullptr) {
+ProParams prologue_params(const Dims& m, const cvae_net_desc* d, const float* P, const Prep& pl, const PassRows& r, const ProTargets& o,
+                          RangeSlot* range = nullptr) {
     const Cell* cells = r.cells;
     const int ncell = r.ncell, B = r.B, T = r.T, Bp = r.Bp, shape = o.shape;
     const int Brows = ncell * B, Tp = T + 2 * m.pad;
@@ -590,10 +594,18 @@
     pp.gx0 = o.gx0; pp.wyT = P + pl.wyT;
     range_params(pp, o.ws_status, o.limbs, o.new_call, P, pl);
     if (range) *range = RangeSlot{pp.range_word, pp.range_val, pp.range_at};
+    return pp;
+}
+inline size_t pro_tiles_lds(const Dims& m, int L) {
+    return (size_t)32 * (m.C + 1) * sizeof(float) + (size_t)(m.Cp / 8) * 1280 + (size_t)32 * L * sizeof(float);
+}
+void run_prologue(const Dims& m, const cvae_net_desc* d, const float* P, const Prep& pl, const PassRows& r, const ProTargets& o,
+                  hipStream_t st, RangeSlot* range = nullptr) {
+    const ProParams pp = prologue_params(m, d, P, pl, r, o, range);
+    const int shape = o.shape;
     const dim3 gp(pp.nA + pp.nH + pp.nD + pp.nG + 1);
     if (shape == PRO_TILES)
-        hipLaunchKernelGGL((k_prologue), gp, dim3(256),
-                           (size_t)32 * (m.C + 1) * sizeof(float) + (size_t)(m.Cp / 8) * 1280 + (size_t)32 * pp.L * sizeof(float), st, pp);
+        hipLaunchKernelGGL((k_prologue), gp, dim3(256), pro_tiles_lds(m, pp.L), st, pp);
     else if (shape == PRO_DRAWS)
         hipLaunchKernelGGL((k_prologue), gp, dim3(256), (size_t)(m.C + 1024 + 256) * sizeof(float), st, pp);
     else
@@ -648,15 +660,84 @@
                                m.H, last_slot(r.cells[c].in, r.T), c * r.B);
 }
 
-int run_pass(const Dims& m, const cvae_net_desc* d, const float* P, const Cell* cells, int ncell, int B, int T,
-             int clamp_lat_dim, float* ws, int* status, int flags, hipStream_t st, bool clear_status = false) {
-    const Prep pl = prep_layout(m, d->has_scale_in != 0, d->has_scale_out != 0);
-    const int Brows = ncell * B;
-    const Work wl = work_layout(m, Brows, T);
-    int* const ws_status = status;
-    if (cx().status_sink) status = cx().status_sink;
-    const PassRows rows = {cells, ncell, B, T, wl.Bp, wl.mtot};
-    if (int rc = check_cells(m, rows)) return rc;
+struct PassJob {
+    Dims m;
+    const cvae_net_desc* d;
+    const float* P;
+    Prep pl;
+    Work wl;
+    PassRows rows;
+    EvalPlan pn;
+    float* ws;
+    int* status;
+    int* ws_status;
+    int flags, clamp_lat_dim;
+    bool clear_status;
+};
+
+int plan_pass_job(PassJob& j, const Dims& m, const cvae_net_desc* d, const float* P, const Cell* cells, int ncell, int B, int T,
+                  int clamp_lat_dim, float* ws, int* status, int flags, bool clear_status) {
+    j.m = m; j.d = d; j.P = P;
+    j.pl = prep_layout(m, d->has_scale_in != 0, d->has_scale_out != 0);
+    j.wl = work_layout(m, ncell * B, T);
+    j.ws = ws; j.ws_status = status;
+    j.status = cx().status_sink ? cx().status_sink : status;
+    j.flags = flags; j.clamp_lat_dim = clamp_lat_dim; j.clear_status = clear_status;
+    j.rows = PassRows{cells, ncell, B, T, j.wl.Bp, j.wl.mtot};
+    if (int rc = check_cells(m, j.rows)) return rc;
+    PassFacts facts = {};
+    for (int c = 0; c < ncell; ++c) {
+        facts.h_in = facts.h_in || cells[c].h_in != nullptr;
+        facts.y_last = facts.y_last || cells[c].y_last != nullptr;
+        facts.h_last = facts.h_last || cells[c].h_last != nullptr;
+        facts.many_draws = facts.many_draws || (cells[c].in->lat && cells[c].in->n_draws > 1);
+    }
+    j.pn = plan_eval_pass(m, ncell * B, T, flags, cu_count(), image_known_unfit(P), facts);
+    return 0;
+}
+
+ProTargets pass_pro_targets(const PassJob& j) {
+    const Dims& m = j.m;
+    const Work& wl = j.wl;
+    const EvalPlan& pn = j.pn;
+    float* const ws = j.ws;
+    int* const status = j.status;
+    int* const ws_status = j.ws_status;
+    const bool clear_status = j.clear_status;
+    float* xnp = ws + wl.xnp;
+    float* hbuf = ws + wl.hbuf;
+    float* dy = ws + wl.dy;
+    unsigned* hflags = (unsigned*)(ws + wl.flags);
+    ProTargets o = {};
+    o.shape = pn.prologue; o.xnp = xnp; o.dy = dy;
+    o.slot0 = hbuf;
+    o.zero_words = hflags; o.nzero = wl.Bp / 16 * m.nch;
+    o.zero_status = clear_status ? status : nullptr;
+    o.zero_status_n = cx().status_sink ? 4 : 8;
+    o.ws_status = ws_status; o.limbs = pn.limbs; o.new_call = clear_status;
+    const bool triples = pn.form == CVAE_EVAL_V6 || pn.form == CVAE_EVAL_V6H;
+    o.hx = triples ? ws + wl.hs : nullptr;
+    o.xt = pn.form == CVAE_EVAL_V6 ? ws + wl.xt : nullptr;
+    o.nxt_slack = (int)wl.xt_slack;
+    o.hs = pn.pairs ? ws + wl.hs : nullptr;
+    o.xs = pn.pairs ? ws + wl.xs : nullptr;
+    o.xs_plane = wl.xs_plane;
+    o.gx0 = pn.gx0_ready ? ws + wl.gx0 : nullptr;
+    o.ll_counter = pn.form == CVAE_EVAL_LL ? (unsigned*)(ws + wl.status) + 16 : nullptr;
+    return o;
+}
+
+void pass_prologue(const PassJob& j, hipStream_t st) { run_prologue(j.m, j.d, j.P, j.pl, j.rows, pass_pro_targets(j), st); }
+
+int pass_recurrence(const PassJob& j, hipStream_t st) {
+    const Dims& m = j.m;
+    const float* P = j.P;
+    const Prep& pl = j.pl;
+    const Work& wl = j.wl;
+    const EvalPlan& pn = j.pn;
+    float* const ws = j.ws;
+    int* const status = j.status;
+    const int flags = j.flags, ncell = j.rows.ncell, B = j.rows.B, T = j.rows.T, Brows = ncell * B;
     unsigned* bar = (unsigned*)(ws + wl.status) + 8;
     float* xnp = ws + wl.xnp;
     float* gx = ws + wl.gx;
@@ -665,35 +746,6 @@
     unsigned* hflags = (unsigned*)(ws + wl.flags);
     long long* const step_prof = (flags & CVAE_FLAG_STEP_TIMING) ? (long long*)(ws + wl.prof) : nullptr;
     const int cus = cu_count();
-    PassFacts facts = {};
-    for (int c = 0; c < ncell; ++c) {
-        facts.h_in = facts.h_in || cells[c].h_in != nullptr;
-        facts.y_last = facts.y_last || cells[c].y_last != nullptr;
-        facts.h_last = facts.h_last || cells[c].h_last != nullptr;
-        facts.many_draws = facts.many_draws || (cells[c].in->lat && cells[c].in->n_draws > 1);
-    }
-    const EvalPlan pn = plan_eval_pass(m, Brows, T, flags, cus, image_known_unfit(P), facts);
-
-    {
-        ProTargets o = {};
-        o.shape = pn.prologue; o.xnp = xnp; o.dy = dy;
-        o.slot0 = hbuf;
-        o.zero_words = hflags; o.nzero = wl.Bp / 16 * m.nch;
-        o.zero_status = clear_status ? status : nullptr;
-        o.zero_status_n = cx().status_sink ? 4 : 8;
-        o.ws_status = ws_status; o.limbs = pn.limbs; o.new_call = clear_status;
-        const bool triples = pn.form == CVAE_EVAL_V6 || pn.form == CVAE_EVAL_V6H;
-        o.hx = triples ? ws + wl.hs : nullptr;
-        o.xt = pn.form == CVAE_EVAL_V6 ? ws + wl.xt : nullptr;
-        o.nxt_slack = (int)wl.xt_slack;
-        o.hs = pn.pairs ? ws + wl.hs : nullptr;
-        o.xs = pn.pairs ? ws + wl.xs : nullptr;
-        o.xs_plane = wl.xs_plane;
-        o.gx0 = pn.gx0_ready ? ws + wl.gx0 : nullptr;
-        o.ll_counter = pn.form == CVAE_EVAL_LL ? (unsigned*)(ws + wl.status) + 16 : nullptr;
-        run_prologue(m, d, P, pl, rows, o, st);
-    }
-
     const size_t lds2 = (4 * 16 * 84 + 16 * 16) * sizeof(float);
     const bool prof = (flags & CVAE_FLAG_PROFILE) && prof_begin(st, ncell * B, m.C);
     const auto refused = [](hipError_t e) {
@@ -793,21 +845,100 @@
     }
     }
     if (prof) prof_end(st);
-
-    if (pn.proj == PROJ_V6) {
-        Out6Params op;
-        op.hx = ws + wl.hs; op.mtot = wl.mtot; op.wo3 = P + pl.wo3; op.bo2 = P + pl.bo2; op.H = m.H; op.Bp = wl.Bp; op.T = T;
-        op.B = B; op.ncell = ncell; op.Co = m.Co; op.clamp_from = d->has_scale_out ? -1 : clamp_dim(clamp_lat_dim);
-        op.clamp_min = clamp_floor(clamp_lat_dim);
-        for (int c = 0; c < CVAE_MAX_CELLS; ++c) op.out[c] = c < ncell ? cells[c].trj_out : nullptr;
-        const dim3 g((unsigned)((long)T * wl.Bp / 32), (unsigned)((m.Cop + 31) / 32));
-        hipLaunchKernelGGL(pn.kout6, g, dim3(256), (size_t)4 * 32 * 36 * sizeof(float), st, op);
+    return 0;
+}
+
+Out6Params out6_params(const PassJob& j) {
+    const Dims& m = j.m;
+    const cvae_net_desc* d = j.d;
+    const float* P = j.P;
+    const Prep& pl = j.pl;
+    const Work& wl = j.wl;
+    const EvalPlan& pn = j.pn;
+    const PassRows& rows = j.rows;
+    float* const ws = j.ws;
+    const int ncell = rows.ncell, B = rows.B, T = rows.T, clamp_lat_dim = j.clamp_lat_dim;
+    const Cell* cells = rows.cells;
+    Out6Params op;
+    op.hx = ws + wl.hs; op.mtot = wl.mtot; op.wo3 = P + pl.wo3; op.bo2 = P + pl.bo2; op.H = m.H; op.Bp = wl.Bp; op.T = T;
+    op.B = B; op.ncell = ncell; op.Co = m.Co; op.clamp_from = d->has_scale_out ? -1 : clamp_dim(clamp_lat_dim);
+    op.clamp_min = clamp_floor(clamp_lat_dim);
+    for (int c = 0; c < CVAE_MAX_CELLS; ++c) op.out[c] = c < ncell ? cells[c].trj_out : nullptr;
+    return op;
+}
+
+void pass_projection(const PassJob& j, hipStream_t st) {
+    const Dims& m = j.m;
+    if (j.pn.proj == PROJ_V6) {
+        const dim3 g((unsigned)((long)j.rows.T * j.wl.Bp / 32), (unsigned)((m.Cop + 31) / 32));
+        hipLaunchKernelGGL(j.pn.kout6, g, dim3(256), (size_t)4 * 32 * 36 * sizeof(float), st, out6_params(j));
     } else {
-        run_projection(m, d, P, pl, rows, pn.proj, hbuf, ws + wl.y, clamp_lat_dim, st);
-    }
-    run_last_states(m, rows, hbuf, st);
+        run_projection(m, j.d, j.P, j.pl, j.rows, j.pn.proj, j.ws + j.wl.hbuf, j.ws + j.wl.y, j.clamp_lat_dim, st);
+    }
+}
+
+void pass_last_states(const PassJob& j, hipStream_t st) { run_last_states(j.m, j.rows, j.ws + j.wl.hbuf, st); }
+
+int run_pass(const Dims& m, const cvae_net_desc* d, const float* P, const Cell* cells, int ncell, int B, int T,
+             int clamp_lat_dim, float* ws, int* status, int flags, hipStream_t st, bool clear_status = false) {
+    PassJob j;
+    if (int rc = plan_pass_job(j, m, d, P, cells, ncell, B, T, clamp_lat_dim, ws, status, flags, clear_status)) return rc;
+    pass_prologue(j, st);
+    if (int rc = pass_recurrence(j, st)) return rc;
+    pass_projection(j, st);
+    pass_last_states(j, st);
     CVAE_HIP_OK(hipGetLastError());
     return 0;
+}
+
+typedef unsigned Feed;
+inline bool feeds(Feed f, int sc, int dc) { return ((f >> (CVAE_BOUNDARY_CELLS * sc + dc)) & 1u) != 0; }
+
+bool boundary_plans_fusable(const EvalPlan& a, const Dims& am, int a_ncell, const EvalPlan& b, int b_ncell, int B) {
+    if (!opt(OPT_CHAIN_FUSE)) return false;
+    if (a.form != CVAE_EVAL_V6 || a.proj != PROJ_V6 || b.form != CVAE_EVAL_V6 || b.prologue != PRO_TILES) return false;
+    if (B % 32 || a_ncell > CVAE_BOUNDARY_CELLS || b_ncell > CVAE_BOUNDARY_CELLS) return false;
+    for (const Bnd6Inst& i : g_bnd6_inst)
+        if (i.H == am.H) return true;
+    return false;
+}
+bool boundary_cells_fusable(const PassJob& a, const PassJob& b, Feed f) {
+    int fed[CVAE_BOUNDARY_CELLS] = {};
+    for (int sc = 0; sc < CVAE_BOUNDARY_CELLS; ++sc)
+        for (int dc = 0; dc < CVAE_BOUNDARY_CELLS; ++dc)
+            if (feeds(f, sc, dc)) {
+                if (sc >= a.rows.ncell || dc >= b.rows.ncell) return false;
+                fed[dc] += 1;
+            }
+    for (int c = 0; c < b.rows.ncell; ++c) {
+        const cvae_pass_input* in = b.rows.cells[c].in;
+        if (in->frames || in->n_draws > 1 || in->ctx_before || in->ctx_after || in->draw_frame0) return false;
+        const int w = in->lat ? 2 * in->lat_dim : in->seg1.width;
+        if (fed[c] != (w > 0 ? 1 : 0) || (w > 0 && w != a.m.Co)) return false;
+    }
+    return true;
+}
+
+void run_boundary(const PassJob& a, const PassJob& b, Feed f, hipStream_t st) {
+    BoundaryParams bp;
+    memset(&bp, 0, sizeof(bp));
+    bp.out = out6_params(a);
+    const ProParams pp = prologue_params(b.m, b.d, b.P, b.pl, b.rows, pass_pro_targets(b));
+    (ProCommon&)bp.pro = (const ProCommon&)pp;
+    for (int c = 0; c < CVAE_BOUNDARY_CELLS; ++c) bp.pro.cell[c] = pp.cell[c];
+    const int T = a.rows.T;
+    bp.nF = a.wl.Bp / 32 * T;
+    bp.nP = b.wl.Bp / 32 * 2 * b.m.pad;
+    bp.cell_tiles = a.rows.B / 32;
+    bp.feed = f;
+    const int ntn = (a.m.Co + 31) / 32;
+    bp.keep_ld = 32 * ntn + 1;
+    void (*fn)(BoundaryParams) = nullptr;
+    for (const Bnd6Inst& i : g_bnd6_inst)
+        if (i.H == a.m.H) fn = i.fn;
+    const int roles = (opt(OPT_EXP) & 128) ? 0 : bp.nP + pp.nH + pp.nD + pp.nG + 1;
+    const size_t lds = (size_t)(2 * 4 * 32 * 36 + 32 * bp.keep_ld) * sizeof(float) + pro_tiles_lds(b.m, pp.L);
+    hipLaunchKernelGGL(fn, dim3(bp.nF + roles), dim3(256), lds, st, bp);
 }
 
 }
@@ -1121,11 +1252,12 @@
     return 0;
 }
 
-static long cycle_layout(const Dims& me, const Dims& md, int B, int T, long* pass_off, long* traj_off) {
+static long cycle_layout(const Dims& me, const Dims& md, int B, int T, long* pass_off, long* pass_size, long* traj_off) {
     const long pe = work_layout(me, B, T).total, pd = work_layout(md, 2 * B, T).total;
     long o = 64;
     *pass_off = o;
-    o += pe > pd ? pe : pd;
+    *pass_size = pe > pd ? pe : pd;
+    o += 2 * *pass_size;
     *traj_off = o;
     o += up((long)B * T * me.Co, 64) * 2 + up((long)B * T * md.Co, 64) * 3;
     return o;
@@ -1135,9 +1267,12 @@
     CVAE_ENTER_SZ(ctx);
     Dims me, md;
     if (make_dims(enc, &me) || make_dims(dec, &md) || B < 1 || T < 1 || n_cyc < 1) return 0;
-    long po, to;
-    return (size_t)cycle_layout(me, md, B, T, &po, &to) * sizeof(float);
-}
+    long po, ps, to;
+    return (size_t)cycle_layout(me, md, B, T, &po, &ps, &to) * sizeof(float);
+}
+
+static const Feed g_chain_feed[4] = {1u << 0 | 1u << 1, 1u << (CVAE_BOUNDARY_CELLS * 1 + 0), 1u << 0, 1u << 0};
+static const int g_chain_ncell[4] = {1, 2, 1, 1};
 
 static int cycle_forward_impl(const cvae_net_desc* enc, const void* enc_prepared, const cvae_net_desc* dec,
                        const void* dec_prepared, const float* x, const float* cvx, int stdim, const float* code_src,
@@ -1157,9 +1292,8 @@
     if (workspace_bytes < cvae_cycle_workspace_bytes(tl_ctx, enc, dec, B, T, n_cyc)) return fail(-2, "workspace too small");
     hipStream_t st = (hipStream_t)stream;
     float* ws = (float*)workspace;
-    long po, to;
-    cycle_layout(me, md, B, T, &po, &to);
-    float* pws = ws + po;
+    long po, ps, to;
+    cycle_layout(me, md, B, T, &po, &ps, &to);
     const long ne = (long)B * T * me.Co, nd = (long)B * T * md.Co;
     float* t_lat = ws + to;
     float* t_latcv = t_lat + up(ne, 64);
@@ -1176,56 +1310,75 @@
     auto yd = [&](const cvae_cycle_state* s, int i, int slot) { return s ? s->y_dec + ((long)i * 3 + slot) * B * md.Co : nullptr; };
     auto hd = [&](const cvae_cycle_state* s, int i, int slot) { return s ? s->h_dec + ((long)i * 3 + slot) * B * md.H : nullptr; };
 
+    struct ChainPass { cvae_pass_input in[2]; Cell cells[2]; };
+    std::vector<ChainPass> cp((size_t)4 * n_cyc);
     for (int i = 0; i < n_cyc; ++i) {
         float* lat = out_lat ? out_lat + i * ne : t_lat;
         float* latcv = out_latcv ? out_latcv + i * ne : t_latcv;
         float* rec = out_rec ? out_rec + i * nd : t_rec;
         float* cv = out_cv ? out_cv + i * nd : t_cv;
         float* reccyc = out_reccyc ? out_reccyc + i * nd : t_reccyc;
-        cvae_pass_input in, in2;
-        memset(&in, 0, sizeof(in));
-        int rc;
+        ChainPass* q = &cp[(size_t)4 * i];
+        for (int k = 0; k < 4; ++k) memset(q[k].in, 0, sizeof(q[k].in));
         if (i == 0) {
-            in.seg0 = cvae_seg{x, me.C, me.C};
+            q[0].in[0].seg0 = cvae_seg{x, me.C, me.C};
         } else {
-            in.seg0 = cvae_seg{x, stdim, me.C};
-            in.seg1 = cvae_seg{prev_reccyc, md.Co, md.Co};
+            q[0].in[0].seg0 = cvae_seg{x, stdim, me.C};
+            q[0].in[0].seg1 = cvae_seg{prev_reccyc, md.Co, md.Co};
         }
-        {
-            const Cell c{&in, sin ? ye(sin, i, 0) : y_in_enc, he(sin, i, 0), lat, ye(sout, i, 0), he(sout, i, 0)};
-            if ((rc = run_pass(me, enc, (const float*)enc_prepared, &c, 1, B, T, lat_dim, pws, status, flags, st, i == 0))) return rc;
-        }
-        memset(&in, 0, sizeof(in));
+        q[0].cells[0] = Cell{&q[0].in[0], sin ? ye(sin, i, 0) : y_in_enc, he(sin, i, 0), lat, ye(sout, i, 0), he(sout, i, 0)};
+        cvae_pass_input& in = q[1].in[0];
         in.seg0 = cvae_seg{code_src, ncode, ncode};
         in.lat = lat; in.lat_dim = lat_dim;
         in.eps = eps ? eps + (i * 3 + 0) * neps : nullptr;
         in.seed = seed; in.draw_id = (uint64_t)(i * 3 + 0);
+        cvae_pass_input& in2 = q[1].in[1];
         in2 = in;
         in2.seg0 = cvae_seg{code_trg, ncode, ncode};
         in2.eps = eps ? eps + (i * 3 + 1) * neps : nullptr;
         in2.draw_id = (uint64_t)(i * 3 + 1);
-        {
-            const Cell c2[2] = {{&in, sin ? yd(sin, i, 0) : y_in_dec, hd(sin, i, 0), rec, yd(sout, i, 0), hd(sout, i, 0)},
-                                {&in2, sin ? yd(sin, i, 1) : y_in_dec, hd(sin, i, 1), cv, yd(sout, i, 1), hd(sout, i, 1)}};
-            if ((rc = run_pass(md, dec, (const float*)dec_prepared, c2, 2, B, T, -1, pws, status, flags, st))) return rc;
+        q[1].cells[0] = Cell{&in, sin ? yd(sin, i, 0) : y_in_dec, hd(sin, i, 0), rec, yd(sout, i, 0), hd(sout, i, 0)};
+        q[1].cells[1] = Cell{&in2, sin ? yd(sin, i, 1) : y_in_dec, hd(sin, i, 1), cv, yd(sout, i, 1), hd(sout, i, 1)};
+        q[2].in[0].seg0 = cvae_seg{cvx, stdim, stdim};
+        q[2].in[0].seg1 = cvae_seg{cv, md.Co, md.Co};
+        q[2].cells[0] = Cell{&q[2].in[0], sin ? ye(sin, i, 1) : y_in_enc, he(sin, i, 1), latcv, ye(sout, i, 1), he(sout, i, 1)};
+        cvae_pass_input& in3 = q[3].in[0];
+        in3.seg0 = cvae_seg{code_src, ncode, ncode};
+        in3.lat = latcv; in3.lat_dim = lat_dim;
+        in3.eps = eps ? eps + (i * 3 + 2) * neps : nullptr;
+        in3.seed = seed; in3.draw_id = (uint64_t)(i * 3 + 2);
+        q[3].cells[0] = Cell{&in3, sin ? yd(sin, i, 2) : y_in_dec, hd(sin, i, 2), reccyc, yd(sout, i, 2), hd(sout, i, 2)};
+        prev_reccyc = reccyc;
+    }
+    const int npass = 4 * n_cyc;
+    auto plan = [&](PassJob& j, int k) {
+        const bool e = k % 2 == 0;
+        return plan_pass_job(j, e ? me : md, e ? enc : dec, (const float*)(e ? enc_prepared : dec_prepared), cp[k].cells, g_chain_ncell[k % 4],
+                             B, T, e ? lat_dim : -1, ws + po + (k % 2) * ps, status, flags, k == 0);
+    };
+    PassJob cur, nxt;
+    if (int rc = plan(cur, 0)) return rc;
+    pass_prologue(cur, st);
+    for (int k = 0; k < npass; ++k) {
+        if (int rc = pass_recurrence(cur, st)) return rc;
+        const bool last = k + 1 == npass;
+        if (!last) {
+            if (int rc = plan(nxt, k + 1)) return rc;
+            const Feed f = g_chain_feed[k % 4];
+            if (boundary_plans_fusable(cur.pn, cur.m, cur.rows.ncell, nxt.pn, nxt.rows.ncell, B) && boundary_cells_fusable(cur, nxt, f)) {
+                run_boundary(cur, nxt, f, st);
+                pass_last_states(cur, st);
+            } else {
+                pass_projection(cur, st);
+                pass_last_states(cur, st);
+                pass_prologue(nxt, st);
+            }
+        } else {
+            pass_projection(cur, st);
+            pass_last_states(cur, st);
         }
-        memset(&in, 0, sizeof(in));
-        in.seg0 = cvae_seg{cvx, stdim, stdim};
-        in.seg1 = cvae_seg{cv, md.Co, md.Co};
-        {
-            const Cell c{&in, sin ? ye(sin, i, 1) : y_in_enc, he(sin, i, 1), latcv, ye(sout, i, 1), he(sout, i, 1)};
-            if ((rc = run_pass(me, enc, (const float*)enc_prepared, &c, 1, B, T, lat_dim, pws, status, flags, st))) return rc;
-        }
-        memset(&in, 0, sizeof(in));
-        in.seg0 = cvae_seg{code_src, ncode, ncode};
-        in.lat = latcv; in.lat_dim = lat_dim;
-        in.eps = eps ? eps + (i * 3 + 2) * neps : nullptr;
-        in.seed = seed; in.draw_id = (uint64_t)(i * 3 + 2);
-        {
-            const Cell c{&in, sin ? yd(sin, i, 2) : y_in_dec, hd(sin, i, 2), reccyc, yd(sout, i, 2), hd(sout, i, 2)};
-            if ((rc = run_pass(md, dec, (const float*)dec_prepared, &c, 1, B, T, -1, pws, status, flags, st))) return rc;
-        }
-        prev_reccyc = reccyc;
+        CVAE_HIP_OK(hipGetLastError());
+        if (!last) cur = nxt;
     }
     return 0;
 }
@@ -1252,6 +1405,26 @@
     return cycle_forward_impl(enc, enc_prepared, dec, dec_prepared, x, cvx, stdim, code_src, code_trg, ncode, y_in_enc, y_in_dec,
                               B, T, n_cyc, lat_dim, eps, seed, out_lat, out_rec, out_cv, out_latcv, out_reccyc, workspace,
                               workspace_bytes, flags, stream, state_in, state_out);
+}
+
+int cvae_cycle_plan(cvae_ctx* ctx, const cvae_net_desc* enc, const cvae_net_desc* dec, int B, int T, int n_cyc, int flags,
+                    int* fused_boundaries) {
+    CVAE_ENTER(ctx);
+    Dims me, md;
+    if (int rc = make_dims(enc, &me)) return rc;
+    if (int rc = make_dims(dec, &md)) return rc;
+    if (B < 1 || T < 1 || n_cyc < 1 || !fused_boundaries) return fail(-1, "bad argument: B=%d T=%d n_cyc=%d", B, T, n_cyc);
+    const bool carry = (flags & CVAE_FLAG_PLAN_CARRY) != 0;
+    PassFacts facts = {};
+    facts.h_in = facts.y_last = facts.h_last = carry;
+    EvalPlan pn[4];
+    for (int k = 0; k < 4; ++k)
+        pn[k] = plan_eval_pass(k % 2 ? md : me, g_chain_ncell[k] * B, T, flags & ~CVAE_FLAG_PLAN_CARRY, cu_count(), false, facts);
+    int n = 0;
+    for (int k = 0; k + 1 < 4 * n_cyc; ++k)
+        if (boundary_plans_fusable(pn[k % 4], k % 2 ? md : me, g_chain_ncell[k % 4], pn[(k + 1) % 4], g_chain_ncell[(k + 1) % 4], B)) n += 1;
+    *fused_boundaries = n;
+    return 0;
 }
 
 int cvae_step_timing(cvae_ctx* ctx, const cvae_net_desc* d, int B, int T, const void* workspace, double out[8], void* stream) {
diff --git a/include/cyclevae_hip.h b/include/cyclevae_hip.h
--- a/include/cyclevae_hip.h
+++ b/include/cyclevae_hip.h
@@ -112,6 +112,7 @@
 #define CVAE_FLAG_GENERIC_STEP 4
 #define CVAE_FLAG_STEP_TIMING 8
 #define CVAE_FLAG_PROFILE 2
+#define CVAE_FLAG_PLAN_CARRY 1024
 
 #define CVAE_STATUS_RANGE 7
 #define CVAE_STATUS_RANGE_WORD 3
@@ -176,6 +177,9 @@
                        int B, int T, int n_cyc, int lat_dim, const float* eps, uint64_t seed,
                        float* out_lat, float* out_rec, float* out_cv, float* out_latcv, float* out_reccyc,
                        void* workspace, size_t workspace_bytes, int flags, void* stream);
+
+int cvae_cycle_plan(cvae_ctx* ctx, const cvae_net_desc* enc, const cvae_net_desc* dec, int B, int T, int n_cyc, int flags,
+                    int* fused_boundaries);
 
 typedef struct cvae_cycle_state {
     float* y_enc;
```

Result: no change. 1.318 million, median of 5 (+0.1%).
